# adam-kerrigan/pybader

Hardware: AMD Instinct MI355X
Metric: Mvoxels/s neargrid assign+refine on 512^3 grid (higher is better)
Workload: dtype f64; 1 GPU; 512^3 synthetic 8-Gaussian-atom cubic cell (BASELINE config 3), neargrid assign + neargrid edge refinement changed:2, density resident in HBM; method=neargrid, device_driven_slab_step=False, basins=8

## Files before the change

include/bader_hip.h:

```cpp
#ifndef BADER_HIP_H
#define BADER_HIP_H

#include <stdint.h>

#ifdef __cplusplus
extern "C" {
#endif

typedef struct xb_ctx xb_ctx;

enum { XB_OK = 0, XB_E_ARG = -1, XB_E_HIP = -2, XB_E_STATE = -3, XB_E_LIMIT = -4, XB_E_COMM = -5,
       XB_E_SHORT = -6  };

enum { XB_I8 = 1, XB_I16 = 2, XB_I32 = 4, XB_I64 = 8 };

enum { XB_METHOD_ONGRID = 0, XB_METHOD_NEARGRID = 1 };
enum { XB_REFINE_ALL = 0, XB_REFINE_CHANGED = 1 };

const char *xb_last_error(void);
int xb_device_count(void);
int xb_create(int device, xb_ctx **out);
void xb_destroy(xb_ctx *c);
int xb_sync(xb_ctx *c);
void *xb_stream(xb_ctx *c);
// ... 123 lines not shown
    XB_XC_LOST = 5,
    XB_XC_MINE = 6,
    XB_XC_ROUNDS = 7,
    XB_XC_COUNT = 8
};
int xb_slab_refine_counts(xb_ctx *c, int64_t *local, int64_t *global);
int xb_slab_block(xb_ctx *c, int which, void **dev_ptr, int64_t *bytes_total, int64_t *own_offset, int64_t *own_bytes);
int xb_slab_block_copy(xb_ctx *c, int which, int to_device, void *host, int64_t off, int64_t bytes);
int xb_host_waits(int64_t *n);

enum {
    XB_TIMER_ASSIGN = 0,
    XB_TIMER_OG_MASKS = 1,
    XB_TIMER_EDGE_FIND = 2,
    XB_TIMER_REFINE_TRACE = 3,
    XB_TIMER_MASKS_GROWTH = 4,
    XB_TIMER_BRICK_MASKS = 5,
    XB_TIMER_TRACE = 6,
    XB_TIMER_BRICK_RECORDS = 7,
    XB_TIMER_MOMENTS = 8,
    XB_TIMER_ADJACENCY = 9,
    XB_TIMER_MERGE = 10,
    XB_TIMER_COUNT = 11
};
int xb_kernel_time(xb_ctx *c, int which, double *ms_total, int64_t *launches);
int xb_kernel_time_reset(xb_ctx *c);
int xb_enable_timing(xb_ctx *c, int on);
enum {
    XB_OPT_REGIONS = 1,
    XB_OPT_CROSS_CHECK = 2,
    XB_OPT_DEBUG = 3,
    XB_OPT_EC_GROUPS = 4,
    XB_OPT_EC_QCAP = 5,
    XB_OPT_DROP_TABLE = 6,
    XB_OPT_KILL_LAUNCHES = 17,
    XB_OPT_SELF_EXCHANGE = 19,
    XB_OPT_ASYNC_COMM = 24,
    XB_OPT_WEIGHT_NO_LABELS = 30
};
enum {
    XB_REGIONS_BOXES = 1,
    XB_REGIONS_BRICKS = 2
};
enum { XB_DROP_TABLE_AND_MAXIMA = 2 };
enum {
    XB_CHECK_NO_MIRROR = 1,
    XB_CHECK_GENERIC_WALKER = 2,
    XB_CHECK_FULL_TGRAD = 4,
    XB_CHECK_LIST_DILATE = 8,
    XB_CHECK_WIDE_HALO = 16,
    XB_CHECK_NO_EC_SHARE = 32,
    XB_CHECK_IO_GATHER = 64
};
enum {
    XB_DBG_EC_PASSES = 4,
    XB_DBG_SLAB_STATS = 16,
    XB_DBG_STAGE_WAIT = 32,
    XB_DBG_SHORT_TIERS = 64
};
int xb_set_option(xb_ctx *c, int key, int value);
int xb_host_alloc(int64_t bytes, void **out);
int xb_host_free(void *p);
int xb_memory_stats(xb_ctx *c, int64_t *bytes_total, int64_t *bytes_table, int64_t *bytes_scratch);
int xb_box_stats(xb_ctx *c, int64_t *n_boxes, int64_t *box_voxels);
int xb_brick_labels(xb_ctx *c, int32_t *out, int64_t capacity, int64_t dims[3]);
int xb_slow_path_stats(xb_ctx *c, int64_t *assign_total, int64_t *refine_total);
int xb_deferred_stats(xb_ctx *c, int64_t *refine_total);
int xb_growth_stats(xb_ctx *c, int64_t *retries, int64_t *kill_launches);

int xb_comm_unique_id(uint8_t id_out[128]);
int xb_comm_init(xb_ctx *c, int rank, int nranks, const uint8_t id_in[128]);
int xb_comm_destroy(xb_ctx *c);
int xb_comm_exchange_planes(xb_ctx *c, int which, int n_send, const int32_t *send_peer, const int64_t *send_xa,
                            const int64_t *send_xb, int n_recv, const int32_t *recv_peer, const int64_t *recv_xa,
                            const int64_t *recv_xb);
int xb_comm_allreduce_i64(xb_ctx *c, int64_t *inout, int64_t n, int op);
int xb_comm_allgather_i64(xb_ctx *c, const int64_t *in, int64_t n, int64_t *out);
int xb_comm_share_brick_masks(xb_ctx *c, const int64_t *first, const int64_t *count);
int xb_comm_allgather_block(xb_ctx *c, int which, const int64_t *first, const int64_t *count);
int xb_comm_allreduce_block(xb_ctx *c);
int xb_comm_info(xb_ctx *c, int64_t out[4]);
int xb_comm_stats(xb_ctx *c, int64_t *bytes_sent);

#ifdef __cplusplus
}
#endif
#endif
```

pybader_amd/_lib.py:

```python
import ctypes as C
import threading
import os

import numpy as np

HERE = os.path.dirname(os.path.abspath(__file__))
LIB_PATH = os.environ.get('XB_LIBRARY') or os.path.join(HERE, 'libbader_hip.so')

METHODS = {'ongrid': 0, 'neargrid': 1}
REFINE_MODES = {'all': 0, 'changed': 1}
DTYPE_CODE = {np.dtype(np.int8): 1, np.dtype(np.int16): 2, np.dtype(np.int32): 4, np.dtype(np.int64): 8}
(XB_XC_EDGES, XB_XC_CHANGED, XB_XC_ESCAPED, XB_XC_TRAVELLING, XB_XC_SLOW, XB_XC_LOST, XB_XC_MINE, XB_XC_ROUNDS,
 XB_XC_COUNT) = range(9)
(XB_TIMER_ASSIGN, XB_TIMER_OG_MASKS, XB_TIMER_EDGE_FIND, XB_TIMER_REFINE_TRACE, XB_TIMER_MASKS_GROWTH, XB_TIMER_BRICK_MASKS,
 XB_TIMER_TRACE, XB_TIMER_BRICK_RECORDS, XB_TIMER_MOMENTS, XB_TIMER_ADJACENCY, XB_TIMER_MERGE, XB_TIMER_COUNT) = range(12)
XB_OPT_REGIONS = 1
XB_REGIONS_BOXES, XB_REGIONS_BRICKS = 1, 2
XB_OPT_CROSS_CHECK = 2
(XB_CHECK_NO_MIRROR, XB_CHECK_GENERIC_WALKER, XB_CHECK_FULL_TGRAD, XB_CHECK_LIST_DILATE, XB_CHECK_WIDE_HALO,
 XB_CHECK_NO_EC_SHARE, XB_CHECK_IO_GATHER) = (1, 2, 4, 8, 16, 32, 64)
XB_OPT_DEBUG = 3
XB_DBG_EC_PASSES, XB_DBG_SLAB_STATS, XB_DBG_STAGE_WAIT, XB_DBG_SHORT_TIERS = 4, 16, 32, 64
XB_OPT_EC_GROUPS = 4
XB_OPT_EC_QCAP = 5
XB_OPT_DROP_TABLE = 6
XB_DROP_TABLE_AND_MAXIMA = 2
XB_OPT_KILL_LAUNCHES = 17
XB_OPT_SELF_EXCHANGE = 19
XB_OPT_ASYNC_COMM = 24
XB_OPT_WEIGHT_NO_LABELS = 30
XB_VORONOI_FULL_SEARCH = 1
XB_VORONOI_CAND_MAX = 512

_vp, _i64, _dbl, _int = C.c_void_p, C.c_int64, C.c_double, C.c_int
_pi64, _pdbl = C.POINTER(C.c_int64), C.POINTER(C.c_double)
SYMBOLS = {
    'xb_last_error': (C.c_char_p, []),
    'xb_device_count': (_int, []),
    'xb_create': (_int, [_int, C.POINTER(_vp)]),
    'xb_destroy': (None, [_vp]),
    'xb_sync': (_int, [_vp]),
    'xb_stream': (_vp, [_vp]),
    'xb_set_grid': (_int, [_vp, _pi64, _pdbl, _pdbl, _i64, _i64]),
    'xb_upload_density': (_int, [_vp, _vp]),
    'xb_synth_density': (_int, [_vp, _pdbl, _pdbl, _i64, _dbl]),
    'xb_parse_density_text': (_int, [_vp, _vp, _i64, _dbl, _pi64, _pi64]),
    'xb_parse_cube_text': (_int, [_vp, _vp, _i64, _i64, _i64, _int, _dbl, _pi64, _pi64]),
    'xb_download_density': (_int, [_vp, _vp]),
    'xb_format_begin': (_int, [_vp, _vp, _pi64, _int, _dbl, _int, _int, _vp, _i64, _i64, _pi64]),
    'xb_format_host_values': (_int, [_vp, _vp, _vp]),
    'xb_format_set_host_text': (_int, [_vp, _vp, _vp]),
    'xb_format_next': (_int, [_vp, C.POINTER(_vp), _pi64]),
    'xb_format_times': (_int, [_vp, _pdbl, _pdbl]),
    'xb_format_end': (_int, [_vp]),
    'xb_upload_labels': (_int, [_vp, _vp, _int]),
    'xb_download_labels': (_int, [_vp, _vp, _int]),
    'xb_import_density': (_int, [_vp, _vp, _int, _pi64, _vp]),
    'xb_import_labels': (_int, [_vp, _vp, _int, _vp]),
    'xb_export_labels': (_int, [_vp, _vp, _int, _vp]),
    'xb_export_volume': (_int, [_vp, _i64, _vp, _int, _vp]),
    'xb_device_alloc': (_int, [_int, _i64, C.POINTER(_vp)]),
    'xb_device_free': (_int, [_vp]),
    'xb_device_read': (_int, [_vp, _vp, _vp, _i64, _vp]),
    'xb_upload_known': (_int, [_vp, _vp]),
    'xb_download_known': (_int, [_vp, _vp]),
    'xb_vacuum_assign': (_int, [_vp, _dbl, _dbl, _pdbl, _pdbl]),
    'xb_assign': (_int, [_vp, _int, _pi64]),
    'xb_get_maxima': (_int, [_vp, _vp, _i64]),
    'xb_assign_trace': (_int, [_vp, _int, _pi64]),
    'xb_assign_local_table': (_int, [_vp, _vp, _vp, _i64]),
    'xb_assign_finish': (_int, [_vp, _vp, _i64]),
    'xb_prepare_refine': (_int, [_vp]),
    'xb_edge_find': (_int, [_vp, _pi64]),
# ... 930 lines not shown
```

pybader_amd/csrc/bader_hip.hip:

```cpp
#include "bader_kernels.h"
#include "../../include/bader_hip.h"

#include <algorithm>
#include <cmath>
#include <cstdarg>
#include <cstdio>
#include <cstring>
#include <string>
#include <thread>
#include <vector>

static thread_local long long xb_waits = 0;
static inline hipError_t xb_counted_sync(hipStream_t s) { xb_waits++; return (hipStreamSynchronize)(s); }
#define hipStreamSynchronize(s) xb_counted_sync(s)

#include "k_common.h"
#include "k_masks.h"
#include "k_fused.h"
#include "k_trace.h"
#include "k_ongrid.h"
#include "k_edges.h"
#include "k_sums.h"
#include "k_text.h"
#include "k_format.h"
// ... 6 lines not shown

static thread_local std::string g_err;
static int fail(int code, const char *fmt, ...) {
    char buf[512];
    va_list ap;
    va_start(ap, fmt);
    vsnprintf(buf, sizeof buf, fmt, ap);
    va_end(ap);
    g_err = buf;
    return code;
}
#define XB_BIG_CHUNK ((size_t)16 << 20)
#define HIPCHK(x)                                                                                   \
    do {                                                                                            \
        hipError_t e_ = (x);                                                                        \
        if (e_ != hipSuccess) return fail(XB_E_HIP, "%s:%d %s: %s", __FILE__, __LINE__, #x, hipGetErrorString(e_)); \
    } while (0)

struct TimedKernel {
    std::vector<std::pair<hipEvent_t, hipEvent_t>> pending;
    double ms = 0.;
    long long launches = 0;
};

namespace xbcomm { struct State; }
struct xb_ctx {
    int device = 0;
    xbcomm::State *comm = nullptr;
    struct FmtState *fmt = nullptr;
    hipStream_t stream = nullptr;
    Grid g{};
    bool has_grid = false;
    long long N = 0;
    int halo = 0;
    double *rho = nullptr;
    GradRec *grad = nullptr;
    long long grad_cap = 0;
    long long list_cap = 0;
    int *ec_buf = nullptr;
    long long ec_buf_cap = 0;
    double *dist_dev = nullptr;
    int *boxbuf = nullptr;
    int *box_max_tab = nullptr;
    int n_boxes = 0;
    long long box_voxels = 0;
    struct Options {
        int boxes = 1, bricks = 1;
        int mirror = 1;
        int lean = 1;
        int mask_diag = 1;
        int tile_dilate = 1;
        int narrow_halo = 1;
        int ec_share = 1;
        int io_tiled = 1;
        int dbg = 0;
        int ec_groups = 256;
        int ec_qcap = EC_Q;
        int self_exchange = 0;
        int async_comm = 0;
        bool weight_no_labels = false;
    } opt;
    int *ec_share = nullptr;
    std::vector<int64_t> esc_starts, esc_offsets, esc_vox;
    unsigned long long *ec_pend = nullptr;
    int8_t *ec_pflag = nullptr;
    std::vector<int8_t> esc_complete;
    bool has_vacuum = true;
    bool vac_by_tol = false;
    double vac_tol = 0.;
    bool regions_pending = false;
    bool buni_valid = false;
    bool buni_halo_safe = false;
    bool regions_neargrid = false;
    bool regions_labels = false;
    int n_walk = 0;
    int *walk = nullptr;
    int table_margin = -1;
    bool table_prebuilt = false;
    int table_stage = 0;
    std::vector<int> window_seeds;
    bool window_ties = true;
    bool slab_sparse = false;
    int ec_local_n = 0;
    int walk_n_out = 0;
    void *walk_out_dev = nullptr;
    std::vector<int64_t> walk_host, res_host;
    int walk_n_res = 0;
    void *walk_in = nullptr, *walk_out2 = nullptr, *walk_res = nullptr;
    long long walk_cap = 0;
    long long stat_deferred = 0;
    long long stat_ovf_assign = 0, stat_ovf_refine = 0;
    int *bres_last = nullptr;
    int *blab = nullptr;
    int nbk[3] = {0, 0, 0};
    bool grad_valid = false;
    bool brick_max_valid = false;
    int grad_cover = 0;
    unsigned char *brick_rec = nullptr;
    void *xbuf = nullptr;
    int slab_rank = 0, slab_nranks = 0, slab_stage = 0;
    void *wbuf[2] = {nullptr, nullptr};
    void *wk_in = nullptr;
    int wbuf_ranks = 0, walk_last = -1, walk_round = 0, wcap = 0;
    int walk_send = 0;
    int grow_kill_launches = 6;
    long long stat_grow_retries = 0;
    bool defer_wait = false;
    bool pending_assign = false;
    int64_t pending_n_maxima = 0;
    int grad_rule = 0;
    int *labels = nullptr;
    int8_t *known = nullptr;
    int *first = nullptr;
    int *list = nullptr;
    int8_t *st = nullptr;
    void *stage = nullptr;
    size_t stage_bytes = 0;
    int *max_list = nullptr;
    int *max_aux = nullptr;
    int max_cap = 0;
    int *ovf_list = nullptr;
    int ovf_cap = 0;
    int *counters = nullptr;
    int *fs = nullptr;
    int *blab_buf = nullptr;
    long long blab_alloc = 0;
    bool labels_zero_pending = false;
    int zero_outside[3] = {-1, -1, -1};
    static constexpr int trace_waves = 8192;
    unsigned long long *counters64 = nullptr;
    double *dsum = nullptr;
    int *host_ints = nullptr;
    char *big_pin[2] = {nullptr, nullptr};
    hipEvent_t big_ev[2] = {nullptr, nullptr};
    hipEvent_t io_ev = nullptr;
    char *pin = nullptr;
    size_t pin_bytes = 0;
    std::vector<int> maxima_sorted;
    int label_wire = 4;
    std::vector<int> local_max, local_first;
    bool first_clean = false;
    int chg_n = -1;
    int list_n = 0;
    bool list_valid = false;
    unsigned timing = 0;
    TimedKernel tk[XB_TIMER_COUNT];
    long long n_alloc = 0;
    bool thin = false;
    double *w_A = nullptr, *w_V = nullptr, *w_S = nullptr;
    unsigned char *w_pending = nullptr;
    int *w_list[2] = {nullptr, nullptr};
// ... 82 lines not shown
                ip[(ax + 1) % 3] = im[(ax + 1) % 3] = u;
                ip[(ax + 2) % 3] = im[(ax + 2) % 3] = v;
                const double a = g.dist[ip[0] * 9 + ip[1] * 3 + ip[2]], b = g.dist[im[0] * 9 + im[1] * 3 + im[2]];
                ok = std::memcmp(&a, &b, sizeof a) == 0;
            }
        if (ok) mirror |= 1 << ax;
    }
    mu_scale = std::ldexp(1. + 1. / dmin, -48);
}

struct ScopedTimer {
    xb_ctx *c;
    int which;
    hipEvent_t a = nullptr, b = nullptr;
    ScopedTimer(xb_ctx *c_, int w) : c(c_), which(w) {
        if ((c->timing >> which) & 1u) {
            hipEventCreate(&a);
            hipEventCreate(&b);
            hipEventRecord(a, c->stream);
        }
    }
    ~ScopedTimer() {
        if ((c->timing >> which) & 1u) {
            hipEventRecord(b, c->stream);
            c->tk[which].pending.push_back({a, b});
        }
    }
};

extern "C" {

const char *xb_last_error(void) { return g_err.c_str(); }

#include "host_context.h"
#include "host_stages.h"
#include "host_format.h"
#include "host_assign.h"
#include "host_refine.h"
#include "host_sums.h"
#include "host_slab_table.h"
#include "host_interop.h"
#include "host_weight.h"
#include "host_moments.h"
#include "host_adjacency.h"
#include "host_merge.h"
#include "host_voronoi.h"

int xb_set_option(xb_ctx *c, int key, int value) {
    if (!c) return fail(XB_E_ARG, "null ctx");
    bool ok = true;
    switch (key) {
    case XB_OPT_REGIONS: c->opt.boxes = (value & XB_REGIONS_BOXES) != 0; c->opt.bricks = (value & XB_REGIONS_BRICKS) != 0; break;
    case XB_OPT_CROSS_CHECK:
        c->opt.mirror = !(value & XB_CHECK_NO_MIRROR);
        c->opt.lean = !(value & XB_CHECK_GENERIC_WALKER);
        c->opt.mask_diag = !(value & XB_CHECK_FULL_TGRAD);
        c->opt.tile_dilate = !(value & XB_CHECK_LIST_DILATE);
        c->opt.narrow_halo = !(value & XB_CHECK_WIDE_HALO);
        c->opt.ec_share = !(value & XB_CHECK_NO_EC_SHARE);
        c->opt.io_tiled = !(value & XB_CHECK_IO_GATHER);
        break;
    case XB_OPT_DEBUG: c->opt.dbg = value; break;
    case XB_OPT_EC_GROUPS: if ((ok = value >= 1 && value <= 4096)) c->opt.ec_groups = value; break;
    case XB_OPT_EC_QCAP: if ((ok = value >= 2 && value <= EC_Q)) c->opt.ec_qcap = value; break;
    case XB_OPT_DROP_TABLE: c->grad_valid = false; if (value == XB_DROP_TABLE_AND_MAXIMA) c->brick_max_valid = false; break;
    case XB_OPT_KILL_LAUNCHES: if ((ok = value >= 1)) c->grow_kill_launches = value; break;
    case XB_OPT_SELF_EXCHANGE: c->opt.self_exchange = value != 0; break;
    case XB_OPT_ASYNC_COMM: c->opt.async_comm = value != 0; break;
    case XB_OPT_WEIGHT_NO_LABELS: c->opt.weight_no_labels = value != 0; break;
    default: ok = false;
    }
    if (!ok) return fail(XB_E_ARG, "xb_set_option: unknown key %d", key);
    return XB_OK;
}
int xb_growth_stats(xb_ctx *c, int64_t *retries, int64_t *kill_launches) {
    if (!c) return fail(XB_E_ARG, "null ctx");
    if (retries) *retries = c->stat_grow_retries;
    if (kill_launches) *kill_launches = c->grow_kill_launches;
    return XB_OK;
}
int xb_deferred_stats(xb_ctx *c, int64_t *refine_total) {
    if (!c) return fail(XB_E_ARG, "null ctx");
    if (refine_total) *refine_total = c->stat_deferred;
    return XB_OK;
}
int xb_slow_path_stats(xb_ctx *c, int64_t *assign_total, int64_t *refine_total) {
    if (!c) return fail(XB_E_ARG, "null ctx");
    if (assign_total) *assign_total = c->stat_ovf_assign;
    if (refine_total) *refine_total = c->stat_ovf_refine;
    return XB_OK;
}
int xb_memory_stats(xb_ctx *c, int64_t *bytes_total, int64_t *bytes_table, int64_t *bytes_scratch) {
    if (!c || !c->has_grid) return fail(XB_E_STATE, "xb_memory_stats: no grid");
    const long long N = c->N;
    const long long table = c->grad_cap * (long long)sizeof(GradRec);
    const long long scratch = c->list_cap * 4 + (long long)c->stage_bytes + c->ec_buf_cap * 4 + (c->ec_pend ? 8 * N + 16 : 0) +
                              (c->w_cap ? 25 * c->w_cap + (c->w_S ? 8 * c->w_cap : 0) : 0)  +
                              (long long)c->m_cap * 8  +
                              (long long)c->aj_bytes  +
                              (long long)c->mg_cap * MG_BYTES  +
                              (long long)c->vo_cap * 8 ;
    const long long fixed = 8 * N  + 4 * N  + (N + 16)  + 4 * N  + N  +
                            2LL * c->max_cap * 4 + (long long)c->ovf_cap * 4 + c->blab_alloc * 5 + (long long)c->walk_cap * 3 * 80 +
                            (1 << 22) ;
    if (bytes_total) *bytes_total = fixed + table + scratch;
    if (bytes_table) *bytes_table = table;
    if (bytes_scratch) *bytes_scratch = scratch;
    return XB_OK;
}
int xb_box_stats(xb_ctx *c, int64_t *n_boxes, int64_t *box_voxels) {
    if (!c) return fail(XB_E_ARG, "null ctx");
    if (n_boxes) *n_boxes = c->n_boxes;
    if (box_voxels) *box_voxels = c->box_voxels;
    return XB_OK;
}
int xb_brick_labels(xb_ctx *c, int32_t *out, int64_t capacity, int64_t dims[3]) {
    if (!c || !c->has_grid) return fail(XB_E_STATE, "xb_brick_labels: no grid");
    if (!c->blab) return fail(XB_E_STATE, "xb_brick_labels: no trapping regions on this context (no neargrid assignment yet)");
    const int64_t nbr = (int64_t)c->nbk[0] * c->nbk[1] * c->nbk[2];
    if (dims) { dims[0] = c->nbk[0]; dims[1] = c->nbk[1]; dims[2] = c->nbk[2]; }
    if (!out) return XB_OK;
    if (capacity < nbr) return fail(XB_E_ARG, "xb_brick_labels: capacity too small");
    HIPCHK(hipSetDevice(c->device));
    HIPCHK(hipMemcpyAsync(out, c->blab, nbr * sizeof(int), hipMemcpyDeviceToHost, c->stream));
    HIPCHK(hipStreamSynchronize(c->stream));
    return XB_OK;
}
#ifdef XB_DEBUG_COUNT
int xb_debug_steps(xb_ctx *c, int on, signed char *host_out) {
    static signed char *buf = nullptr;
    if (host_out && buf) {
        if (hipMemcpy(host_out, buf, (size_t)c->N, hipMemcpyDeviceToHost) != hipSuccess) return XB_E_HIP;
    }
    if (on && !buf && hipMalloc(&buf, (size_t)c->N) != hipSuccess) return XB_E_HIP;
    if (on && hipMemset(buf, 0, (size_t)c->N) != hipSuccess) return XB_E_HIP;
    signed char *p = on ? buf : nullptr;
    return hipMemcpyToSymbol(HIP_SYMBOL(xb_dbg_steps), &p, sizeof p) == hipSuccess ? XB_OK : XB_E_HIP;
}
int xb_debug_counts(unsigned long long *out, int reset) {
    hipDeviceSynchronize();
    if (out && hipMemcpyFromSymbol(out, HIP_SYMBOL(xb_dbg), sizeof(unsigned long long) * 65536) != hipSuccess) return XB_E_HIP;
    if (reset) {
        static unsigned long long z[65536];
        if (hipMemcpyToSymbol(HIP_SYMBOL(xb_dbg), z, sizeof z) != hipSuccess) return XB_E_HIP;
    }
    return XB_OK;
}
#endif
int xb_enable_timing(xb_ctx *c, int on) {
    if (!c) return fail(XB_E_ARG, "null ctx");
    c->timing = on == 0 ? 0u : (on == 1 ? (1u << XB_TIMER_COUNT) - 1u : ((unsigned)on >> 1));
    return XB_OK;
}
int xb_kernel_time_reset(xb_ctx *c) {
    if (!c) return fail(XB_E_ARG, "null ctx");
    HIPCHK(hipSetDevice(c->device));
// ... 33 lines not shown
```

pybader_amd/csrc/bader_kernels.h:

```cpp
#pragma once
#include <hip/hip_runtime.h>
#include <stdint.h>

struct Grid {
    int nx, ny, nz;
    int nyz;
    int x0, x1;
    int vx0, vlen;
    int wx0, wlen;
    int wbase, ntot;
    int main_ties;
    double T[9];
    double dist[27];
};

struct GridS {
    int nx, ny, nz, nyz;
    int x0, x1, vx0, vlen;
    int wx0, wlen;
    int wbase, ntot;
    int main_ties;
    double T[9];
    double dsym[14];
};
// ... 47 lines not shown
__device__ __forceinline__ bool axis_flat(int main_ties, double hi, double c, double lo) {
    return main_ties ? (hi <= c && c >= lo) : (hi < c && c > lo);
}
__device__ __forceinline__ bool axis_tie(double hi, double c, double lo) {
    return (hi <= c && c >= lo) && !(hi < c && c > lo);
}
template <typename GT>
__device__ __forceinline__ bool ng_dir_vals(const GT &g, double c, double hx, double lx, double hy, double ly,
                                            double hz, double lz, double &d0, double &d1, double &d2) {
    const double g0 = axis_flat(g.main_ties, hx, c, lx) ? 0. : (hx - lx) / 2.;
    const double g1 = axis_flat(g.main_ties, hy, c, ly) ? 0. : (hy - ly) / 2.;
    const double g2 = axis_flat(g.main_ties, hz, c, lz) ? 0. : (hz - lz) / 2.;
    d0 = ((g.T[0] * g0) + (g.T[1] * g1)) + (g.T[2] * g2);
    d1 = ((g.T[3] * g0) + (g.T[4] * g1)) + (g.T[5] * g2);
    d2 = ((g.T[6] * g0) + (g.T[7] * g1)) + (g.T[8] * g2);
    const double mg = fmax(fmax(fabs(d0), fabs(d1)), fabs(d2));
    if (mg < 1E-14) return true;
    d0 /= mg; d1 /= mg; d2 /= mg;
    return false;
}
__device__ __forceinline__ bool ng_dir(const double *__restrict__ rho, const Grid &g, int px, int py, int pz,
                                       int lp, double c, double &d0, double &d1, double &d2) {
    const int xp = wrapi(px + 1, g.nx), xm = wrapi(px - 1, g.nx);
    const int yp = wrapi(py + 1, g.ny), ym = wrapi(py - 1, g.ny);
    const int zp = wrapi(pz + 1, g.nz), zm = wrapi(pz - 1, g.nz);
    const double hx = rho[lp + (xp - px) * g.nyz], lx = rho[lp + (xm - px) * g.nyz];
    const double hy = rho[lp + (yp - py) * g.nz], ly = rho[lp + (ym - py) * g.nz];
    const double hz = rho[lp + (zp - pz)], lz = rho[lp + (zm - pz)];
    return ng_dir_vals(g, c, hx, lx, hy, ly, hz, lz, d0, d1, d2);
}

__device__ __forceinline__ int rha_cs(double x) { return (int)(x + __builtin_copysign(0.5, x)); }
__device__ __forceinline__ void ng_move(const Grid &g, int px, int py, int pz, double d0, double d1, double d2,
                                        double &dr0, double &dr1, double &dr2, int &qx, int &qy, int &qz) {
    int ig, id;
    ig = rha_cs(d0); dr0 += d0 - (double)ig; id = rha_cs(dr0); qx = px + ig + id; dr0 -= (double)id;
    ig = rha_cs(d1); dr1 += d1 - (double)ig; id = rha_cs(dr1); qy = py + ig + id; dr1 -= (double)id;
    ig = rha_cs(d2); dr2 += d2 - (double)ig; id = rha_cs(dr2); qz = pz + ig + id; dr2 -= (double)id;
    qx = wrapi(qx, g.nx); qy = wrapi(qy, g.ny); qz = wrapi(qz, g.nz);
}

__device__ __forceinline__ bool ng_step(const double *__restrict__ rho, const Grid &g, int px, int py, int pz,
                                        int lp, double c, double &dr0, double &dr1, double &dr2, int &qx,
                                        int &qy, int &qz) {
    double d0, d1, d2;
    if (ng_dir(rho, g, px, py, pz, lp, c, d0, d1, d2)) { qx = px; qy = py; qz = pz; return true; }
    ng_move(g, px, py, pz, d0, d1, d2, dr0, dr1, dr2, qx, qy, qz);
    return false;
}

struct __attribute__((aligned(32))) GradRec { double r0, r1, r2, key; };
#define XB_STAY_CODE 63
#define XB_OG_SELF 13
#define XB_MAX_BOXES 1023
__device__ __forceinline__ GradRec fetch_rec(const GradRec *__restrict__ G, int l) {
    return *reinterpret_cast<const GradRec *>(reinterpret_cast<const char *>(G) + ((unsigned long long)(unsigned)l << 5));
}

template <typename GT>
__device__ __forceinline__ int rec_slot(const GT &g, int l) {
    const int s = l - g.wbase;
    return s + ((s >> 31) & g.ntot);
}
template <typename GT>
__device__ __forceinline__ GradRec fetch_rec_w(const GT &g, const GradRec *__restrict__ G, int l) { return fetch_rec(G, rec_slot(g, l)); }

__device__ __forceinline__ double pack_key(double rho, int code, int og) {
    return __longlong_as_double((__double_as_longlong(rho) & ~0x1FFFFFLL) | (long long)(code | (og << 6)));
}
__device__ __forceinline__ double key_floor(double rho) {
    const long long b = __double_as_longlong(rho);
    return __longlong_as_double(b >= 0 ? (b & ~0x1FFFFFLL) : (b | 0x1FFFFFLL));
}
__device__ __forceinline__ int key_bits(double key) { return (int)(__double_as_longlong(key) & 0x1FFFFFLL); }
__device__ __forceinline__ int key_code(double key) { return key_bits(key) & 63; }
__device__ __forceinline__ int key_og(double key) { return (key_bits(key) >> 6) & 31; }
__device__ __forceinline__ int key_box(double key) { return key_bits(key) >> 11; }

__device__ __forceinline__ int wrap_u(int q, int n) {
    unsigned u = min((unsigned)q, (unsigned)(q + n));
    return (int)min(u, u - (unsigned)n);
}
__device__ __forceinline__ int lin3f(const GridL &g, int x, int y, int z) {
    if (g.use24) return (int)__umul24(__umul24(x, g.ny) + y, g.nz) + z;
    return (x * g.ny + y) * g.nz + z;
}
__device__ __forceinline__ void ng_move_t(const GridL &g, int px, int py, int pz, const GradRec &rec, int code,
                                          double &dr0, double &dr1, double &dr2, int &qx, int &qy, int &qz) {
    int id;
    dr0 += rec.r0; id = rha_cs(dr0); qx = px + ((code & 3) - 1) + id; dr0 -= (double)id;
    dr1 += rec.r1; id = rha_cs(dr1); qy = py + (((code >> 2) & 3) - 1) + id; dr1 -= (double)id;
    dr2 += rec.r2; id = rha_cs(dr2); qz = pz + ((code >> 4) - 1) + id; dr2 -= (double)id;
    qx = wrap_u(qx, g.nx); qy = wrap_u(qy, g.ny); qz = wrap_u(qz, g.nz);
}

template <typename GT>
__device__ __forceinline__ void og_step(const double *__restrict__ rho, const GT &g, const double *__restrict__ dist,
                                        int px, int py, int pz, double ctr, int &qx, int &qy, int &qz) {
    double max_val = ctr;
    qx = px; qy = py; qz = pz;
#pragma unroll
    for (int ix = -1; ix < 2; ix++) {
        const int tx = wrapi(px + ix, g.nx);
#pragma unroll
        for (int iy = -1; iy < 2; iy++) {
            const int ty = wrapi(py + iy, g.ny);
#pragma unroll
            for (int iz = -1; iz < 2; iz++) {
                const int tz = wrapi(pz + iz, g.nz);
                double v = rho[(tx * g.ny + ty) * g.nz + tz];
                v = (v - ctr) * dist[((ix + 3) % 3) * 9 + ((iy + 3) % 3) * 3 + ((iz + 3) % 3)];
                v += ctr;
                if (v > max_val) { max_val = v; qx = tx; qy = ty; qz = tz; }
            }
        }
    }
}

template <int K>
struct PathWindow {
    int idx[K];
    double val[K];
    double m_old;
    __device__ __forceinline__ void init(int l, double c) {
#pragma unroll
        for (int k = 0; k < K; k++) { idx[k] = -1; val[k] = -1.7976931348623157e308; }
        idx[0] = l; val[0] = c;
        m_old = -1.7976931348623157e308;
    }
    __device__ __forceinline__ bool contains(int l) const {
// ... 57 lines not shown
```

pybader_amd/csrc/host_assign.h:

```cpp

static GridL light(const Grid &g);

static int ensure_brick_bytes(xb_ctx *c, int nbr) {
    if (c->blab_alloc < nbr) {
        hipFree(c->blab_buf); c->blab_buf = nullptr; c->blab_alloc = 0; c->brick_rec = nullptr; c->brick_max_valid = false;
        if (c->grad_cover) { c->grad_cover = 0; c->grad_valid = false; }
        HIPCHK(hipMalloc(&c->blab_buf, (size_t)nbr * sizeof(int) + (size_t)nbr + 16));
        c->blab_alloc = nbr;
        c->brick_rec = reinterpret_cast<unsigned char *>(c->blab_buf + nbr);
    }
    return XB_OK;
}

static int ensure_grad(xb_ctx *c, bool force, bool boxes, bool main_rule) {
    if (int rc = need_grad(c)) return rc;
    c->g.main_ties = main_rule ? 1 : 0;
    if (c->grad_valid && !force && (c->grad_rule == 2 || c->grad_rule == (main_rule ? 1 : 0))) return XB_OK;
    const Grid &g = c->g;
    if (c->grad_valid && !force && !boxes && c->grad_cover == 1 && c->brick_rec) {
        const int nb1r = (g.ny + BRK - 1) / BRK, nb2r = (g.nz + BRK - 1) / BRK, nbr = ((g.nx + BRK - 1) / BRK) * nb1r * nb2r;
        ScopedTimer t(c, XB_TIMER_MASKS_GROWTH);
        launch_brick_records(c, nullptr, nullptr, nbr, nb1r, nb2r);
        HIPCHK(hipGetLastError());
        c->grad_rule = main_rule ? 1 : 0;
        return XB_OK;
    }
    if (!force && !boxes && !table_windowed(c) && g.x0 == 0 && g.x1 == g.nx && g.nx >= 16 && g.ny >= 16 && g.nz >= 16) {
        const int nb0 = (g.nx + BRK - 1) / BRK, nb1 = (g.ny + BRK - 1) / BRK, nb2 = (g.nz + BRK - 1) / BRK, nbr = nb0 * nb1 * nb2;
        if (int rc = ensure_brick_bytes(c, nbr)) return rc;
        ScopedTimer t(c, XB_TIMER_MASKS_GROWTH);
        int *buni = reinterpret_cast<int *>(c->st);
        if (!c->buni_valid) k_label_uniform_list<<<4096, TPB, 0, c->stream>>>(light(g), c->labels, nb1, nb2, nullptr, nbr, nullptr, nullptr, buni, 0, nbr);
        c->buni_valid = true;
        k_buni3<<<(nbr + 255) / 256, 256, 0, c->stream>>>(nb0, nb1, nb2, buni, buni + nbr);
        k_flag_mixed_bricks<<<(nbr + 255) / 256, 256, 0, c->stream>>>(nbr, buni + nbr, c->brick_rec);
        launch_brick_records(c, nullptr, nullptr, nbr, nb1, nb2);
        HIPCHK(hipGetLastError());
        c->grad_valid = true;
        c->grad_cover = 1;
        c->grad_rule = main_rule ? 1 : 0;
        c->regions_labels = false;
        c->blab = nullptr;
        c->table_stage = 0;
        return XB_OK;
    }
    {
        const int nb0 = (g.nx + BRK - 1) / BRK, nb1 = (g.ny + BRK - 1) / BRK, nb2 = (g.nz + BRK - 1) / BRK, nbr = nb0 * nb1 * nb2;
        if (int rc = ensure_brick_bytes(c, nbr)) return rc;
        ScopedTimer t(c, XB_TIMER_MASKS_GROWTH);
        ScopedTimer t_masks(c, XB_TIMER_BRICK_MASKS);
        const int wb0 = table_windowed(c) ? g.wx0 / BRK : 0, wnb = table_windowed(c) ? g.wlen / BRK : nb0;
        k_flag_window_bricks<<<(nbr + 255) / 256, 256, 0, c->stream>>>(nb0, nb1 * nb2, wb0, wnb, (unsigned char)3, c->brick_rec);
        launch_brick_records(c, nullptr, nullptr, nbr, nb1, nb2);
        HIPCHK(hipGetLastError());
    }
    c->grad_valid = true;
    c->grad_cover = 1;
    c->grad_rule = main_rule ? 1 : 0;
    c->window_ties = true;
    c->n_boxes = 0;
    c->box_voxels = 0;
    c->blab = nullptr;
// ... 403 lines not shown
            const bool vac = c->has_vacuum && c->vac_by_tol;
            k_brick_walk_list_morton<<<(n_codes + 16 * TPB - 1) / (16 * TPB), TPB, 0, c->stream>>>(nb0, nb1, nb2, n_codes, c->blab, walk,
                                                                                                  fs + FS_N_WALK, fs + FS_GROW_RETRY,
                                                                                                  vac ? bpot : nullptr, c->vac_tol);
        }
        {
            ScopedTimer t_records(c, XB_TIMER_BRICK_RECORDS);
            launch_brick_records(c, walk, fs + FS_N_WALK, nbr, nb1, nb2);
        }
        stage_done("walk list + records");
        if (c->has_vacuum)
            k_fill_certain<<<nblocks(own), TPB, 0, c->stream>>>(gl, c->blab, nb1, nb2, box_max, c->labels, c->first, c->max_list,
                                                                fs + FS_N_MAX, c->max_cap, fs + FS_GROW_RETRY);
        else {
            k_note_regions<<<1, XB_BOXES_MAX, 0, c->stream>>>(gl, nb1, nb2, fs, box_first, box_max, c->first, c->max_list, fs + FS_N_MAX, c->max_cap);
            c->regions_pending = true;
        }
        {
            ScopedTimer t_trace(c, XB_TIMER_TRACE);
            int *bres_buf = c->has_vacuum ? nullptr : c->list + 6 * nbr;
            if (launch_persistent_trace(c, true, part, box_max, walk, c->has_vacuum ? 1 : 0, bres_buf)) bres = bres_buf;
        }
        HIPCHK(hipGetLastError());
        stage_done("trace");
    }
    c->bres_last = bres;
    if (int rc = fused_numbering_launch(c)) return rc;
    stage_done("numbering + relabel");
    HIPCHK(hipMemcpyAsync(c->host_ints, fs, (FS_TOTAL + XB_SORT_MAX) * sizeof(int), hipMemcpyDeviceToHost, c->stream));
    if (c->defer_wait) {
        g.main_ties = 0;
        c->grad_rule = 2;
        c->regions_pending = false;
        c->buni_valid = !c->has_vacuum;
        c->regions_labels = !c->has_vacuum;
        c->pending_assign = true;
        return XB_OK;
    }
    HIPCHK(hipStreamSynchronize(c->stream));
    return assign_neargrid_tail(c, n_maxima);
}

static int assign_neargrid_tail(xb_ctx *c, int64_t *n_maxima) {
    Grid &g = c->g;
    int *fs = c->fs;
    const int nb1 = c->nbk[1], nb2 = c->nbk[2];
    int *walk = c->walk, *box_max = c->box_max_tab;
    const int *h = c->host_ints;
    g.main_ties = 0;
    const GridL gl = light(g);
    if (h[FS_GROW_RETRY]) {
        c->grow_kill_launches = 1 << 20;
        c->stat_grow_retries++;
        c->grad_valid = false;
        return assign_neargrid_fused(c, n_maxima);
    }
    if (h[FS_TIES] == 0) c->grad_rule = 2;
    c->n_boxes = h[FS_N_BOXES];
    c->box_voxels = (long long)h[FS_N_CERTAIN] * BRK * BRK * BRK;
    c->n_walk = h[FS_N_WALK];
    const int novf = h[FS_N_OVF];
    int nmax = h[FS_N_MAX];
    if (nmax > c->max_cap) return fail(XB_E_LIMIT, "%d maxima exceed the table capacity %d", nmax, c->max_cap);
    c->stat_ovf_assign += novf;
    const int *sorted = h[FS_SORT_OK] && novf == 0 ? h + FS_TOTAL : nullptr;
    if (novf > 0) {
        g.main_ties = 1;
        const GridL glt = light(g);
        const int maxsteps = trace_maxsteps(g);
        int *list2 = (int *)c->stage;
        const int cap2 = (int)std::min<size_t>(c->stage_bytes / sizeof(int), 0x7fffffffu);
        auto two_tiers = [&](int n_listed) -> int {
            c->host_ints[HI_UPLOAD] = n_listed;
            HIPCHK(hipMemcpyAsync(c->counters + CT_MID_LISTED, c->host_ints + HI_UPLOAD, sizeof(int), hipMemcpyHostToDevice, c->stream));
            HIPCHK(hipMemsetAsync(c->counters + CT_MID_LEFT, 0, sizeof(int), c->stream));
            k_ng_trace_list<XB_MID_K><<<512, TPB, 0, c->stream>>>(glt, c->grad, box_max, c->blab, nb1, nb2, c->ovf_list, c->counters + CT_MID_LISTED, c->labels, c->first,
                                                          c->max_list, fs + FS_N_MAX, c->max_cap, list2, c->counters + CT_MID_LEFT, cap2, maxsteps, c->rho, c->dist_dev,
                                                          c->has_vacuum ? 1 : 0);
            HIPCHK(hipGetLastError());
            if (c->opt.dbg & XB_DBG_EC_PASSES) {
                int m2 = 0;
                if (int rc2 = read_counter(c, CT_MID_LEFT, &m2)) return rc2;
                fprintf(stderr, "[assign] %d walkers listed, %d left for the exact slow kernel after the %d-voxel window\n", n_listed, m2, XB_MID_K);
            }
            if (n_listed > cap2) return fail(XB_E_LIMIT, "%d walkers for the exact slow path exceed its list (%d)", n_listed, cap2);
            return run_slow(c, n_listed, 0, fs + FS_N_MAX, nullptr, nullptr, list2, c->counters + CT_MID_LEFT, true);
        };
        int rc = two_tiers(std::min(novf, c->ovf_cap));
        for (int left = novf - c->ovf_cap; !rc && left > 0;) {
            HIPCHK(hipMemsetAsync(c->counters + CT_N_OVF, 0, sizeof(int), c->stream));
            k_list_unfinished<<<4096, TPB, 0, c->stream>>>(gl, walk, fs + FS_N_WALK, nb1, nb2, c->labels, c->ovf_list, c->counters + CT_N_OVF, c->ovf_cap);
            HIPCHK(hipGetLastError());
            int m = 0;
            if ((rc = read_counter(c, CT_N_OVF, &m))) break;
            if (m == 0) break;
            rc = two_tiers(std::min(m, c->ovf_cap));
            left = m - c->ovf_cap;
        }
        g.main_ties = 0;
        if (rc) return rc;
        HIPCHK(hipMemsetAsync(fs + FS_N_OVF, 0, sizeof(int), c->stream));
        if (int rc2 = fused_numbering_launch(c)) return rc2;
        HIPCHK(hipMemcpyAsync(c->host_ints, fs, (FS_TOTAL + XB_SORT_MAX) * sizeof(int), hipMemcpyDeviceToHost, c->stream));
        HIPCHK(hipStreamSynchronize(c->stream));
        nmax = h[FS_N_MAX];
        if (nmax > c->max_cap) return fail(XB_E_LIMIT, "%d maxima exceed the table capacity %d", nmax, c->max_cap);
        if (h[FS_SORT_OK]) sorted = h + FS_TOTAL;
// ... 1 lines not shown
    if (!sorted) {
        if (int rc = number_maxima_big(c, nmax)) return rc;
    }
    numbering_done(c, sorted, nmax, n_maxima);
    c->buni_valid = !c->has_vacuum;
    c->regions_labels = !c->has_vacuum;
    return XB_OK;
}


static bool assign_neargrid_complete(xb_ctx *c, int64_t *n_maxima) {
    c->pending_assign = false;
    const int *h = c->host_ints;
    const int nmax = h[FS_N_MAX];
    if (h[FS_GROW_RETRY] || h[FS_TIES] != 0 || h[FS_N_OVF] != 0 || !h[FS_SORT_OK] || nmax > c->max_cap || nmax > XB_SORT_MAX) return false;
    c->n_boxes = h[FS_N_BOXES];
    c->box_voxels = (long long)h[FS_N_CERTAIN] * BRK * BRK * BRK;
    c->n_walk = h[FS_N_WALK];
    numbering_done(c, h + FS_TOTAL, nmax, n_maxima);
    return true;
}

static int assign_ongrid_fused(xb_ctx *c, int64_t *n_maxima) {
    Grid &g = c->g;
    const int nb0 = (g.nx + BRK - 1) / BRK, nb1 = (g.ny + BRK - 1) / BRK, nb2 = (g.nz + BRK - 1) / BRK, nbr = nb0 * nb1 * nb2;
    const bool part = g.nx % BRK || g.ny % BRK || g.nz % BRK;
    if (int rc = ensure_brick_bytes(c, nbr)) return rc;
    int *fs = c->fs;
    int *seed = c->list, *bmask = c->list + nbr, *buf0 = c->list + 2 * nbr, *buf1 = c->list + 3 * nbr, *walk = c->list + 4 * nbr;
    int *bmaxv = walk, *bpot = c->list + 5 * nbr;
    int *box_max = c->boxbuf + BB_REGMAX, *box_first = c->boxbuf + BB_REGFIRST;
    c->box_max_tab = box_max;
    if (int rc = begin_assignment(c, fs, FS_TOTAL, true)) return rc;
    c->zero_outside[0] = -1;
    const GridL gl = light(g);
    {
        ScopedTimer t(c, XB_TIMER_OG_MASKS);
        const int small = small_grid(g);
        dim3 grid((g.nz + GT_Z - 1) / GT_Z, (g.ny + GT_Y - 1) / GT_Y, (g.nx + GT_X - 1) / GT_X);
        GridS gs;
        if (sym_grid(g, gs)) {
            if (part) k_og_masks<GridS, true><<<grid, TPB, 0, c->stream>>>(gs, c->rho, c->labels, small, 0, bmask, bmaxv, bpot);
            else k_og_masks<GridS, false><<<grid, TPB, 0, c->stream>>>(gs, c->rho, c->labels, small, 0, bmask, bmaxv, bpot);
        } else {
            if (part) k_og_masks<Grid, true><<<grid, TPB, 0, c->stream>>>(g, c->rho, c->labels, small, 0, bmask, bmaxv, bpot);
            else k_og_masks<Grid, false><<<grid, TPB, 0, c->stream>>>(g, c->rho, c->labels, small, 0, bmask, bmaxv, bpot);
        }
    }
    {
        ScopedTimer t_growth(c, XB_TIMER_MASKS_GROWTH);
        launch_region_growth(c, nb0, nb1, nb2, bmask, bmaxv, bpot, seed, buf0, buf1, box_max, box_first, true);
        HIPCHK(hipGetLastError());
    }
    c->grad_valid = false;
    c->grad_cover = 0;
    c->brick_max_valid = true;
    c->blab = c->blab_buf;
    c->regions_neargrid = false;
    c->walk = walk;
    c->bres_last = nullptr;
    c->nbk[0] = nb0; c->nbk[1] = nb1; c->nbk[2] = nb2;
    {
        ScopedTimer t_assign(c, XB_TIMER_ASSIGN);
        int bits = 0;
        while ((1 << bits) < std::max(std::max(nb0, nb1), nb2)) bits++;
        const unsigned n_codes = 1u << (3 * bits);
        k_brick_walk_list_morton<<<(n_codes + 16 * TPB - 1) / (16 * TPB), TPB, 0, c->stream>>>(nb0, nb1, nb2, n_codes, c->blab, walk,
                                                                                              fs + FS_N_WALK, fs + FS_GROW_RETRY);
        k_note_regions<<<1, XB_BOXES_MAX, 0, c->stream>>>(gl, nb1, nb2, fs, box_first, box_max, c->first, c->max_list, fs + FS_N_MAX, c->max_cap);
        c->regions_pending = true;
        k_og_walk_dev<<<16384, XB_WAVE, 0, c->stream>>>(gl, box_max, c->blab, nb1, nb2, walk, fs, c->labels, c->first, c->max_list, c->max_cap,
                                                        1 << 22);
        HIPCHK(hipGetLastError());
    }
    if (int rc = fused_numbering_launch(c)) return rc;
    HIPCHK(hipMemcpyAsync(c->host_ints, fs, (FS_TOTAL + XB_SORT_MAX) * sizeof(int), hipMemcpyDeviceToHost, c->stream));
    HIPCHK(hipStreamSynchronize(c->stream));
    const int *h = c->host_ints;
    if (h[FS_GROW_RETRY]) {
        c->grow_kill_launches = 1 << 20;
        c->stat_grow_retries++;
        return assign_ongrid_fused(c, n_maxima);
    }
    if (h[FS_ERR] & 1) return fail(XB_E_STATE, "ongrid pointer chase did not terminate");
    c->n_boxes = h[FS_N_BOXES];
    c->box_voxels = (long long)h[FS_N_CERTAIN] * BRK * BRK * BRK;
    c->n_walk = h[FS_N_WALK];
    const int nmax = h[FS_N_MAX];
    if (nmax > c->max_cap) return fail(XB_E_LIMIT, "%d maxima exceed the table capacity %d", nmax, c->max_cap);
    const int *sorted = h[FS_SORT_OK] ? h + FS_TOTAL : nullptr;
    if (!sorted) {
        if (int rc = number_maxima_big(c, nmax)) return rc;
    }
    numbering_done(c, sorted, nmax, n_maxima);
    c->buni_valid = true;
    return XB_OK;
}

static int sort_and_finish(xb_ctx *c, int64_t n, int64_t *n_maxima);
int xb_assign(xb_ctx *c, int method, int64_t *n_maxima) {
    NEED_GRID_RAW("xb_assign");
    c->have_labels = true;
    if (method == XB_METHOD_NEARGRID && fused_ok(c)) {
        if (c->has_vacuum) { if (int rc = settle_labels(c)) return rc; }
        else c->labels_zero_pending = false;
        return assign_neargrid_fused(c, n_maxima);
    }
// ... 43 lines not shown
```

pybader_amd/csrc/host_context.h:

```cpp

int xb_device_count(void) {
    int n = 0;
    if (hipGetDeviceCount(&n) != hipSuccess) return 0;
    return n;
}

int xb_create(int device, xb_ctx **out) {
    if (!out) return fail(XB_E_ARG, "xb_create: null out");
    int n = 0;
    hipError_t e = hipGetDeviceCount(&n);
    if (e != hipSuccess || n <= 0)
        return fail(XB_E_HIP, "xb_create: no HIP device visible (%s); libbader_hip has no CPU fallback",
                    e == hipSuccess ? "device count 0" : hipGetErrorString(e));
    if (device < 0 || device >= n) return fail(XB_E_ARG, "xb_create: device %d out of range [0,%d)", device, n);
    HIPCHK(hipSetDevice(device));
    xb_ctx *c = new xb_ctx();
    c->device = device;
    HIPCHK(hipStreamCreate(&c->stream));
    HIPCHK(hipMalloc(&c->counters, (1024 + XB_SORT_MAX) * sizeof(int)));
    c->fs = c->counters + CT_FS;
    HIPCHK(hipMalloc(&c->counters64, 16 * sizeof(unsigned long long)));
    HIPCHK(hipMalloc(&c->dsum, 16 * sizeof(double)));
    HIPCHK(hipMalloc(&c->dist_dev, 36 * sizeof(double)));
    HIPCHK(hipMalloc(&c->boxbuf, (size_t)(1 << 20) * sizeof(int)));
    HIPCHK(hipHostMalloc(&c->host_ints, HI_TOTAL * sizeof(int)));
    *out = c;
    return XB_OK;
}

static void weight_free(xb_ctx *c);
static void moments_free(xb_ctx *c);
static void adjacency_free(xb_ctx *c);
static void merge_free(xb_ctx *c);
static void voronoi_free(xb_ctx *c);
static void free_grid(xb_ctx *c) {
    weight_free(c);
    moments_free(c);
    adjacency_free(c);
    merge_free(c);
    voronoi_free(c);
    c->have_rho = c->have_labels = false;
    hipFree(c->rho); hipFree(c->grad); hipFree(c->labels); hipFree(c->known); hipFree(c->first); hipFree(c->list);
    hipFree(c->st); hipFree(c->stage); hipFree(c->ec_pend); c->ec_pend = nullptr; hipFree(c->ec_share); c->ec_share = nullptr; hipFree(c->ec_pflag); c->ec_pflag = nullptr; hipFree(c->max_list); hipFree(c->max_aux); hipFree(c->ovf_list);
    hipFree(c->blab_buf); c->blab_buf = nullptr; c->blab_alloc = 0; c->labels_zero_pending = false;
    hipFree(c->ec_buf); c->ec_buf = nullptr; c->ec_buf_cap = 0; c->grad_cap = 0; c->list_cap = 0;
    c->brick_rec = nullptr; c->grad_cover = 0;
    c->rho = nullptr; c->grad = nullptr; c->grad_valid = false; c->brick_max_valid = false; c->labels = nullptr; c->known = nullptr; c->first = nullptr; c->list = nullptr;
    c->st = nullptr; c->stage = nullptr; c->max_list = nullptr; c->max_aux = nullptr; c->ovf_list = nullptr;
    c->n_alloc = 0; c->stage_bytes = 0;
}

int xb_comm_destroy(xb_ctx *c);
static void fmt_release(xb_ctx *c);
void xb_destroy(xb_ctx *c) {
    if (!c) return;
    hipSetDevice(c->device);
    hipStreamSynchronize(c->stream);
    xb_comm_destroy(c);
    fmt_release(c);
    for (auto &t : c->tk)
        for (auto &p : t.pending) { hipEventDestroy(p.first); hipEventDestroy(p.second); }
    free_grid(c);
    hipFree(c->counters); hipFree(c->counters64); hipFree(c->dsum); hipFree(c->dist_dev); hipFree(c->boxbuf);
    hipFree(c->walk_in); hipFree(c->walk_out2); hipFree(c->walk_res); hipFree(c->xbuf); hipFree(c->wbuf[0]); hipFree(c->wbuf[1]); hipFree(c->wk_in);
    hipHostFree(c->host_ints);
    hipHostFree(c->pin);
    for (int k = 0; k < 2; k++) { hipHostFree(c->big_pin[k]); if (c->big_ev[k]) hipEventDestroy(c->big_ev[k]); }
    if (c->io_ev) hipEventDestroy(c->io_ev);
    hipStreamDestroy(c->stream);
    delete c;
}

int xb_sync(xb_ctx *c) {
    HIPCHK(hipSetDevice(c->device));
    HIPCHK(hipStreamSynchronize(c->stream));
    return XB_OK;
}
void *xb_stream(xb_ctx *c) { return (void *)c->stream; }

#define XB_SYNTH_ATOMS_MAX 4096
#define XB_SURFACE_ATOMS_MAX 100000
#define XB_STAGE_FLOOR ((size_t)4 << 20)
static_assert((16 + 5 * (size_t)XB_SYNTH_ATOMS_MAX) * sizeof(double) <= XB_STAGE_FLOOR &&
              (16 + 4 * (size_t)XB_SURFACE_ATOMS_MAX) * sizeof(double) <= XB_STAGE_FLOOR, "stage floor below a documented atom maximum");
static int need_scratch(xb_ctx *c) {
    const Grid &g = c->g;
    const long long N = c->N ? c->N : (long long)g.nx * g.nyz;
    const int own = g.x1 - g.x0;
    long long planes = own + 2LL * (std::max(c->halo, 16) + 16);
    if (own == g.nx || planes >= g.nx) planes = g.nx;
    const long long list_want = planes == g.nx ? N : std::max<long long>(planes * g.nyz, 8 * (N / 512) + 4096);
    const size_t stage_want = planes == g.nx ? std::max<size_t>((size_t)N * 8, XB_STAGE_FLOOR) : std::max<size_t>((size_t)planes * g.nyz * 8, (size_t)64 << 20);
    if (c->list_cap < list_want) {
        HIPCHK(hipStreamSynchronize(c->stream));
        hipFree(c->list); c->list = nullptr; c->list_cap = 0;
        HIPCHK(hipMalloc(&c->list, (size_t)list_want * sizeof(int)));
        c->list_cap = list_want;
        c->list_valid = false; c->chg_n = -1; c->walk = nullptr; c->n_walk = 0;
    }
    if (c->stage_bytes < stage_want) {
        HIPCHK(hipStreamSynchronize(c->stream));
        hipFree(c->stage); c->stage = nullptr; c->stage_bytes = 0;
        HIPCHK(hipMalloc(&c->stage, stage_want));
        c->stage_bytes = stage_want;
    }
    return XB_OK;
}
static int need_grad(xb_ctx *c) {
    Grid &g = c->g;
    const long long want = (long long)g.wlen * g.nyz;
    g.wbase = g.wlen < g.nx ? g.wx0 * g.nyz : 0;
    g.ntot = (int)c->N;
    if (c->grad_cap < want || c->grad_cap > 2 * want) {
        HIPCHK(hipStreamSynchronize(c->stream));
        hipFree(c->grad); c->grad = nullptr; c->grad_cap = 0; c->grad_valid = false; c->brick_max_valid = false;
        HIPCHK(hipMalloc(&c->grad, (size_t)want * sizeof(GradRec)));
        c->grad_cap = want;
    }
    return XB_OK;
}

static void set_valid_range(xb_ctx *c) {
    Grid &g = c->g;
    const int own = g.x1 - g.x0;
    if (own + 2 * c->halo >= g.nx) { g.vx0 = 0; g.vlen = g.nx; }
    else {
        const int hv = c->halo - 2;
        g.vx0 = ((g.x0 - hv) % g.nx + g.nx) % g.nx;
        g.vlen = own + 2 * hv;
    }
}

int xb_set_grid(xb_ctx *c, const int64_t shape[3], const double dist_mat[27], const double T_grad[9],
                int64_t x0, int64_t x1) {
    if (!c || !shape) return fail(XB_E_ARG, "xb_set_grid: null argument");
    bool thin = false;
    for (int j = 0; j < 3; j++) {
        if (shape[j] < 1) return fail(XB_E_ARG, "xb_set_grid: every axis needs >= 1 voxel (got %lld)", (long long)shape[j]);
        thin = thin || shape[j] < 3;
    }
    const long long N = (long long)shape[0] * shape[1] * shape[2];
    if (N >= 2147483647LL) return fail(XB_E_LIMIT, "xb_set_grid: %lld voxels exceed the int32 index range", N);
    if (x0 < 0 || x1 > shape[0] || x0 >= x1) return fail(XB_E_ARG, "xb_set_grid: bad slab [%lld,%lld)", (long long)x0, (long long)x1);
    HIPCHK(hipSetDevice(c->device));
    if (N != c->n_alloc) {
        free_grid(c);
        HIPCHK(hipMalloc(&c->rho, N * sizeof(double)));
        HIPCHK(hipMalloc(&c->labels, N * sizeof(int)));
        HIPCHK(hipMalloc(&c->known, N + 16));
        HIPCHK(hipMalloc(&c->first, N * sizeof(int)));
        HIPCHK(hipMalloc(&c->st, N));
        c->max_cap = (int)std::min<long long>(N, 1 << 22);
        HIPCHK(hipMalloc(&c->max_list, c->max_cap * sizeof(int)));
        HIPCHK(hipMalloc(&c->max_aux, c->max_cap * sizeof(int)));
        c->ovf_cap = (int)std::min<long long>(N, std::max<long long>(1 << 22, N / 16));
        HIPCHK(hipMalloc(&c->ovf_list, c->ovf_cap * sizeof(int)));
        c->n_alloc = N;
        c->first_clean = false;
    }
    c->zero_outside[0] = -1;
    Grid &g = c->g;
    if (g.nx != (int)shape[0] || g.ny != (int)shape[1] || g.nz != (int)shape[2]) { c->grad_valid = false; c->brick_max_valid = false; c->have_rho = c->have_labels = false; adjacency_free(c); merge_free(c); }
    if (dist_mat && !T_grad) return fail(XB_E_ARG, "xb_set_grid: dist_mat without T_grad");
    g.nx = (int)shape[0]; g.ny = (int)shape[1]; g.nz = (int)shape[2];
    g.nyz = g.ny * g.nz;
    g.x0 = (int)x0; g.x1 = (int)x1;
    if (dist_mat) {
        if (memcmp(g.dist, dist_mat, sizeof g.dist) != 0) { c->grad_valid = false; c->brick_max_valid = false; }
        memcpy(g.dist, dist_mat, sizeof g.dist);
        HIPCHK(hipMemcpyAsync(c->dist_dev, dist_mat, sizeof g.dist, hipMemcpyHostToDevice, c->stream));
        HIPCHK(hipMemcpyAsync(c->dist_dev + 27, T_grad, sizeof g.T, hipMemcpyHostToDevice, c->stream));
        HIPCHK(hipStreamSynchronize(c->stream));
    }
    if (T_grad && memcmp(g.T, T_grad, sizeof g.T) != 0) { memcpy(g.T, T_grad, sizeof g.T); c->grad_valid = false; c->brick_max_valid = false; }
    c->N = N;
    c->thin = thin;
    c->halo = (x0 == 0 && x1 == shape[0]) ? g.nx : 0;
    set_valid_range(c);
    g.wx0 = 0; g.wlen = g.nx;
    g.wbase = 0; g.ntot = (int)N;
    c->table_margin = -1;
    if (int rc = need_scratch(c)) return rc;
    c->table_stage = 0;
    c->has_grid = true;
    c->maxima_sorted.clear();
    c->label_wire = 4;
    if (!c->first_clean) {
        k_fill<int><<<4096, TPB, 0, c->stream>>>(c->first, XB_INT_MAX, N);
        HIPCHK(hipGetLastError());
        c->first_clean = true;
    }
    return XB_OK;
}

static int settle_labels(xb_ctx *c);
int xb_set_halo(xb_ctx *c, int64_t halo) {
    if (!c || !c->has_grid) return fail(XB_E_STATE, "xb_set_halo: no grid");
    if (halo < 2) return fail(XB_E_ARG, "xb_set_halo: halo must be >= 2 planes");
    HIPCHK(hipSetDevice(c->device));
    if (int rc = settle_labels(c)) return rc;
    c->zero_outside[0] = -1;
    c->halo = (int)halo;
    set_valid_range(c);
    return need_scratch(c);
}

static int zero_slab_labels(xb_ctx *c) {
    const Grid &g = c->g;
    const int len = std::min(g.nx, (g.x1 - g.x0) + 2 * c->halo), first = ((g.x0 - c->halo) % g.nx + g.nx) % g.nx;
    const int run1 = std::min(len, g.nx - first);
    HIPCHK(hipMemsetAsync(c->labels + (size_t)first * g.nyz, 0, (size_t)run1 * g.nyz * sizeof(int), c->stream));
    if (len > run1) HIPCHK(hipMemsetAsync(c->labels, 0, (size_t)(len - run1) * g.nyz * sizeof(int), c->stream));
    return XB_OK;
}
static int settle_labels(xb_ctx *c) {
    if (c->labels_zero_pending) {
        c->labels_zero_pending = false;
        if (c->g.x1 - c->g.x0 == c->g.nx) HIPCHK(hipMemsetAsync(c->labels, 0, c->N * sizeof(int), c->stream));
        else return zero_slab_labels(c);
    }
    return XB_OK;
}
#define NEED_GRID_RAW_THIN(name) \
    if (!c || !c->has_grid) return fail(XB_E_STATE, name ": call xb_set_grid first"); \
    HIPCHK(hipSetDevice(c->device))
#define NEED_GRID_RAW(name) \
    NEED_GRID_RAW_THIN(name); \
// ... 32 lines not shown
        const size_t n = std::min<size_t>(XB_BIG_CHUNK, bytes - off);
        HIPCHK(hipEventSynchronize(c->big_ev[k]));
        copy_threads(c->big_pin[k], (const char *)src_host + off, n);
        HIPCHK(hipMemcpyAsync((char *)dst_dev + off, c->big_pin[k], n, hipMemcpyHostToDevice, c->stream));
        HIPCHK(hipEventRecord(c->big_ev[k], c->stream));
        off += n;
    }
    return XB_OK;
}
int xb_host_alloc(int64_t bytes, void **out) {
    if (!out || bytes <= 0) return fail(XB_E_ARG, "xb_host_alloc: bad argument");
    void *p = nullptr;
    HIPCHK(hipHostMalloc(&p, (size_t)bytes));
    *out = p;
    return XB_OK;
}
int xb_host_free(void *p) {
    if (p) HIPCHK(hipHostFree(p));
    return XB_OK;
}
static bool host_pinned(const void *p) {
    hipPointerAttribute_t a;
    if (hipPointerGetAttributes(&a, p) != hipSuccess) { (void)hipGetLastError(); return false; }
    return a.type == hipMemoryTypeHost;
}
static int staged_d2h(xb_ctx *c, void *dst_host, const void *src_dev, size_t bytes) {
    if (bytes < (4u << 20) || host_pinned(dst_host)) {
        HIPCHK(hipMemcpyAsync(dst_host, src_dev, bytes, hipMemcpyDeviceToHost, c->stream));
        HIPCHK(hipStreamSynchronize(c->stream));
        return XB_OK;
    }
    if (int rc = big_buffers(c)) return rc;
    size_t off = 0, prev_off = 0, prev_n = 0;
    int prev = -1;
    for (int k = 0; off < bytes; k ^= 1) {
        const size_t n = std::min<size_t>(XB_BIG_CHUNK, bytes - off);
        HIPCHK(hipMemcpyAsync(c->big_pin[k], (const char *)src_dev + off, n, hipMemcpyDeviceToHost, c->stream));
        HIPCHK(hipEventRecord(c->big_ev[k], c->stream));
        if (prev >= 0) {
            HIPCHK(hipEventSynchronize(c->big_ev[prev]));
            copy_threads((char *)dst_host + prev_off, c->big_pin[prev], prev_n);
        }
        prev = k; prev_off = off; prev_n = n;
        off += n;
    }
    HIPCHK(hipEventSynchronize(c->big_ev[prev]));
    copy_threads((char *)dst_host + prev_off, c->big_pin[prev], prev_n);
    return XB_OK;
}

int xb_upload_density(xb_ctx *c, const double *rho_host) {
    if (c) c->vac_by_tol = false;
    NEED_GRID_THIN("xb_upload_density");
    c->grad_valid = false; c->brick_max_valid = false; c->have_rho = true;
    if (int rc = staged_h2d(c, c->rho, rho_host, c->N * sizeof(double))) return rc;
    HIPCHK(hipStreamSynchronize(c->stream));
    return XB_OK;
}
int xb_download_density(xb_ctx *c, double *rho_host) {
    NEED_GRID_THIN("xb_download_density");
    HIPCHK(hipMemcpyAsync(rho_host, c->rho, c->N * sizeof(double), hipMemcpyDeviceToHost, c->stream));
    HIPCHK(hipStreamSynchronize(c->stream));
    return XB_OK;
}

static int read_counter(xb_ctx *c, int idx, int *out) {
    HIPCHK(hipMemcpyAsync(c->host_ints, c->counters + idx, sizeof(int), hipMemcpyDeviceToHost, c->stream));
    HIPCHK(hipStreamSynchronize(c->stream));
    *out = c->host_ints[0];
    return XB_OK;
}
static int device_scan(xb_ctx *c, int *data, int n, int *scratch) {
    const int nb = (n + 2047) / 2048;
    k_scan_2048<<<nb, TPB, 0, c->stream>>>(data, n, data, scratch);
    HIPCHK(hipGetLastError());
    if (nb > 1) {
        if (int rc = device_scan(c, scratch, nb, scratch + nb)) return rc;
        k_scan_add<<<nb, TPB, 0, c->stream>>>(data, n, scratch);
        HIPCHK(hipGetLastError());
    }
    return XB_OK;
}
extern "C++" {
template <class Map>
static int parse_text(xb_ctx *c, const char *who, const char *text, int64_t nbytes, const Map &map, int64_t *n_tokens,
                      int64_t *n_host) {
    if (!text || nbytes <= 0) return fail(XB_E_ARG, "%s: empty text", who);
    if (nbytes / (TPB * TXT_BYTES) >= (1LL << 31) - 2) return fail(XB_E_LIMIT, "%s: text too large", who);
    c->grad_valid = false; c->brick_max_valid = false; c->have_rho = true;
    static const double P10[23] = {1e0, 1e1, 1e2, 1e3, 1e4, 1e5, 1e6, 1e7, 1e8, 1e9, 1e10, 1e11,
                                   1e12, 1e13, 1e14, 1e15, 1e16, 1e17, 1e18, 1e19, 1e20, 1e21, 1e22};
    const int nblk = (int)((nbytes + TPB * TXT_BYTES - 1) / (TPB * TXT_BYTES));
    const int todo_cap = 1 << 20;
    unsigned char *dtext = nullptr;
    int *counts = nullptr;
    double *dp10 = nullptr;
    long long *dtodo = nullptr;
    int rc = XB_OK;
    auto cleanup = [&]() { hipFree(dtext); hipFree(counts); hipFree(dp10); hipFree(dtodo); };
    hipError_t e = hipMalloc(&dtext, (size_t)nbytes + 32);
    if (e == hipSuccess) e = hipMalloc(&counts, ((size_t)nblk + nblk / 1024 + 4096) * sizeof(int));
    if (e == hipSuccess) e = hipMalloc(&dp10, sizeof P10);
    if (e == hipSuccess) e = hipMalloc(&dtodo, (size_t)todo_cap * 2 * sizeof(long long));
    if (e == hipSuccess) e = hipMemcpyAsync(dtext, text, (size_t)nbytes, hipMemcpyHostToDevice, c->stream);
    if (e == hipSuccess) e = hipMemcpyAsync(dp10, P10, sizeof P10, hipMemcpyHostToDevice, c->stream);
    if (e == hipSuccess) e = hipMemsetAsync(c->counters + CT_TEXT_TODO, 0, sizeof(int), c->stream);
    if (e != hipSuccess) { cleanup(); return fail(XB_E_HIP, "%s: %s", who, hipGetErrorString(e)); }
    int last_count = 0, last_off = 0, n_todo = 0;
    k_text_count<<<nblk, TPB, 0, c->stream>>>(dtext, nbytes, counts);
    e = hipMemcpyAsync(&last_count, counts + nblk - 1, sizeof(int), hipMemcpyDeviceToHost, c->stream);
    if (e == hipSuccess) e = hipStreamSynchronize(c->stream);
    if (e == hipSuccess && (nbytes + 1) / 2 > XB_INT_MAX) {
        std::vector<int> blk(nblk);
        e = hipMemcpyAsync(blk.data(), counts, (size_t)nblk * sizeof(int), hipMemcpyDeviceToHost, c->stream);
        if (e == hipSuccess) e = hipStreamSynchronize(c->stream);
        long long sum = 0;
        for (int b : blk) sum += b;
        if (e == hipSuccess && sum > XB_INT_MAX) rc = fail(XB_E_LIMIT, "%s: %lld numbers in the text, at most %d", who, sum, XB_INT_MAX);
    }
    if (e == hipSuccess && rc == XB_OK) rc = device_scan(c, counts, nblk, counts + nblk);
    if (e == hipSuccess && rc == XB_OK) e = hipMemcpyAsync(&last_off, counts + nblk - 1, sizeof(int), hipMemcpyDeviceToHost, c->stream);
    if (e == hipSuccess && rc == XB_OK) e = hipStreamSynchronize(c->stream);
    const long long tokens = (long long)last_off + last_count;
    if (e == hipSuccess && rc == XB_OK && tokens < map.count())
        rc = fail(XB_E_SHORT, "%s: %lld numbers in the text, the grid needs %lld", who, tokens, map.count());
    if (e == hipSuccess && rc == XB_OK) {
        k_text_parse<<<nblk, TPB, 0, c->stream>>>(dtext, nbytes, counts, dp10, map, c->rho, dtodo, c->counters + CT_TEXT_TODO, todo_cap);
        e = hipGetLastError();
        if (e == hipSuccess) rc = read_counter(c, CT_TEXT_TODO, &n_todo);
    }
    if (e == hipSuccess && rc == XB_OK && n_todo > todo_cap)
        rc = fail(XB_E_LIMIT, "%s: %d tokens need the host parser (cap %d)", who, n_todo, todo_cap);
    if (e == hipSuccess && rc == XB_OK && n_todo) {
        std::vector<long long> todo(2 * (size_t)n_todo), at(n_todo);
        std::vector<double> val(n_todo);
        e = hipMemcpyAsync(todo.data(), dtodo, todo.size() * sizeof(long long), hipMemcpyDeviceToHost, c->stream);
        if (e == hipSuccess) e = hipStreamSynchronize(c->stream);
        for (int k = 0; k < n_todo && e == hipSuccess && rc == XB_OK; k++) {
            const long long off = todo[2 * k], idx = todo[2 * k + 1];
            long long end = off;
            while (end < nbytes && !(text[end] == ' ' || (text[end] >= 9 && text[end] <= 13))) end++;
            const std::string tok(text + off, text + end);
            char *stop = nullptr;
            val[k] = std::strtod(tok.c_str(), &stop);
            if (stop == tok.c_str() || *stop != 0) rc = fail(XB_E_ARG, "%s: could not convert '%s' to a number", who, tok.c_str());
            map.voxel(idx, at[k]);
        }
        if (e == hipSuccess && rc == XB_OK) {
            long long *dat = dtodo;
            double *dval = reinterpret_cast<double *>(dtodo + n_todo);
            e = hipMemcpyAsync(dat, at.data(), n_todo * sizeof(long long), hipMemcpyHostToDevice, c->stream);
            if (e == hipSuccess) e = hipMemcpyAsync(dval, val.data(), n_todo * sizeof(double), hipMemcpyHostToDevice, c->stream);
            if (e == hipSuccess) k_text_patch<<<(n_todo + 255) / 256, 256, 0, c->stream>>>(dat, dval, n_todo, map, c->rho);
            if (e == hipSuccess) e = hipGetLastError();
            if (e == hipSuccess) e = hipStreamSynchronize(c->stream);
        }
    }
    if (e == hipSuccess) e = hipStreamSynchronize(c->stream);
    cleanup();
    if (e != hipSuccess) return fail(XB_E_HIP, "%s: %s", who, hipGetErrorString(e));
    if (rc != XB_OK) return rc;
    if (n_tokens) *n_tokens = tokens;
    if (n_host) *n_host = n_todo;
    return XB_OK;
}
}
int xb_parse_density_text(xb_ctx *c, const char *text, int64_t nbytes, double divisor, int64_t *n_tokens,
                          int64_t *n_host) {
    if (c) c->vac_by_tol = false;
    NEED_GRID("xb_parse_density_text");
    if (!(divisor == divisor) || divisor == 0.) return fail(XB_E_ARG, "xb_parse_density_text: bad divisor");
    const TxtFortran map{c->g.nx, c->g.ny, c->g.nz, divisor};
    return parse_text(c, "xb_parse_density_text", text, nbytes, map, n_tokens, n_host);
}
int xb_parse_cube_text(xb_ctx *c, const char *text, int64_t nbytes, int64_t nval, int64_t pick, int accumulate,
                       double scale, int64_t *n_tokens, int64_t *n_host) {
    if (c) c->vac_by_tol = false;
    NEED_GRID("xb_parse_cube_text");
    if (nval < 1 || pick < 0 || pick >= nval) return fail(XB_E_ARG, "xb_parse_cube_text: bad nval %lld / pick %lld", (long long)nval, (long long)pick);
    if (nval > XB_INT_MAX / c->N) return fail(XB_E_LIMIT, "xb_parse_cube_text: %lld voxels x %lld values exceed %d numbers", (long long)c->N, (long long)nval, XB_INT_MAX);
    const TxtCube map{(long long)c->N * nval, nval, pick, accumulate ? 1 : 0, scale};
    return parse_text(c, "xb_parse_cube_text", text, nbytes, map, n_tokens, n_host);
}

int xb_synth_density(xb_ctx *c, const double lattice[9], const double *atoms5, int64_t n_atoms, double background) {
    if (c) c->vac_by_tol = false;
    NEED_GRID("xb_synth_density");
    if (n_atoms < 0 || n_atoms > XB_SYNTH_ATOMS_MAX) return fail(XB_E_ARG, "xb_synth_density: bad atom count");
    if ((16 + 5 * (size_t)n_atoms) * sizeof(double) > c->stage_bytes)
        return fail(XB_E_LIMIT, "xb_synth_density: %lld atoms do not fit the scratch buffer", (long long)n_atoms);
    c->grad_valid = false; c->brick_max_valid = false; c->have_rho = true;
    double *tmp = (double *)c->stage;
    HIPCHK(hipMemcpyAsync(tmp, lattice, 9 * sizeof(double), hipMemcpyHostToDevice, c->stream));
    HIPCHK(hipMemcpyAsync(tmp + 16, atoms5, n_atoms * 5 * sizeof(double), hipMemcpyHostToDevice, c->stream));
    k_synth_density<<<nblocks(c->N), TPB, 0, c->stream>>>(c->g, tmp, tmp + 16, (int)n_atoms, background, c->rho);
    HIPCHK(hipGetLastError());
    HIPCHK(hipStreamSynchronize(c->stream));
    return XB_OK;
}

static size_t dtype_size(int dtype) { return (dtype == XB_I8 || dtype == XB_I16 || dtype == XB_I32 || dtype == XB_I64) ? (size_t)dtype : 0; }

int xb_upload_labels(xb_ctx *c, const void *labels_host, int dtype) {
    NEED_GRID_RAW_THIN("xb_upload_labels");
    c->labels_zero_pending = false;
    c->zero_outside[0] = -1;
    c->list_valid = false; c->chg_n = -1;
    c->has_vacuum = true;
    c->vac_by_tol = false;
    c->buni_valid = false; c->regions_labels = false;
    const size_t sz = dtype_size(dtype);
    if (!sz) return fail(XB_E_ARG, "xb_upload_labels: bad dtype code %d", dtype);
    c->label_wire = sz >= 4 ? 4 : (int)sz;
    c->have_labels = true;
    if (dtype == XB_I32) {
        if (int rc = staged_h2d(c, c->labels, labels_host, c->N * 4)) return rc;
    } else {
        const long long per = std::max<long long>(1, (long long)(c->stage_bytes / sz));
        for (long long o = 0; o < c->N; o += per) {
            const long long n = std::min(per, c->N - o);
            if (int rc = staged_h2d(c, c->stage, (const char *)labels_host + (size_t)o * sz, (size_t)n * sz)) return rc;
            if (dtype == XB_I8) k_widen<int8_t><<<nblocks(n), TPB, 0, c->stream>>>((const int8_t *)c->stage, c->labels + o, n);
            else if (dtype == XB_I16) k_widen<int16_t><<<nblocks(n), TPB, 0, c->stream>>>((const int16_t *)c->stage, c->labels + o, n);
            else k_widen<long long><<<nblocks(n), TPB, 0, c->stream>>>((const long long *)c->stage, c->labels + o, n);
            HIPCHK(hipGetLastError());
        }
    }
    HIPCHK(hipMemsetAsync(c->counters + CT_ANY_EQUAL, 0, sizeof(int), c->stream));
    k_any_equal<<<2048, TPB, 0, c->stream>>>(c->labels, c->N, -1, c->counters + CT_ANY_EQUAL);
    HIPCHK(hipGetLastError());
    int any = 0;
    if (int rc = read_counter(c, CT_ANY_EQUAL, &any)) return rc;
    c->has_vacuum = any != 0;
    return XB_OK;
}
int xb_download_labels(xb_ctx *c, void *labels_host, int dtype) {
    NEED_GRID_THIN("xb_download_labels");
    const size_t sz = dtype_size(dtype);
    if (!sz) return fail(XB_E_ARG, "xb_download_labels: bad dtype code %d", dtype);
    if (dtype == XB_I32) {
        if (int rc = staged_d2h(c, labels_host, c->labels, c->N * 4)) return rc;
    } else if (void *dev_view = nullptr; host_pinned(labels_host) && hipHostGetDevicePointer(&dev_view, labels_host, 0) == hipSuccess && dev_view) {
        if (dtype == XB_I8 || dtype == XB_I16) {
            const long long per = 16 / (long long)sz, n16 = c->N / per, done = n16 * per;
// ... 78 lines not shown
```

pybader_amd/csrc/host_interop.h:

```cpp

static size_t io_float_size(int dtype) { return dtype == XB_F32 ? 4 : (dtype == XB_F64 ? 8 : 0); }

static int io_check(xb_ctx *c, const char *who, const void *p, size_t isz, const int64_t shape[3], const int64_t stride[3],
                    uintptr_t *lo_out, uintptr_t *hi_out) {
    if (!p) return fail(XB_E_ARG, "%s: null device pointer", who);
    __int128 lo = 0, hi = 0;
    for (int j = 0; j < 3; j++) {
        const __int128 reach = (__int128)(shape[j] - 1) * stride[j];
        (reach < 0 ? lo : hi) += reach;
    }
    lo *= (__int128)isz;
    hi = (hi + 1) * (__int128)isz;
    hipPointerAttribute_t a;
    if (hipPointerGetAttributes(&a, p) != hipSuccess) {
        (void)hipGetLastError();
        return fail(XB_E_ARG, "%s: %p is not memory the HIP runtime knows (a host pointer?)", who, p);
    }
    if (a.type != hipMemoryTypeDevice) return fail(XB_E_ARG, "%s: %p is not device memory (memory type %d)", who, p, (int)a.type);
    if (a.device != c->device) return fail(XB_E_ARG, "%s: %p lives on device %d, the context on device %d", who, p, a.device, c->device);
    hipDeviceptr_t base = nullptr;
    size_t size = 0;
    if (hipMemGetAddressRange(&base, &size, (hipDeviceptr_t)p) != hipSuccess) {
        (void)hipGetLastError();
        return fail(XB_E_ARG, "%s: no allocation holds %p", who, p);
// ... 44 lines not shown
int xb_device_free(void *p) {
    if (p) HIPCHK(hipFree(p));
    return XB_OK;
}

extern "C++" {
template <typename T>
static int io_import_density(xb_ctx *c, const T *src, const int64_t st[3], double *dst) {
    const Grid &g = c->g;
    const long long N = c->N, sx = st[0], sy = st[1], sz = st[2];
    const bool contiguous = sz == 1 && sy == g.nz && sx == g.nyz;
    long long first = 0;
    if (contiguous && sizeof(T) == 8) {
        HIPCHK(hipMemcpyAsync(dst, src, (size_t)N * 8, hipMemcpyDeviceToDevice, c->stream));
        return XB_OK;
    }
    if constexpr (sizeof(T) == 4)
        if (contiguous && (uintptr_t)src % 16 == 0) {
            const long long n4 = N / 4;
            k_io_widen4<<<nblocks(n4), TPB, 0, c->stream>>>(src, dst, n4);
            HIPCHK(hipGetLastError());
            first = 4 * n4;
            if (first == N) return XB_OK;
        }
    if (first == 0 && sz != 1 && (sy == 1 || sx == 1) && c->opt.io_tiled) {
        const bool fy = sy == 1;
        const int nf = fy ? g.ny : g.nx, no = fy ? g.nx : g.ny;
        const int tiles_f = (nf + IO_TILE - 1) / IO_TILE, tiles_z = (g.nz + IO_TILE - 1) / IO_TILE;
        const long long blocks = (long long)tiles_f * tiles_z * no;
        k_io_tiled<T><<<(unsigned)blocks, TPB, 0, c->stream>>>(src, dst, no, nf, g.nz, fy ? sx : sy, sz, fy ? (long long)g.nyz : g.nz,
                                                              fy ? (long long)g.nz : g.nyz, tiles_f, tiles_z);
        HIPCHK(hipGetLastError());
        return XB_OK;
    }
    k_io_gather<T><<<nblocks(N - first), TPB, 0, c->stream>>>(src, dst, g.ny, g.nz, sx, sy, sz, first, N);
    HIPCHK(hipGetLastError());
    return XB_OK;
}
}

int xb_import_density(xb_ctx *c, const void *dev_ptr, int dtype, const int64_t stride[3], void *stream) {
    if (!c || !c->has_grid) return fail(XB_E_ARG, "xb_import_density: call xb_set_grid first");
    const size_t isz = io_float_size(dtype);
    if (!isz) return fail(XB_E_ARG, "xb_import_density: dtype code %d is neither XB_F32 nor XB_F64", dtype);
    if (!stride) return fail(XB_E_ARG, "xb_import_density: null stride");
    if ((uintptr_t)dev_ptr % isz) return fail(XB_E_ARG, "xb_import_density: %p is not aligned to its %zu-byte elements", dev_ptr, isz);
    HIPCHK(hipSetDevice(c->device));
    const int64_t shape[3] = {c->g.nx, c->g.ny, c->g.nz};
    uintptr_t lo, hi;
    if (int rc = io_check(c, "xb_import_density", dev_ptr, isz, shape, stride, &lo, &hi)) return rc;
    if (io_overlaps(lo, hi, c->rho, (size_t)c->N * 8)) return fail(XB_E_ARG, "xb_import_density: the source overlaps the resident density");
    c->vac_by_tol = false;
    NEED_GRID_THIN("xb_import_density");
    c->grad_valid = false; c->brick_max_valid = false; c->have_rho = true;
    const hipStream_t s = (hipStream_t)stream;
    if (int rc = io_after_caller(c, s)) return rc;
    if (int rc = dtype == XB_F32 ? io_import_density(c, (const float *)dev_ptr, stride, c->rho) : io_import_density(c, (const double *)dev_ptr, stride, c->rho)) return rc;
    return io_before_caller(c, s);
}

int xb_import_labels(xb_ctx *c, const void *dev_ptr, int dtype, void *stream) {
    if (!c || !c->has_grid) return fail(XB_E_ARG, "xb_import_labels: call xb_set_grid first");
    const size_t sz = dtype_size(dtype);
    if (!sz) return fail(XB_E_ARG, "xb_import_labels: bad dtype code %d", dtype);
    if ((uintptr_t)dev_ptr % sz) return fail(XB_E_ARG, "xb_import_labels: %p is not aligned to its %zu-byte elements", dev_ptr, sz);
    HIPCHK(hipSetDevice(c->device));
    uintptr_t lo, hi;
    if (int rc = io_check_flat(c, "xb_import_labels", dev_ptr, sz, &lo, &hi)) return rc;
    if (io_overlaps(lo, hi, c->labels, (size_t)c->N * 4)) return fail(XB_E_ARG, "xb_import_labels: the source overlaps the resident labels");
    c->labels_zero_pending = false;
    c->zero_outside[0] = -1;
    c->list_valid = false; c->chg_n = -1;
    c->has_vacuum = true;
    c->vac_by_tol = false;
    c->buni_valid = false; c->regions_labels = false;
    c->label_wire = sz >= 4 ? 4 : (int)sz;
    c->have_labels = true;
    const hipStream_t s = (hipStream_t)stream;
    if (int rc = io_after_caller(c, s)) return rc;
    if (dtype == XB_I32) HIPCHK(hipMemcpyAsync(c->labels, dev_ptr, (size_t)c->N * 4, hipMemcpyDeviceToDevice, c->stream));
    else if (dtype == XB_I8) k_widen<int8_t><<<nblocks(c->N), TPB, 0, c->stream>>>((const int8_t *)dev_ptr, c->labels, c->N);
    else if (dtype == XB_I16) k_widen<int16_t><<<nblocks(c->N), TPB, 0, c->stream>>>((const int16_t *)dev_ptr, c->labels, c->N);
    else k_widen<long long><<<nblocks(c->N), TPB, 0, c->stream>>>((const long long *)dev_ptr, c->labels, c->N);
    HIPCHK(hipGetLastError());
    if (int rc = io_before_caller(c, s)) return rc;
    HIPCHK(hipMemsetAsync(c->counters + CT_ANY_EQUAL, 0, sizeof(int), c->stream));
    k_any_equal<<<2048, TPB, 0, c->stream>>>(c->labels, c->N, -1, c->counters + CT_ANY_EQUAL);
    HIPCHK(hipGetLastError());
    int any = 0;
    if (int rc = read_counter(c, CT_ANY_EQUAL, &any)) return rc;
    c->has_vacuum = any != 0;
    return XB_OK;
}

int xb_export_labels(xb_ctx *c, void *dev_ptr, int dtype, void *stream) {
    if (!c || !c->has_grid) return fail(XB_E_ARG, "xb_export_labels: call xb_set_grid first");
    const size_t sz = dtype_size(dtype);
    if (!sz) return fail(XB_E_ARG, "xb_export_labels: bad dtype code %d", dtype);
    if ((uintptr_t)dev_ptr % sz) return fail(XB_E_ARG, "xb_export_labels: %p is not aligned to its %zu-byte elements", dev_ptr, sz);
    HIPCHK(hipSetDevice(c->device));
    uintptr_t lo, hi;
    if (int rc = io_check_flat(c, "xb_export_labels", dev_ptr, sz, &lo, &hi)) return rc;
    if (io_overlaps(lo, hi, c->labels, (size_t)c->N * 4)) return fail(XB_E_ARG, "xb_export_labels: the destination overlaps the resident labels");
    NEED_GRID_THIN("xb_export_labels");
    const hipStream_t s = (hipStream_t)stream;
    if (int rc = io_after_caller(c, s)) return rc;
    const long long N = c->N;
// ... 46 lines not shown
```

pybader_amd/csrc/host_refine.h:

```cpp

static void plane_range(const Grid &g, int ext, int &xa, int &np) {
    const int own = g.x1 - g.x0;
    if (own + 2 * ext >= g.nx) { xa = 0; np = g.nx; }
    else { xa = ((g.x0 - ext) % g.nx + g.nx) % g.nx; np = own + 2 * ext; }
}

static int preset_known_planes(xb_ctx *c, int p0, int np) {
    const Grid &g = c->g;
    const int run1 = std::min(np, g.nx - p0);
    HIPCHK(hipMemsetAsync(c->known + (size_t)p0 * g.nyz, 2, (size_t)run1 * g.nyz, c->stream));
    if (np > run1) HIPCHK(hipMemsetAsync(c->known, 2, (size_t)(np - run1) * g.nyz, c->stream));
    return XB_OK;
}
static int *launch_brick_uniformity(xb_ctx *c, const GridL &gl, int b_off, int count, unsigned scan_grid) {
    const Grid &g = c->g;
    const int nb0 = (g.nx + 7) / 8, nb1 = (g.ny + 7) / 8, nb2 = (g.nz + 7) / 8, nbr = nb0 * nb1 * nb2;
    int *buni = reinterpret_cast<int *>(c->st);
    if (!c->buni_valid)
        k_label_uniform_list<<<scan_grid, TPB, 0, c->stream>>>(gl, c->labels, nb1, nb2, nullptr, count, nullptr, nullptr, buni, b_off, nbr);
    k_buni3<<<(nbr + 255) / 256, 256, 0, c->stream>>>(nb0, nb1, nb2, buni, buni + nbr);
    return buni + nbr;
}

static int edge_find_launch(xb_ctx *c, bool *dilate_owned) {
// ... 192 lines not shown
        if (e == hipSuccess) e = hipMemcpyAsync(lab, dlab, n * sizeof(int), hipMemcpyDeviceToHost, c->stream);
        if (e == hipSuccess) e = hipMemcpyAsync(kn, dkn, n, hipMemcpyDeviceToHost, c->stream);
    }
    if (e == hipSuccess) e = hipStreamSynchronize(c->stream);
    if (e != hipSuccess) return fail(XB_E_HIP, "xb_gather/scatter_voxels: %s", hipGetErrorString(e));
    return XB_OK;
}
int xb_gather_voxels(xb_ctx *c, const int64_t *idx, int64_t n, int32_t *labels_out, int8_t *known_out) {
    return voxel_io(c, idx, n, labels_out, known_out, false);
}
int xb_scatter_voxels(xb_ctx *c, const int64_t *idx, int64_t n, const int32_t *labels_in, const int8_t *known_in) {
    return voxel_io(c, idx, n, const_cast<int32_t *>(labels_in), const_cast<int8_t *>(known_in), true);
}

static int refine_trace_impl(xb_ctx *c, int flag, int64_t *changed, int64_t *escaped);
int xb_refine_trace(xb_ctx *c, int64_t *changed, int64_t *escaped) { return refine_trace_impl(c, -2, changed, escaped); }
int xb_refine_trace_escaped(xb_ctx *c, int64_t *changed, int64_t *escaped) { return refine_trace_impl(c, -6, changed, escaped); }
static int refine_trace_impl(xb_ctx *c, int flag, int64_t *changed, int64_t *escaped) {
    NEED_GRID("xb_refine_trace");
    const Grid &g = c->g;
    c->g.main_ties = 0;
    int n = 0;
    if (c->list_valid && flag == -2) n = c->list_n;
    else if (int rc = compact(c, flag, &n)) return rc;
    c->list_valid = false; c->chg_n = -1;
    c->buni_valid = false;
    c->walk_n_out = 0; c->walk_n_res = 0; c->walk_out_dev = nullptr;
    c->walk_host.clear(); c->res_host.clear();
    static_assert(CT_ESCAPED == CT_N_MAX + 3 && CT_WALK_OUT == CT_N_MAX + 16, "one memset clears maxima .. escaped; one copy brings back everything up to the exported walkers");
    HIPCHK(hipMemsetAsync(c->counters + CT_N_MAX, 0, CT_INTS(CT_N_MAX, CT_ESCAPED) * sizeof(int), c->stream));
    int n_changed = 0, n_escaped = 0;
    if (n) {
        Walker *wio_out = nullptr;
        int wio_cap = 0;
        if (int rc = ensure_grad(c, false, false, false)) return rc;
        {
            ScopedTimer t(c, XB_TIMER_REFINE_TRACE);
            const unsigned char *brec = c->grad_cover == 1 ? c->brick_rec : nullptr;
            const int regions_ok = brec && c->regions_labels && !c->has_vacuum ? 1 : 0;
            const int *slab_regions = slab_regions_of(c);
            const bool slab = g.vlen < g.nx;
            int *defer = (int *)c->stage;
            WalkerIO wio{};
            if (flag == -2 && slab) {
                const size_t off = (((size_t)n * sizeof(int)) + 255) & ~(size_t)255;
                if (off + sizeof(Walker) <= c->stage_bytes) {
                    HIPCHK(hipMemsetAsync(c->counters + CT_WALK_OUT, 0, sizeof(int), c->stream));
                    wio.out = (Walker *)((char *)c->stage + off); wio.out_count = c->counters + CT_WALK_OUT;
                    wio.out_cap = (int)std::min<size_t>((c->stage_bytes - off) / sizeof(Walker), 1u << 30);
                    c->walk_out_dev = wio.out;
                }
            }
            HIPCHK(hipMemsetAsync(c->counters + CT_DEFER, 0, sizeof(int), c->stream));
            launch_refine_trace<2, false>(c, nblocks(n), TPB, c->list, n, nullptr, c->counters + CT_CHANGED, c->counters + CT_ESCAPED, c->ovf_list,
                                          c->counters + CT_N_OVF, c->ovf_cap, brec, defer, c->counters + CT_DEFER, regions_ok, slab_regions, WalkerIO{});
            if (brec || slab || table_windowed(c))
                launch_refine_trace<2, true>(c, 512, TPB, defer, 0, c->counters + CT_DEFER, c->counters + CT_CHANGED, c->counters + CT_ESCAPED, c->ovf_list,
                                             c->counters + CT_N_OVF, c->ovf_cap, brec, nullptr, nullptr, 0, slab_regions, wio);
            wio_out = wio.out; wio_cap = wio.out_cap;
        }
        HIPCHK(hipGetLastError());
        HIPCHK(hipMemcpyAsync(c->host_ints, c->counters + CT_N_MAX, CT_INTS(CT_N_MAX, CT_WALK_OUT) * sizeof(int), hipMemcpyDeviceToHost, c->stream));
        HIPCHK(hipStreamSynchronize(c->stream));
        const int novf = c->host_ints[CT_N_OVF];
        n_changed = c->host_ints[CT_CHANGED]; n_escaped = c->host_ints[CT_ESCAPED];
        if (wio_out) {
            c->walk_n_out = std::min(c->host_ints[CT_WALK_OUT], wio_cap);
            c->walk_host.resize((size_t)c->walk_n_out * (sizeof(Walker) / 8));
            if (int rc = download_pinned(c, c->walk_host.data(), wio_out, (size_t)c->walk_n_out * sizeof(Walker))) return rc;
        }
        if (novf > c->ovf_cap) return fail(XB_E_LIMIT, "%d retraces need the slow path (cap %d)", novf, c->ovf_cap);
        c->stat_ovf_refine += novf;
        if (novf > 0) {
            if (int rc = run_slow(c, novf, 1)) return rc;
            HIPCHK(hipMemcpyAsync(c->host_ints, c->counters + CT_CHANGED, CT_INTS(CT_CHANGED, CT_ESCAPED) * sizeof(int), hipMemcpyDeviceToHost, c->stream));
            HIPCHK(hipStreamSynchronize(c->stream));
            n_changed = c->host_ints[0]; n_escaped = c->host_ints[1];
        }
    }
    if (changed) *changed = n_changed;
    if (escaped) *escaped = n_escaped;
    return XB_OK;
}

static int ensure_walker_bufs(xb_ctx *c, int64_t n) {
    if (c->walk_cap >= n) return XB_OK;
    (void)hipFree(c->walk_in); (void)hipFree(c->walk_out2); (void)hipFree(c->walk_res);
    c->walk_in = c->walk_out2 = c->walk_res = nullptr; c->walk_cap = 0;
    const size_t cap = (size_t)n + n / 2 + 4096;
    HIPCHK(hipMalloc(&c->walk_in, cap * sizeof(Walker)));
    HIPCHK(hipMalloc(&c->walk_out2, cap * sizeof(Walker)));
    HIPCHK(hipMalloc(&c->walk_res, cap * 2 * sizeof(int)));
    c->walk_cap = (long long)cap;
    return XB_OK;
}
int xb_walkers_count(xb_ctx *c, int64_t *n_walkers, int64_t *n_results) {
    NEED_GRID("xb_walkers_count");
    if (n_walkers) *n_walkers = c->walk_n_out;
    if (n_results) *n_results = c->walk_n_res;
    return XB_OK;
}
int xb_walkers_fetch(xb_ctx *c, int64_t *walkers, int64_t *results) {
    NEED_GRID("xb_walkers_fetch");
    if (walkers && c->walk_n_out) memcpy(walkers, c->walk_host.data(), (size_t)c->walk_n_out * sizeof(Walker));
    if (results && c->walk_n_res) memcpy(results, c->res_host.data(), (size_t)c->walk_n_res * sizeof(int64_t));
    return XB_OK;
}
// ... 281 lines not shown
    HIPCHK(hipMemsetAsync(fs + FS_N_EDGES, 0, 7 * sizeof(int), c->stream));
    c->chg_n = -1;
    {
        ScopedTimer t(c, XB_TIMER_EDGE_FIND);
        const int small = small_grid(g);
        int *buni = nullptr;
        int ntiles_listed = 0;
        if (g.nx >= 16 && g.ny >= 16 && g.nz >= 16)
            buni = launch_brick_uniformity(c, gl, 0, ((g.nx + 7) / 8) * ((g.ny + 7) / 8) * ((g.nz + 7) / 8), 4096);
        const unsigned char *brec = (c->grad_valid && c->grad_cover == 1) || late_records ? c->brick_rec : nullptr;
        if (buni) {
            const int ntiles = ((g.nz + ET_Z - 1) / ET_Z) * ((g.ny + ET_Y - 1) / ET_Y) * ((g.nx + ET_X - 1) / ET_X);
            ntiles_listed = ntiles;
            int *tiles = (int *)c->stage;
            HIPCHK(hipMemsetAsync(c->known, 2, (size_t)c->N, c->stream));
            k_edge_tile_list<<<(ntiles + TPB - 1) / TPB, TPB, 0, c->stream>>>(gl, buni, tiles, fs + FS_N_TILES, 0, (g.nx + ET_X - 1) / ET_X,
                                                                              c->pending_assign ? fs : nullptr);
            k_edge_flag_listed<<<std::min(ntiles, 2048), TPB, 0, c->stream>>>(gl, c->rho, c->labels, c->known, c->list, fs + FS_N_EDGES, small,
                                                           c->grad_valid ? c->grad : nullptr, brec, c->has_vacuum ? 0 : 1, tiles, fs + FS_N_TILES);
        } else {
            dim3 grid((g.nz + ET_Z - 1) / ET_Z, (g.ny + ET_Y - 1) / ET_Y, (g.nx + ET_X - 1) / ET_X);
            k_edge_flag_tiled<<<grid, TPB, 0, c->stream>>>(gl, c->rho, c->labels, c->known, 0, g.nx, c->list, fs + FS_N_EDGES, small, buni,
                                                           c->grad_valid ? c->grad : nullptr, brec, c->has_vacuum ? 0 : 1);
        }
        if (buni && c->opt.tile_dilate && g.nz % ET_Z == 0) k_edge_dilate_tiles<<<std::min(ntiles_listed, 4096), TPB, 0, c->stream>>>(gl, c->known, (const int *)c->stage, fs + FS_N_TILES);
        else k_edge_dilate_list<<<nblocks(c->N / 16), TPB, 0, c->stream>>>(gl, c->known, c->list, 0, fs + FS_N_EDGES);
    }
    c->list_valid = false; c->chg_n = -1;
    c->buni_valid = false;
    if (late_records) {
        if (int rc = need_grad(c)) return rc;
        ScopedTimer t(c, XB_TIMER_MASKS_GROWTH);
        const int nb0 = (g.nx + 7) / 8, nb1 = (g.ny + 7) / 8, nb2 = (g.nz + 7) / 8, nbr = nb0 * nb1 * nb2;
        unsigned char *band = reinterpret_cast<unsigned char *>(c->blab_buf);
        HIPCHK(hipMemsetAsync(band, 0, (size_t)nbr, c->stream));
        k_flag_band_bricks<<<4096, TPB, 0, c->stream>>>(gl, c->known, (const int *)c->stage, fs + FS_N_TILES, band);
        k_rec_set_bit0<<<(nbr + 255) / 256, 256, 0, c->stream>>>(nbr, c->brick_rec, band);
        launch_brick_records(c, nullptr, nullptr, nbr, nb1, nb2);
        HIPCHK(hipGetLastError());
        c->grad_valid = true;
        c->grad_cover = 1;
        c->grad_rule = 0;
        c->regions_labels = false;
        c->blab = nullptr;
        c->table_stage = 0;
    }
    const unsigned char *brec = c->grad_cover == 1 ? c->brick_rec : nullptr;
    const int regions_ok = c->grad_cover == 1 && c->regions_labels && !c->has_vacuum ? 1 : 0;
    {
        ScopedTimer t(c, XB_TIMER_REFINE_TRACE);
        int *defer = (int *)c->stage;
        WalkerIO wl{};
        constexpr int XB_RT_BLOCK = 128;
        launch_refine_trace<2, false>(c, (unsigned)((c->N / 16 + XB_RT_BLOCK - 1) / XB_RT_BLOCK), XB_RT_BLOCK, c->list, 0, fs + FS_N_EDGES,
                                      fs + FS_CHANGED, fs + FS_ESCAPED, c->ovf_list, fs + FS_R_OVF, c->ovf_cap, brec, defer, fs + FS_R_DEFER,
                                      regions_ok, nullptr, wl);
        if (c->grad_cover == 1 && !regions_ok)
            launch_refine_trace<2, true>(c, 512, TPB, (int *)c->stage, 0, fs + FS_R_DEFER, fs + FS_CHANGED, fs + FS_ESCAPED, c->ovf_list,
                                         fs + FS_R_OVF, c->ovf_cap, c->brick_rec, nullptr, nullptr, 0, nullptr, wl);
    }
    HIPCHK(hipGetLastError());
    int *hr = c->host_ints + HI_REFINE;
    HIPCHK(hipMemcpyAsync(hr, fs + FS_N_EDGES, 7 * sizeof(int), hipMemcpyDeviceToHost, c->stream));
    HIPCHK(hipStreamSynchronize(c->stream));
    if (c->pending_assign && !assign_neargrid_complete(c, &c->pending_n_maxima)) return XB_STEP_REDO;
    *edges = hr[0];
    *changed = hr[1];
    const int novf = hr[3];
    if (novf == 0 && hr[1] > 0 && c->stage_bytes >= 8 * (size_t)c->N && hr[1] <= (int)std::min<long long>(c->N, 0x7fffffffLL)) {
        k_list_changed<<<1024, TPB, 0, c->stream>>>(c->list, fs + FS_N_EDGES, c->known, (int *)c->stage + c->N, fs + FS_N_CHGLIST,
                                                    (int)std::min<long long>(c->N, 0x7fffffffLL), fs + FS_CHANGED);
        HIPCHK(hipGetLastError());
        c->chg_n = hr[1];
    } else if (novf == 0 && hr[1] == 0)
        c->chg_n = 0;
    c->stat_deferred += hr[4];
    if (hr[2]) return fail(XB_E_STATE, "xb_refine: %d traces left the grid", hr[2]);
    if (novf > c->ovf_cap) return fail(XB_E_LIMIT, "%d retraces need the slow path (cap %d)", novf, c->ovf_cap);
    c->stat_ovf_refine += novf;
    if (novf > 0) {
        const int *slow_list = nullptr, *slow_n_dev = nullptr;
        const int n_slow = novf;
        const bool can_defer = c->grad_cover == 1 && !regions_ok;
        if (!can_defer && c->stage_bytes >= sizeof(int) * (size_t)novf) {
            int *list2 = (int *)c->stage;
            HIPCHK(hipMemsetAsync(c->counters + CT_MID_LEFT, 0, sizeof(int), c->stream));
            launch_refine_trace<XB_MID_K, false>(c, nblocks(novf), TPB, c->ovf_list, novf, nullptr, fs + FS_CHANGED, fs + FS_ESCAPED, list2,
                                                 c->counters + CT_MID_LEFT, novf, brec, nullptr, nullptr, regions_ok, nullptr, WalkerIO{});
            HIPCHK(hipGetLastError());
            slow_list = list2;
            slow_n_dev = c->counters + CT_MID_LEFT;
            if (c->opt.dbg & XB_DBG_EC_PASSES) {
                int m2 = 0;
                if (int rc = read_counter(c, CT_MID_LEFT, &m2)) return rc;
                fprintf(stderr, "[refine] %d retraces listed, %d left for the exact slow kernel after the %d-voxel window\n", novf, m2, XB_MID_K);
            }
        }
        if (int rc = run_slow(c, n_slow, 1, nullptr, fs + FS_CHANGED, fs + FS_ESCAPED, slow_list, slow_n_dev, true)) return rc;
        HIPCHK(hipMemcpyAsync(hr, fs + FS_CHANGED, sizeof(int), hipMemcpyDeviceToHost, c->stream));
        HIPCHK(hipStreamSynchronize(c->stream));
        *changed = hr[0];
    }
    return XB_OK;
}

static int refine_impl(xb_ctx *c, int mode, int64_t iters, int64_t *log, int64_t log_capacity, int64_t *n_iters);
int xb_refine(xb_ctx *c, int mode, int64_t iters, int64_t *log, int64_t log_capacity, int64_t *n_iters) {
// ... 29 lines not shown
    for (int64_t it = 2; iters < 0 || it <= iters; it++) {
        if (fused && mode != XB_REFINE_ALL && changed == 0) {
            put(0, 0);
            break;
        }
        if (fused && mode == XB_REFINE_ALL) {
            if (int rc = refine_iteration_fused(c, &edges, &changed)) return rc;
            put(edges, changed);
            if (changed == 0) break;
            continue;
        }
        if (mode == XB_REFINE_ALL) {
            if (int rc = xb_edge_find(c, &edges)) return rc;
        } else {
            if (int rc = xb_edge_check(c, &checked, &edges)) return rc;
        }
        if (int rc = xb_refine_trace(c, &changed, &esc)) return rc;
        if (esc) return fail(XB_E_STATE, "xb_refine: %lld traces left the valid slab", (long long)esc);
        put(edges, changed);
        if (changed == 0) break;
    }
    return XB_OK;
}

int xb_assign_refine(xb_ctx *c, int method, int mode, int64_t iters, int64_t *n_maxima, int64_t *log, int64_t log_capacity, int64_t *n_iters) {
    NEED_GRID_RAW("xb_assign_refine");
    c->have_labels = true;
    if (n_iters) *n_iters = 0;
    const bool fused = c->g.x0 == 0 && c->g.x1 == c->g.nx && !table_windowed(c);
    if (method == XB_METHOD_NEARGRID && fused && fused_ok(c) && !c->has_vacuum && iters != 0 && (mode == XB_REFINE_ALL || mode == XB_REFINE_CHANGED)) {
        c->labels_zero_pending = false;
        c->defer_wait = true;
        int rc = assign_neargrid_fused(c, nullptr);
        c->defer_wait = false;
        if (rc) { c->pending_assign = false; return rc; }
        rc = refine_impl(c, mode, iters, log, log_capacity, n_iters);
        c->chg_n = -1;
        const bool redo = rc == XB_STEP_REDO || c->pending_assign;
        const bool arrived = rc == XB_STEP_REDO;
        c->pending_assign = false;
        if (!redo) {
            if (n_maxima) *n_maxima = c->pending_n_maxima;
            return rc;
        }
        if (n_iters) *n_iters = 0;
        if (arrived) {
            c->grad_rule = 1;
            c->buni_valid = false; c->regions_labels = false;
            c->regions_pending = true;
            c->list_valid = false;
            if (int rc2 = assign_neargrid_tail(c, n_maxima)) return rc2;
            return xb_refine(c, mode, iters, log, log_capacity, n_iters);
        }
        c->grad_valid = false;
        c->first_clean = false;
        c->buni_valid = false; c->regions_labels = false;
        if (n_iters) *n_iters = 0;
    }
    if (int rc = xb_assign(c, method, n_maxima)) return rc;
    return xb_refine(c, mode, iters, log, log_capacity, n_iters);
}
```

pybader_amd/csrc/host_slab_table.h:

```cpp


int xb_set_table_window(xb_ctx *c, int64_t margin) {
    NEED_GRID("xb_set_table_window");
    Grid &g = c->g;
    c->grad_valid = false;
    c->table_stage = 0;
    const int own = g.x1 - g.x0;
    if (margin < 0 || own == g.nx) { g.wx0 = 0; g.wlen = g.nx; c->table_margin = -1; g.wbase = 0; return XB_OK; }
    if (g.nx % 8 || g.ny % 8 || g.nz % 8 || g.x0 % 8 || g.x1 % 8)
        return fail(XB_E_ARG, "xb_set_table_window: grid and slab must be made of whole 8^3 bricks");
    const int m8 = (int)((std::max<int64_t>(margin, c->halo) + 7) / 8) * 8;
    if (own + 2 * m8 >= g.nx) { g.wx0 = 0; g.wlen = g.nx; c->table_margin = -1; g.wbase = 0; return XB_OK; }
    g.wx0 = ((g.x0 - m8) % g.nx + g.nx) % g.nx;
    g.wlen = own + 2 * m8;
    c->table_margin = m8;
    return need_grad(c);
}
static bool slab_sparse_ok(const xb_ctx *c) {
    const Grid &g = c->g;
    return c->opt.boxes && c->opt.bricks && table_windowed(c) && g.nx % BRK == 0 && g.ny % BRK == 0 && g.nz % BRK == 0 &&
           g.x0 % BRK == 0 && g.x1 % BRK == 0 && g.ny >= 16 && g.nz >= 16 && 7LL * (c->N / (BRK * BRK * BRK)) <= c->N;
}
int xb_table_build(xb_ctx *c, int64_t *n_local_seeds) {
    NEED_GRID_RAW("xb_table_build");
    if (int rc = need_grad(c)) return rc;
    c->slab_sparse = false;
    if (slab_sparse_ok(c)) {
        Grid &g = c->g;
        const int nb1 = g.ny / BRK, nb2 = g.nz / BRK, nbr = (g.nx / BRK) * nb1 * nb2;
        if (int rc = ensure_brick_bytes(c, nbr)) return rc;
        int *fs = c->fs, *bmask = c->list + nbr, *bmaxv = c->list + 4 * nbr;
        HIPCHK(hipMemsetAsync(fs, 0, FS_TOTAL * sizeof(int), c->stream));
        g.main_ties = 1;
        {
            ScopedTimer t_growth(c, XB_TIMER_MASKS_GROWTH);
            ScopedTimer t_masks(c, XB_TIMER_BRICK_MASKS);
            launch_brick_masks(c, false, false, bmask, bmaxv, nullptr);
        }
        HIPCHK(hipGetLastError());
        int ties = 0;
        HIPCHK(hipMemcpyAsync(c->host_ints, fs + FS_TIES, sizeof(int), hipMemcpyDeviceToHost, c->stream));
        HIPCHK(hipStreamSynchronize(c->stream));
        ties = c->host_ints[0];
        c->window_ties = ties != 0;
        c->window_seeds.clear();
        c->grad_valid = true;
        c->grad_cover = 1;
        c->grad_rule = 1;
        c->blab = nullptr;
        c->n_boxes = 0; c->box_voxels = 0;
        c->table_stage = 1;
        c->slab_sparse = true;
        if (n_local_seeds) *n_local_seeds = 0;
        return XB_OK;
    }
    if (int rc = ensure_grad(c, true, true, true)) return rc;
    if (n_local_seeds) *n_local_seeds = table_windowed(c) ? (int64_t)c->window_seeds.size() : 0;
    return XB_OK;
// ... 119 lines not shown
```

pybader_amd/csrc/host_stages.h:

```cpp

enum { BB_TOTAL = 1 << 20, BB_REGMAX = 1 << 16, BB_REGFIRST = 1 << 17 };

static bool table_windowed(const xb_ctx *c) { return c->g.wlen < c->g.nx; }
static int small_grid(const Grid &g) { return g.nx < 16 || g.ny < 16 || g.nz < 80; }
static int trace_maxsteps(const Grid &g) { return 8 * (g.nx + g.ny + g.nz) + 64; }
static const int *slab_regions_of(const xb_ctx *c) {
    const Grid &g = c->g;
    return (table_windowed(c) && c->blab && c->regions_labels && !c->has_vacuum && (c->grad_rule == 2 || c->slab_sparse) &&
            g.nx % 8 == 0 && g.ny % 8 == 0 && g.nz % 8 == 0) ? c->blab : nullptr;
}

static_assert(CT_REDO == CT_N_MAX + 15, "a host-driven assignment zeroes CT_N_MAX .. CT_REDO at once");
static int begin_assignment(xb_ctx *c, int *counts, int n, bool invalidate) {
    HIPCHK(hipMemsetAsync(counts, 0, n * sizeof(int), c->stream));
    if (!c->first_clean) {
        k_fill<int><<<4096, TPB, 0, c->stream>>>(c->first, XB_INT_MAX, c->N);
        HIPCHK(hipGetLastError());
    }
    c->first_clean = false;
    c->regions_pending = false;
    if (invalidate) {
        c->buni_valid = false; c->regions_labels = false;
        c->list_valid = false; c->chg_n = -1;
    }
    return XB_OK;
}

static void launch_brick_masks(xb_ctx *c, bool part, bool allow_diag, int *bmask, int *bmaxv, int *bpot) {
    const Grid &g = c->g;
    const dim3 grid((g.nz + GT_Z - 1) / GT_Z, (g.ny + GT_Y - 1) / GT_Y, (g.x1 - g.x0 + GT_X - 1) / GT_X);
    GridS gs;
    const bool sym = sym_grid(g, gs);
    int mirror = 0;
    double mu_scale = 0.;
    if (sym && c->opt.mirror) mirror_prefilter(g, mirror, mu_scale);
    const bool diag = allow_diag && c->opt.mask_diag && g.T[1] == 0. && g.T[2] == 0. && g.T[3] == 0. && g.T[5] == 0. && g.T[6] == 0. && g.T[7] == 0.;
    auto launch = [&](auto kernel, const auto &gt) {
        kernel<<<grid, TPB, 0, c->stream>>>(gt, c->rho, small_grid(g), bmask, bmaxv, c->fs + FS_TIES, g.x0, mu_scale, mirror, bpot);
    };
    if (!sym) launch(part ? k_brick_masks<Grid, 1, false, true> : k_brick_masks<Grid, 1, false>, g);
    else if (part) launch(diag ? k_brick_masks<GridS, 1, true, true> : k_brick_masks<GridS, 1, false, true>, gs);
    else launch(diag ? k_brick_masks<GridS, 1, true> : k_brick_masks<GridS, 1, false>, gs);
}

static void launch_brick_records(xb_ctx *c, const int *list, const int *n_dev, int nbr, int nb1, int nb2) {
    const Grid &g = c->g;
    auto launch = [&](auto kernel, const auto &gt) {
        kernel<<<4096, TPB, 0, c->stream>>>(gt, c->rho, c->grad, list, n_dev, nbr, nb1, nb2, c->brick_rec, small_grid(g));
    };
    GridS gs;
    if (sym_grid(g, gs)) launch(k_brick_records<GridS>, gs);
    else launch(k_brick_records<Grid>, g);
}

static void launch_region_growth(xb_ctx *c, int nb0, int nb1, int nb2, int *bmask, int *bmaxv, int *bpot, int *seed, int *buf0,
                                 int *buf1, int *box_max, int *box_first, bool chase) {
    const int nbr = nb0 * nb1 * nb2;
    int *fs = c->fs;
    k_seed_bricks<<<(nbr + 255) / 256, 256, 0, c->stream>>>(nbr, bmask, bmaxv, fs, seed, buf0, box_max, box_first);
    if (chase) {
        k_grow_parent<<<(nbr + TPB - 1) / TPB, TPB, 0, c->stream>>>(nb0, nb1, nb2, bmask, bpot, seed, buf1);
        k_grow_chase<<<(nbr + TPB - 1) / TPB, TPB, 0, c->stream>>>(nbr, buf1, seed, buf0, 4 * (nb0 + nb1 + nb2) + 64, fs);
    } else
        k_seed_finish<<<1, 1, 0, c->stream>>>(fs);
    const int long_schedule = 2 * ((std::max(std::max(nb0, nb1), nb2) + BG - 1) / BG) + 12;
    const int launches = chase ? std::min(long_schedule, c->grow_kill_launches) : long_schedule;
    const dim3 ggrid((nb2 + BG - 1) / BG, (nb1 + BG - 1) / BG, (nb0 + BG - 1) / BG);
    for (int l = 0; l < launches; l++)
        k_brick_grow_dev<<<ggrid, BG * BG * BG, 0, c->stream>>>(nb0, nb1, nb2, bmask, seed, buf0, buf1, fs, BG, 0);
    k_grow_finish<<<64, TPB, 0, c->stream>>>(nbr, seed, buf0, buf1, fs, c->blab_buf, box_first, bmask, c->brick_rec, 0, chase && launches < long_schedule ? 1 : 0);
}

static void launch_window_bricks(xb_ctx *c, int *list, int *count, const int *skip) {
    const Grid &g = c->g;
    const int nb0 = c->nbk[0], per_plane = c->nbk[1] * c->nbk[2], nbr = nb0 * per_plane;
    const int w0 = g.wx0 / BRK, wn = g.wlen / BRK, run1 = std::min(wn, nb0 - w0);
    const unsigned grid = (nbr + 16 * TPB - 1) / (16 * TPB);
    k_brick_walk_list<<<grid, TPB, 0, c->stream>>>(nbr, w0 * per_plane, (w0 + run1) * per_plane, c->blab, list, count, skip);
    if (wn > run1) k_brick_walk_list<<<grid, TPB, 0, c->stream>>>(nbr, 0, (wn - run1) * per_plane, c->blab, list, count, skip);
}

static bool launch_persistent_trace(xb_ctx *c, bool lean_ok, bool part, const int *box_max, const int *walk, int has_vacuum, int *bres) {
    const Grid &g = c->g;
    const int groups = std::max(1, c->trace_waves / XB_TRACE_WAVES);
    const int lean = lean_ok && light(g).use24 && c->opt.lean ? ((long long)g.wlen * g.nyz <= (1LL << 27) ? 4 : 3) : 0;
    const bool window = table_windowed(c);
    int *ovf = window ? (int *)c->stage : c->ovf_list;
    const int ovf_cap = window ? (int)std::min<size_t>(c->stage_bytes / sizeof(int), 0x7fffffffu) : c->ovf_cap;
    auto kernel = !lean ? k_ng_trace_g<2, 0>
                : window ? (lean == 4 ? k_ng_trace_g<2, 4, true> : k_ng_trace_g<2, 3, true>)
                : part ? (lean == 4 ? k_ng_trace_g<2, 4, false, true> : k_ng_trace_g<2, 3, false, true>)
                : (lean == 4 ? k_ng_trace_g<2, 4> : k_ng_trace_g<2, 3>);
    kernel<<<groups, XB_WAVE * XB_TRACE_WAVES, 0, c->stream>>>(light(g), c->grad, box_max, c->blab, c->nbk[1], c->nbk[2], walk, c->fs, c->labels,
                                                               c->first, c->max_list, c->max_cap, ovf, ovf_cap, trace_maxsteps(g), has_vacuum,
                                                               8, 1, lean ? bres : nullptr);
    if (window)
        k_ng_trace_list<2><<<512, TPB, 0, c->stream>>>(light(g), c->grad, box_max, c->blab, c->nbk[1], c->nbk[2], ovf, c->fs + FS_N_OVF, c->labels,
                                                       c->first, c->max_list, c->fs + FS_N_MAX, c->max_cap, c->ovf_list, c->counters + CT_N_OVF,
                                                       c->ovf_cap, trace_maxsteps(g), c->rho, c->dist_dev, has_vacuum);
    return lean != 0;
}

enum { BUNI_NONE, BUNI_SCAN, BUNI_MIXED };
static void launch_relabel(xb_ctx *c, int *fs, int n_maxima, bool regions, const int *box_max, int buni, const int *bres) {
    const Grid &g = c->g;
    const GridL gl = light(g);
    const int nb1 = c->nbk[1], nb2 = c->nbk[2], nbr = c->nbk[0] * nb1 * nb2;
    const int *gate = fs ? fs + FS_SORT_OK : nullptr, *n_walk_dev = fs ? fs + FS_N_WALK : nullptr;
    int *ubuf = reinterpret_cast<int *>(c->st);
    if (regions) {
        const int v = g.nz % 4 == 0 ? 4 : 1;
        (v == 4 ? k_relabel_regions_brick<4> : k_relabel_regions_brick<1>)<<<dim3((g.nz / v + 63) / 64, nb1, (g.x1 - g.x0 + 3) / 4), TPB, 0, c->stream>>>(
            gl, c->labels, c->first, c->blab, nb1, nb2, box_max, fs, gate, fs ? -1 : c->n_boxes);
        if (buni == BUNI_MIXED) k_fill<int><<<(nbr + 4 * TPB - 1) / (4 * TPB), TPB, 0, c->stream>>>(ubuf, XB_MIXED, nbr);
        if (buni != BUNI_NONE && bres)
            k_buni_after_relabel<<<(nbr + 255) / 256, 256, 0, c->stream>>>(nbr, c->blab, box_max, c->first, ubuf, gate, c->walk, n_walk_dev, bres);
        else if (buni != BUNI_NONE) {
            k_buni_after_relabel<<<(nbr + 255) / 256, 256, 0, c->stream>>>(nbr, c->blab, box_max, c->first, ubuf, gate, nullptr, nullptr, nullptr);
            if (fs) k_label_uniform_list<<<2048, TPB, 0, c->stream>>>(gl, c->labels, nb1, nb2, c->walk, 0, n_walk_dev, gate, ubuf);
            else if (c->n_walk)
                k_label_uniform_list<<<(c->n_walk + 3) / 4, TPB, 0, c->stream>>>(gl, c->labels, nb1, nb2, c->walk, c->n_walk, nullptr, nullptr, ubuf);
        }
    } else
        k_relabel<<<nblocks((long long)(g.x1 - g.x0) * g.nyz), TPB, 0, c->stream>>>(g, c->labels, c->first, gate);
    if (fs) k_reset_first<<<8, 256, 0, c->stream>>>(c->first, c->max_aux, 0, fs + FS_N_MAX, gate);
    else if (n_maxima) k_reset_first<<<(unsigned)((n_maxima + 255) / 256), 256, 0, c->stream>>>(c->first, c->max_aux, n_maxima, nullptr, nullptr);
}

static void numbering_done(xb_ctx *c, const int *sorted, int nmax, int64_t *n_maxima) {
    if (sorted) c->maxima_sorted.assign(sorted, sorted + nmax);
    c->label_wire = label_wire_for(nmax);
    c->regions_pending = false;
    c->first_clean = true;
    if (n_maxima) *n_maxima = nmax;
}

extern "C++" template <int K, bool RHO, bool RESUME = false, bool EXPORT = false>
static void launch_refine_trace(xb_ctx *c, unsigned grid, int block, const int *list, int n_host, const int *n_dev, int *changed, int *escaped,
                                int *ovf_list, int *ovf_count, int ovf_cap, const unsigned char *brec, int *defer_list, int *defer_count,
                                int regions_ok, const int *region_blab, const WalkerIO &wio) {
    k_refine_trace<K, RHO, RESUME, EXPORT><<<grid, block, 0, c->stream>>>(light(c->g), c->grad, c->labels, c->known, list, n_host, n_dev, changed,
                                                                           escaped, ovf_list, ovf_count, ovf_cap, trace_maxsteps(c->g), c->rho,
                                                                           c->dist_dev, brec, defer_list, defer_count, regions_ok, region_blab, wio);
}
```

pybader_amd/csrc/k_edges.h:

```cpp
#pragma once

__device__ __forceinline__ void classify27(const Grid &g, const double *__restrict__ rho,
                                           const int *__restrict__ labels, int x, int y, int z, int v,
                                           bool &is_edge, bool &is_max) {
    const int vol_num = labels[v];
    is_edge = false;
    is_max = true;
    int nb[27];
    int k = 0;
#pragma unroll
    for (int ix = -1; ix < 2; ix++) {
        const int tx = wrapi(x + ix, g.nx);
#pragma unroll
        for (int iy = -1; iy < 2; iy++) {
            const int ty = wrapi(y + iy, g.ny);
#pragma unroll
            for (int iz = -1; iz < 2; iz++) {
                const int tz = wrapi(z + iz, g.nz);
                const int l = lin3(g, tx, ty, tz);
                const int nv = labels[l];
                nb[k++] = (nv == -1) ? -1 : l;
                if (nv != -1 && nv != vol_num) is_edge = true;
            }
        }
// ... 479 lines not shown
    for (int c = 0; c < CK_CHUNKS; c++)
#pragma unroll
        for (int k = 0; k < 16; k++)
            if (b[c][k] == value) list[w++] = (int)(base[c] + k);
}

__global__ __launch_bounds__(TPB) void k_edge_dilate(Grid g, int8_t *known, int xa, int nplanes, int flag) {
    const long long vv = (long long)blockIdx.x * TPB + threadIdx.x;
    if (vv >= (long long)nplanes * g.nyz) return;
    const int xr = (int)(vv / g.nyz);
    const int r = (int)(vv - (long long)xr * g.nyz);
    int x = xa + xr;
    if (x >= g.nx) x -= g.nx;
    const int y = r / g.nz, z = r - y * g.nz;
    const int v = lin3(g, x, y, z);
    if (known[v] < 0) return;
    bool near = false;
#pragma unroll
    for (int ix = -1; ix < 2; ix++) {
        const int tx = wrapi(x + ix, g.nx);
#pragma unroll
        for (int iy = -1; iy < 2; iy++) {
            const int ty = wrapi(y + iy, g.ny);
#pragma unroll
            for (int iz = -1; iz < 2; iz++) {
                const int tz = wrapi(z + iz, g.nz);
                near |= (known[lin3(g, tx, ty, tz)] == flag);
            }
        }
    }
    if (near) known[v] = -1;
}

struct Walker {
    int v, vol_num;
    int lp, lq;
    double dr0, dr1, dr2;
    int widx[2];
    double wval[2];
    double m_old;
    int steps, og_move;
};
struct WalkerIO {
    const Walker *in;
    Walker *out;
    int *out_count;
    int out_cap;
    int *res;
    int *res_count;
    int own0, own1;
};
#define XB_WALKER_STUCK (-2147483647 - 1)

template <int K, bool RHO, bool RESUME = false, bool EXPORT = false>
__global__ __launch_bounds__(TPB) void k_refine_trace(GridL g, const GradRec *__restrict__ G, int *labels,
                                                      int8_t *known, const int *__restrict__ list, int n_host,
                                                      const int *n_dev, int *changed, int *escaped, int *ovf_list,
                                                      int *ovf_count, int ovf_cap, int maxsteps,
                                                      const double *__restrict__ rho, const double *__restrict__ gc,
                                                      const unsigned char *__restrict__ brick_rec, int *defer_list,
                                                      int *defer_count, int regions_ok, const int *__restrict__ region_blab,
                                                      WalkerIO wio) {
    static_assert(!RESUME || (RHO && K == 2), "walkers are carried on by the from-rho kernel");
    const int n = n_dev ? *n_dev : n_host;
    int n_ch = 0, n_es = 0;
  const XcdRange xr = xcd_range((n + (int)blockDim.x - 1) / (int)blockDim.x);
  for (int chunk = xr.begin; chunk < xr.end; chunk += xr.step) {
    const int t = chunk * (int)blockDim.x + threadIdx.x;
    bool valid = t < n;
    int v = (valid && !RESUME) ? list[t] : 0;
    bool moving = false;
    int result = -3;
    int px = 0, py = 0, pz = 0, lp = 0, steps = 0, vol_num = 0;
    double dr0 = 0., dr1 = 0., dr2 = 0.;
    GradRec rec = {0., 0., 0., 0.};
    PathWindow<K> w;
    w.init(0, 0.);
    bool arrive = false, og_in = false;
    int lq_in = 0;
    if (RESUME) {
        if (valid) {
            const Walker wk = wio.in[t];
            const int qx = wk.lq / g.nyz;
            valid = qx >= wio.own0 && qx < wio.own1;
            if (valid) {
                v = wk.v; vol_num = wk.vol_num; lp = wk.lp; lq_in = wk.lq;
                px = lp / g.nyz;
                const int r = lp - px * g.nyz;
                py = r / g.nz;
                pz = r - py * g.nz;
                dr0 = wk.dr0; dr1 = wk.dr1; dr2 = wk.dr2;
                w.idx[0] = wk.widx[0]; w.idx[K - 1] = wk.widx[1];
                w.val[0] = wk.wval[0]; w.val[K - 1] = wk.wval[1];
                w.m_old = wk.m_old;
                steps = wk.steps; og_in = wk.og_move != 0;
                arrive = true; moving = true;
            }
        }
    } else
    if (valid) {
        px = v / g.nyz;
        const int r = v - px * g.nyz;
        py = r / g.nz;
        pz = r - py * g.nz;
        lp = v;
        rec = fetch_rec_w(g, G, v);
        vol_num = labels[v];
        moving = true;
        if (region_blab && region_blab[((px >> 3) * ((g.ny + 7) >> 3) + (py >> 3)) * ((g.nz + 7) >> 3) + (pz >> 3)] > 0) {
            result = v; moving = false;
        } else
        if (!(plane_in_window(g, px) && rec_exists(brick_rec, g, px, py, pz))) {
            if (RHO) rec = make_rec_rho(g, rho, gc, px, py, pz);
            else { result = regions_ok ? v : -5; moving = false; }
        }
        w.init(v, rec.key);
    }
#ifdef XB_DEBUG_COUNT
    int dbg_it = 0;
#endif
    while (__any(moving)) {
        if (moving) {
#ifdef XB_DEBUG_COUNT
            dbg_it++;
#endif
            int qx = 0, qy = 0, qz = 0, lq = 0;
            bool og_move = false;
            if (RESUME && arrive) {
                arrive = false;
                lq = lq_in; og_move = og_in;
                qx = lq / g.nyz;
                const int r = lq - qx * g.nyz;
                qy = r / g.nz;
                qz = r - qy * g.nz;
            } else {
            const int bits = key_bits(rec.key);
            const int code = bits & 63;
            og_move = (code == XB_STAY_CODE);
            if (!og_move) {
                ng_move_t(g, px, py, pz, rec, code, dr0, dr1, dr2, qx, qy, qz);
                lq = lin3f(g, qx, qy, qz);
                og_move = w.contains(lq);
            }
            if (og_move) {
                const int og = (bits >> 6) & 31;
                if (og == XB_OG_SELF) { result = lp; moving = false; }
                else {
                    int ox, oy, oz;
                    og_offsets(og, ox, oy, oz);
                    dr0 = dr1 = dr2 = 0.;
                    qx = wrap_u(px + ox, g.nx); qy = wrap_u(py + oy, g.ny); qz = wrap_u(pz + oz, g.nz);
                    lq = lin3f(g, qx, qy, qz);
                }
            }
            }
            if (moving) {
                const bool in_win = plane_in_window(g, qx);
                const bool ok_plane = plane_valid(g, qx);
                GradRec nr = fetch_rec(G, in_win ? rec_slot(g, lq) : 0);
                const int8_t kq = known[ok_plane ? lq : lp];
                const bool missing = !(in_win && rec_exists(brick_rec, g, qx, qy, qz));
                const bool in_region = region_blab && ok_plane && region_blab[((qx >> 3) * ((g.ny + 7) >> 3) + (qy >> 3)) * ((g.nz + 7) >> 3) + (qz >> 3)] > 0;
                if (in_region || (!RHO && regions_ok && in_win && missing && ok_plane)) {
                    result = lq;
                    moving = false;
                } else {
                    if (missing && ok_plane) {
                        if (RHO) nr = make_rec_rho(g, rho, gc, qx, qy, qz);
                        else nr.key = key_floor(rho[lq]);
                    }
                    if (!ok_plane) {
                        result = (RHO || EXPORT || !defer_list) ? -4 : -5;
                        moving = false;
                        if ((RHO || EXPORT) && K == 2 && wio.out) {
                            const int k = atomicAdd(wio.out_count, 1);
                            if (k < wio.out_cap) {
                                Walker wk;
                                wk.v = v; wk.vol_num = vol_num; wk.lp = lp; wk.lq = lq;
                                wk.dr0 = dr0; wk.dr1 = dr1; wk.dr2 = dr2;
                                wk.widx[0] = w.idx[0]; wk.widx[1] = w.idx[K - 1];
                                wk.wval[0] = w.val[0]; wk.wval[1] = w.val[K - 1];
                                wk.m_old = w.m_old; wk.steps = steps; wk.og_move = og_move ? 1 : 0;
                                wio.out[k] = wk;
                            }
                        }
                    }
                    else if ((!og_move && nr.key <= w.m_old) || ++steps > maxsteps) { result = -2; moving = false; }
                    else if (kq == 2) { result = lq; moving = false; }
                    else if (!RHO && missing) { result = -5; moving = false; }
                    else {
                        w.push(lq, nr.key);
                        px = qx; py = qy; pz = qz; lp = lq; rec = nr;
                    }
                }
            }
        }
    }
#ifdef XB_DEBUG_COUNT
    if (xb_dbg_steps && valid && !RESUME) xb_dbg_steps[v] = (signed char)min(dbg_it + 1, 127);
#endif
    int ch = 0, es = 0;
    if (RESUME) {
        if (valid) {
            if (result == -4) es = 1;
            else {
                const int k = atomicAdd(wio.res_count, 1);
                wio.res[2 * k] = v;
                wio.res[2 * k + 1] = result >= 0 ? labels[result] : XB_WALKER_STUCK;
            }
        }
    } else
    if (valid) {
        if (result >= 0) {
            const int nv = labels[result];
// ... 551 lines not shown
```

pybader_amd/csrc/k_masks.h:

```cpp
#pragma once

#define GT_X 8
#define GT_Y 8
#define GT_Z 32

#define BRK 8
#define BG 8

__device__ __forceinline__ int wrap_any(int v, int n) { v %= n; return v < 0 ? v + n : v; }

__global__ void k_flag_window_bricks(int nb0, int per_plane, int b0, int nb, unsigned char flag, unsigned char *brick_rec) {
    const int b = blockIdx.x * blockDim.x + threadIdx.x;
    if (b >= nb0 * per_plane) return;
    int d = b / per_plane - b0;
    if (d < 0) d += nb0;
    brick_rec[b] = d < nb ? flag : (unsigned char)0;
}


#define BM_EPS 2e-12
#ifdef XB_DEBUG_COUNT
__device__ unsigned long long xb_dbg[65536];
__device__ signed char *xb_dbg_steps;
#endif
// ... 257 lines not shown
    const double kInf = __builtin_huge_val();
    BmCoef co;
    co.yl = ty == 0 ? BM_EPS : (ty == 1 ? -(1. - BM_EPS) : -kInf);
    co.yh = at_yh ? -BM_EPS : (ty == wy - 2 ? (1. - BM_EPS) : kInf);
    co.zl = zz == 0 ? BM_EPS : (zz == 1 ? -(1. - BM_EPS) : -kInf);
    co.zh = at_zh ? -BM_EPS : (zz == wz - 2 ? (1. - BM_EPS) : kInf);
    const int y = y0 + ty, z = z0 + tz;
    const bool col_in = y < g.ny && z < g.nz;
    const double dface = fmin(fmin(fmin(dist_at(g, 0, 1, 1), dist_at(g, 2, 1, 1)), fmin(dist_at(g, 1, 0, 1), dist_at(g, 1, 2, 1))),
                              fmin(dist_at(g, 1, 1, 0), dist_at(g, 1, 1, 2)));
    double a[3][3][3];
#pragma unroll
    for (int iy = 0; iy < 3; iy++)
#pragma unroll
        for (int iz = 0; iz < 3; iz++) {
            a[1][iy][iz] = tile[0][ty + iy][tz + iz];
            a[2][iy][iz] = tile[1][ty + iy][tz + iz];
        }
    int mine = 0;
    bool any_tie = false;
    double cmax = -1.7976931348623157e308;
#define BM_STEP(K)                                                                                                   \
    {                                                                                                                \
        _Pragma("unroll") for (int iy = 0; iy < 3; iy++) _Pragma("unroll") for (int iz = 0; iz < 3; iz++) {          \
            a[0][iy][iz] = a[1][iy][iz];                                                                             \
            a[1][iy][iz] = a[2][iy][iz];                                                                             \
            a[2][iy][iz] = tile[K + 2][ty + iy][tz + iz];                                                            \
        }                                                                                                            \
        const int x = x0 + K;                                                                                        \
        if (!PART || x < g.nx) cmax = max_raw(cmax, a[1][1][1]);    \
        bm_voxel<MT, K, DIAG, PART>(g, a, dface, col_in && x < g.nx, (x * g.ny + y) * g.nz + z, ty, zz, mine, any_tie, \
                                    &s_cnt[tz >> 3], &s_mv[tz >> 3], mu, mirror, co, deep, wx, at_yh, at_zh);          \
    }
    BM_STEP(0) BM_STEP(1) BM_STEP(2) BM_STEP(3) BM_STEP(4) BM_STEP(5) BM_STEP(6) BM_STEP(7)
#undef BM_STEP
    static_assert(GT_X == 8, "eight x-positions per column");
    if (__any(any_tie) && threadIdx.x % XB_WAVE == 0) atomicAdd(tie_count, 1);
    atomicOr(&s_mask[tz >> 3], mine);
    if (bpot && col_in) {
        const int fi = __float_as_int((float)cmax);
        atomicMax(&s_pot[tz >> 3], fi >= 0 ? fi : fi ^ 0x7fffffff);
    }
    __syncthreads();
    if (threadIdx.x < GT_Z / 8 && z0 + threadIdx.x * 8 < g.nz) {
        const int nb1 = (g.ny + 7) >> 3, nb2 = (g.nz + 7) >> 3;
        if (bpot) bpot[((x0 >> 3) * nb1 + (y0 >> 3)) * nb2 + (z0 >> 3) + threadIdx.x] = s_pot[threadIdx.x];
        const int b = ((x0 >> 3) * nb1 + (y0 >> 3)) * nb2 + (z0 >> 3) + threadIdx.x, n = s_cnt[threadIdx.x];
        const bool dead = PART && (g.nx - x0 == 1 || g.ny - y0 == 1 || g.nz - (z0 + 8 * (int)threadIdx.x) == 1);
        bmask[b] = (s_mask[threadIdx.x] & 0x7ffdfff) | ((n >= 1 || dead) ? 1 << 27 : 0) | ((n >= 2 || dead) ? 1 << 28 : 0);
        bmaxv[b] = (n == 1 && !dead) ? s_mv[threadIdx.x] : -1;
    }
}

#define BR_ROW 24
template <typename GT>
__global__ __launch_bounds__(TPB, 4) void k_brick_records(GT g, const double *__restrict__ rho, GradRec *__restrict__ G,
                                                       const int *__restrict__ walk, const int *n_list, int nbr, int nb1, int nb2,
                                                       unsigned char *brick_rec, int small) {
    __shared__ double tile[10][10][BR_ROW];
    const int n = walk ? *n_list : nbr;
    int goff[4], loff[4];
#pragma unroll
    for (int j = 0; j < 4; j++) {
        const int e = threadIdx.x + j * TPB;
        const int ex = e / 100, ey = (e / 10) % 10, ez = e % 10;
        goff[j] = (ex * g.ny + ey) * g.nz + ez;
        loff[j] = (ex * 10 + ey) * BR_ROW + ez;
    }
    const XcdRange xr = xcd_range(n);
    for (int item = xr.begin; item < xr.end; item += xr.step) {
        const int b = walk ? walk[item] : item;
        if (!walk && !(brick_rec[b] & 1)) continue;
        const int b0 = b / (nb1 * nb2), b1 = (b / nb2) % nb1, b2 = b % nb2;
        const int x0 = b0 * 8, y0 = b1 * 8, z0 = b2 * 8;
        const bool inner = !(small & 1) && x0 >= 1 && x0 + 8 < g.nx && y0 >= 1 && y0 + 8 < g.ny && z0 >= 1 && z0 + 8 < g.nz;
        __syncthreads();
        {
            double val[4];
            if (inner) {
                const double *corner = rho + ((size_t)(x0 - 1) * g.ny + (y0 - 1)) * g.nz + (z0 - 1);
#pragma unroll
                for (int j = 0; j < 4; j++) val[j] = (threadIdx.x + j * TPB < 1000) ? corner[goff[j]] : 0.;
            } else {
#pragma unroll
                for (int j = 0; j < 4; j++) {
                    const int e = threadIdx.x + j * TPB;
                    const int ex = e / 100, ey = (e / 10) % 10, ez = e % 10;
                    int X = x0 + ex - 1, Y = y0 + ey - 1, Z = z0 + ez - 1;
                    if (small & 1) {
                        X = ((X % g.nx) + g.nx) % g.nx; Y = ((Y % g.ny) + g.ny) % g.ny; Z = ((Z % g.nz) + g.nz) % g.nz;
                    } else {
                        X = wrap_u(X, g.nx); Y = wrap_u(Y, g.ny); Z = wrap_u(Z, g.nz);
                    }
                    val[j] = e < 1000 ? rho[(X * g.ny + Y) * g.nz + Z] : 0.;
                }
            }
#pragma unroll
            for (int j = 0; j < 4; j++)
                if (threadIdx.x + j * TPB < 1000) (&tile[0][0][0])[loff[j]] = val[j];
        }
        __syncthreads();
        const int vbase = (x0 * g.ny + y0) * g.nz + z0;
#pragma unroll 1
        for (int j = 0; j < 2; j++) {
            const int l = threadIdx.x + j * TPB;
            const int tx = l >> 6, ty = (l >> 3) & 7, tz = l & 7;
            const double c = tile[tx + 1][ty + 1][tz + 1];
            double max_val = c;
            int og = XB_OG_SELF;
#pragma unroll
            for (int ix = 0; ix < 3; ix++) {
#pragma unroll
                for (int iy = 0; iy < 3; iy++)
#pragma unroll
                    for (int iz = 0; iz < 3; iz++) {
                        double w = tile[tx + ix][ty + iy][tz + iz];
                        w = (w - c) * dist_at(g, ix, iy, iz);
                        w += c;
                        og = (w > max_val) ? ix * 9 + iy * 3 + iz : og;
                        max_val = fmax(max_val, w);
                    }
            }
            GradRec o;
            double d0, d1, d2;
            int code;
            if (ng_dir_vals(g, c, tile[tx + 2][ty + 1][tz + 1], tile[tx][ty + 1][tz + 1], tile[tx + 1][ty + 2][tz + 1],
                            tile[tx + 1][ty][tz + 1], tile[tx + 1][ty + 1][tz + 2], tile[tx + 1][ty + 1][tz], d0, d1, d2)) {
                o.r0 = o.r1 = o.r2 = 0.;
                code = XB_STAY_CODE;
            } else {
                const int i0 = rha_cs(d0), i1 = rha_cs(d1), i2 = rha_cs(d2);
                o.r0 = d0 - (double)i0;
                o.r1 = d1 - (double)i1;
                o.r2 = d2 - (double)i2;
                code = (i0 + 1) | ((i1 + 1) << 2) | ((i2 + 1) << 4);
            }
            o.key = pack_key(c, code, og);
            if (inner || (x0 + tx < g.nx && y0 + ty < g.ny && z0 + tz < g.nz)) G[rec_slot(g, vbase + (tx * g.ny + ty) * g.nz + tz)] = o;
        }
        if (threadIdx.x == 0) brick_rec[b] |= 1;
    }
}

#define XB_MIXED_LABEL (-2147483647 - 1)
__global__ void k_flag_mixed_bricks(int nbr, const int *__restrict__ buni3, unsigned char *brick_rec) {
    const int b = blockIdx.x * blockDim.x + threadIdx.x;
    if (b < nbr) brick_rec[b] = (unsigned char)(2 | (buni3[b] == XB_MIXED_LABEL ? 1 : 0));
}
__global__ void k_rec_set_bit0(int nbr, unsigned char *brick_rec, const unsigned char *__restrict__ flag) {
    const int b = blockIdx.x * blockDim.x + threadIdx.x;
    if (b < nbr) brick_rec[b] = (unsigned char)((brick_rec[b] & 2) | (flag[b] ? 1 : 0));
}
__global__ __launch_bounds__(TPB) void k_flag_band_bricks(GridL g, const int8_t *__restrict__ known, const int *__restrict__ tiles, const int *n_tiles,
                                                          unsigned char *flag) {
    const int ntz = (g.nz + 63) / 64, nty = (g.ny + 7) / 8, n = *n_tiles;
    const int nb0 = (g.nx + 7) >> 3, nb1 = (g.ny + 7) >> 3, nb2 = (g.nz + 7) >> 3;
    for (int item = blockIdx.x; item < n; item += gridDim.x) {
        const int t = (int)((unsigned)tiles[item] & 0x7fffffffu);
        const int x = (t / (ntz * nty)) * 4 + threadIdx.x / 64, y = ((t / ntz) % nty) * 8 + (threadIdx.x / 8) % 8, z = (t % ntz) * 64 + 8 * (threadIdx.x % 8);
        if (x >= g.nx || y >= g.ny || z >= g.nz) continue;
        const int8_t *row = known + ((size_t)x * g.ny + y) * g.nz;
        bool any = false, lo = false, hi = false;
        if (g.nz % 8 == 0) {
            const unsigned long long w = *reinterpret_cast<const unsigned long long *>(row + z);
            any = w != 0x0202020202020202ull; lo = (w & 0xffull) != 2; hi = (w >> 56) != 2;
        } else
            for (int k = 0; k < 8 && z + k < g.nz; k++) {
                const bool bnd = row[z + k] != 2;
                any |= bnd;
                if (k == 0) lo = bnd;
                if (k == 7 || z + k == g.nz - 1) hi = bnd;
            }
        if (!any) continue;
        const int bx = x >> 3, by = y >> 3, bz = z >> 3;
        const bool mx = (x & 7) == 0, px = (x & 7) == 7 || x == g.nx - 1, my = (y & 7) == 0, py = (y & 7) == 7 || y == g.ny - 1;
        for (int ax = -1; ax < 2; ax++) {
            if ((ax < 0 && !mx) || (ax > 0 && !px)) continue;
            for (int ay = -1; ay < 2; ay++) {
                if ((ay < 0 && !my) || (ay > 0 && !py)) continue;
                for (int az = -1; az < 2; az++) {
                    if ((az < 0 && !lo) || (az > 0 && !hi)) continue;
                    flag[(wrapi(bx + ax, nb0) * nb1 + wrapi(by + ay, nb1)) * nb2 + wrapi(bz + az, nb2)] = 1;
                }
            }
        }
    }
}
__device__ __forceinline__ bool rec_exists(const unsigned char *__restrict__ brick_rec, const GridL &g, int x, int y, int z) {
    return !brick_rec || (brick_rec[((x >> 3) * ((g.ny + 7) >> 3) + (y >> 3)) * ((g.nz + 7) >> 3) + (z >> 3)] & 1) != 0;
}
// ... 1 lines not shown
```

pybader_amd/csrc/k_trace.h:

```cpp
#pragma once

__global__ __launch_bounds__(TPB) void k_fill_certain(GridL g, const int *__restrict__ blab, int nb1, int nb2,
                                                      const int *__restrict__ box_max, int *labels, int *first,
                                                      int *max_list, int *max_count, int max_cap, const int *skip = nullptr) {
    if (skip && *skip) return;
    const int vbeg = g.x0 * g.nyz, vend = g.x1 * g.nyz;
    const int v = vbeg + blockIdx.x * TPB + threadIdx.x;
    const bool in = v < vend;
    int result = -1;
    bool has = false;
    if (in) {
        const int x = v / g.nyz;
        const int r = v - x * g.nyz;
        const int y = r / g.nz, z = r - y * g.nz;
        const int b = blab[((x >> 3) * nb1 + (y >> 3)) * nb2 + (z >> 3)];
        if (b > 0 && labels[v] != -1) {
            result = box_max[b - 1];
            if (result != v && labels[result] == -1) result = -1;
            labels[v] = result;
            has = result >= 0;
        }
    }
    note_maximum_wave(has, result, in ? v : 0, first, max_list, max_count, max_cap);
}
// ... 31 lines not shown
#pragma unroll
        for (int k = 0; k < V; k++) v.l[k] = l;
#pragma unroll
        for (int r = 0; r < 8; r++)
            if (r < rows) p[(size_t)r * stride] = v;
    } else {
        Vec m[8];
#pragma unroll
        for (int r = 0; r < 8; r++) {
            if (r < rows) m[r] = p[(size_t)r * stride];
            else
#pragma unroll
                for (int k = 0; k < V; k++) m[r].l[k] = -1;
        }
#pragma unroll
        for (int r = 0; r < 8; r++)
#pragma unroll
            for (int k = 0; k < V; k++)
                if (m[r].l[k] >= 0) m[r].l[k] = rank[m[r].l[k]];
#pragma unroll
        for (int r = 0; r < 8; r++)
            if (r < rows) p[(size_t)r * stride] = m[r];
    }
}
__global__ __launch_bounds__(TPB) void k_brick_walk_list(int nbr, int b_lo, int b_hi, const int *__restrict__ blab,
                                                         int *walk, int *n_walk, const int *skip = nullptr) {
    if (skip && *skip) return;
    const int base = (blockIdx.x * TPB + threadIdx.x) * 16;
    unsigned int hits = 0;
#pragma unroll
    for (int k = 0; k < 16; k++) {
        const int b = base + k;
        if (b < nbr && b >= b_lo && b < b_hi && blab[b] <= 0) hits |= 1u << k;
    }
    int total;
    const int off = block_scan_excl(__popc(hits), total);
    __shared__ int base_s;
    if (threadIdx.x == 0) base_s = total ? atomicAdd(n_walk, total) : 0;
    __syncthreads();
    int w = base_s + off;
#pragma unroll
    for (int k = 0; k < 16; k++)
        if ((hits >> k) & 1u) walk[w++] = base + k;
}

__device__ __forceinline__ int compact3(unsigned x) {
    x &= 0x09249249u;
    x = (x ^ (x >> 2)) & 0x030c30c3u;
    x = (x ^ (x >> 4)) & 0x0300f00fu;
    x = (x ^ (x >> 8)) & 0xff0000ffu;
    x = (x ^ (x >> 16)) & 0x000003ffu;
    return (int)x;
}
#define XB_NOREC (-2147483647 - 1)
__device__ __forceinline__ bool brick_is_vacuum(const int *__restrict__ bpot, int b, double vac_tol) {
    if (!bpot) return false;
    const int p = bpot[b];
    const double f = (double)__int_as_float(p >= 0 ? p : p ^ 0x7fffffff);
    return f + fabs(f) * 1e-6 < vac_tol;
}
__global__ __launch_bounds__(TPB) void k_brick_walk_list_morton(int nb0, int nb1, int nb2, unsigned n_codes,
                                                                int *blab, int *walk, int *n_walk, const int *skip,
                                                                const int *__restrict__ bpot = nullptr, double vac_tol = 0.) {
    if (skip && *skip) return;
    const unsigned base = (blockIdx.x * TPB + threadIdx.x) * 16u;
    unsigned int hits = 0;
    int bidx[16];
#pragma unroll
    for (int k = 0; k < 16; k++) {
        const unsigned code = base + k;
        const int b2 = compact3(code), b1 = compact3(code >> 1), b0 = compact3(code >> 2);
        const bool in = code < n_codes && b0 < nb0 && b1 < nb1 && b2 < nb2;
        bidx[k] = in ? (b0 * nb1 + b1) * nb2 + b2 : 0;
        if (in && blab[bidx[k]] <= 0) {
            if (brick_is_vacuum(bpot, bidx[k], vac_tol)) blab[bidx[k]] = XB_NOREC;
            else hits |= 1u << k;
        }
    }
    int total;
    const int off = block_scan_excl(__popc(hits), total);
    __shared__ int base_s;
    if (threadIdx.x == 0) base_s = total ? atomicAdd(n_walk, total) : 0;
    __syncthreads();
    int w = base_s + off;
#pragma unroll
    for (int k = 0; k < 16; k++)
        if ((hits >> k) & 1u) walk[w++] = bidx[k];
}

__device__ __forceinline__ void og_offsets(int og, int &ox, int &oy, int &oz) {
    ox = og / 9 - 1; oy = (og / 3) % 3 - 1; oz = og % 3 - 1;
}

template <int K, bool WIN>
__device__ __forceinline__ void ng_walk_wave(const GridL &g, const GradRec *__restrict__ G, const int *__restrict__ box_max,
                                             const int *__restrict__ blab, int nb1, int nb2, bool in_walk, int sx, int sy, int sz,
                                             int *labels, int *first, int *max_list, int *max_count, int max_cap,
                                             int *ovf_list, int *ovf_count, int ovf_cap, int maxsteps,
                                             const double *__restrict__ rho, const double *__restrict__ gc,
                                             bool has_vacuum = true) {
    const bool valid = sx < g.x1 && sy < g.ny && sz < g.nz;
    const int v = valid ? (sx * g.ny + sy) * g.nz + sz : 0;
    bool moving = false;
    int result = -1;
    int px = 0, py = 0, pz = 0, lp = 0, steps = 0;
    double dr0 = 0., dr1 = 0., dr2 = 0.;
    GradRec rec = {0., 0., 0., 0.};
    PathWindow<K> w;
    w.init(0, 0.);
    if (valid) {
        const int lab0 = has_vacuum ? labels[v] : 0;
        int b = (blab && !in_walk) ? blab[((sx >> 3) * nb1 + (sy >> 3)) * nb2 + (sz >> 3)] : 0;
        rec = fetch_rec_w(g, G, v);
        if (lab0 != -1) {
            px = sx; py = sy; pz = sz;
            lp = v;
            if (b <= 0) b = key_box(rec.key);
            if (b > 0) result = box_max[b - 1];
            else { w.init(v, rec.key); moving = true; }
        }
    }
    while (__any(moving)) {
        if (moving) {
            const int bits = key_bits(rec.key);
            const int code = bits & 63;
            int qx, qy, qz, lq = 0;
            bool og_move = (code == XB_STAY_CODE);
            if (!og_move) {
                ng_move_t(g, px, py, pz, rec, code, dr0, dr1, dr2, qx, qy, qz);
                lq = lin3f(g, qx, qy, qz);
                og_move = w.contains(lq);
            }
            if (og_move) {
                const int og = (bits >> 6) & 31;
                if (og == XB_OG_SELF) { result = lp; moving = false; }
                else {
                    int ox, oy, oz;
                    og_offsets(og, ox, oy, oz);
                    dr0 = dr1 = dr2 = 0.;
                    qx = wrap_u(px + ox, g.nx); qy = wrap_u(py + oy, g.ny); qz = wrap_u(pz + oz, g.nz);
                    lq = lin3f(g, qx, qy, qz);
                }
            }
            if (moving) {
                const bool in_win = plane_in_window(g, qx);
                GradRec nr = fetch_rec(G, in_win ? rec_slot(g, lq) : 0);
                const int bl = blab ? blab[((qx >> 3) * nb1 + (qy >> 3)) * nb2 + (qz >> 3)] : 0;
                if (WIN && !in_win && bl <= 0) nr = make_rec_rho(g, rho, gc, qx, qy, qz);
                const int b = bl > 0 ? bl : key_box(nr.key);
                if (bl == XB_NOREC) {
                    result = -2;
                    moving = false;
                } else if (b) {
                    result = box_max[b - 1];
                    moving = false;
                } else if ((!WIN && !in_win) || (!og_move && nr.key <= w.m_old) || ++steps > maxsteps) {
                    result = -2;
                    moving = false;
                } else {
                    w.push(lq, nr.key);
                    px = qx; py = qy; pz = qz; lp = lq; rec = nr;
                }
            }
        }
    }
    if (has_vacuum && valid && result >= 0 && result != v && labels[result] == -1) result = -1;
    if (valid) labels[v] = result;
    note_maximum_wave(valid && result >= 0, result, v, first, max_list, max_count, max_cap);
    if (valid && result == -2) {
        const int k = atomicAdd(ovf_count, 1);
        if (k < ovf_cap) ovf_list[k] = v;
    }
}
__device__ __forceinline__ int wrap3(int q, int n) {
    return (int)min(min((unsigned)q, (unsigned)(q + n)), (unsigned)(q - n));
}
__device__ __forceinline__ int mad24(int a, int b, int c) {
    int r;
    asm("v_mad_u32_u24 %0, %1, %2, %3" : "=v"(r) : "v"(a), "s"(b), "v"(c));
    return r;
}
__device__ __forceinline__ int lin24(const GridL &g, int x, int y, int z) { return mad24(mad24(x, g.ny, y), g.nz, z); }
template <bool OFF32>
__device__ __forceinline__ GradRec fetch_rec_o(const GradRec *__restrict__ G, int l) {
    if (OFF32) return *reinterpret_cast<const GradRec *>(reinterpret_cast<const char *>(G) + ((unsigned)l << 5));
    return fetch_rec(G, l);
}
constexpr int XB_TRACE_WAVES = 4;
__shared__ GradRec xb_s_rec[512];
template <bool OFF32, bool CACHE, bool WINDOW = false>
__device__ __forceinline__ int ng_walk_lean(const GridL &g, const GradRec *__restrict__ G, const int *__restrict__ box_max,
                                             const int *__restrict__ blab, int nb1, int nb2, int sx, int sy, int sz,
                                             int *labels, int *first, int *max_list, int *max_count, int max_cap,
                                             int *ovf_list, int *ovf_count, int ovf_cap, int maxsteps, bool has_vacuum) {
    const int v = lin24(g, sx, sy, sz);
    const int lab0 = has_vacuum ? labels[v] : 0;
    const int ox8 = sx & ~7, oy8 = sy & ~7, oz8 = sz & ~7;
    GradRec rec = CACHE ? xb_s_rec[((sx & 7) << 6) | ((sy & 7) << 3) | (sz & 7)] : fetch_rec_o<OFF32>(G, WINDOW ? rec_slot(g, v) : v);
    int result = -1;
    int px = sx, py = sy, pz = sz, steps = 0;
    double dr0 = 0., dr1 = 0., dr2 = 0.;
    int i0 = v, i1 = -1;
    double k0 = rec.key, k1 = -1.7976931348623157e308, m_old = -1.7976931348623157e308;
#ifdef XB_DEBUG_COUNT
    int dbg_lane_steps = 0;
#endif
    if (lab0 != -1) for (;;) {
        const int bits = key_bits(rec.key);
        const double t0 = dr0 + rec.r0, t1 = dr1 + rec.r1, t2 = dr2 + rec.r2;
        const int id0 = rha_cs(t0), id1 = rha_cs(t1), id2 = rha_cs(t2);
        const int m0 = (bits & 3) + id0 - 1, m1 = ((bits >> 2) & 3) + id1 - 1, m2 = ((bits >> 4) & 3) + id2 - 1;
        px += m0; py += m1; pz += m2;
        dr0 = t0 - (double)id0; dr1 = t1 - (double)id1; dr2 = t2 - (double)id2;
        if (__builtin_amdgcn_ballot_w64((unsigned)px >= (unsigned)g.nx || (unsigned)py >= (unsigned)g.ny || (unsigned)pz >= (unsigned)g.nz) != 0) {
            px = wrap3(px, g.nx); py = wrap3(py, g.ny); pz = wrap3(pz, g.nz);
        }
        int lq = lin24(g, px, py, pz);
        const bool og_move = (bits & 63) == XB_STAY_CODE || lq == i0 || lq == i1;
        bool at_max = false;
        if (__builtin_amdgcn_ballot_w64(og_move) != 0) {
            if (og_move) {
                const int og = (bits >> 6) & 31;
                int ox, oy, oz;
                og_offsets(og, ox, oy, oz);
                at_max = og == XB_OG_SELF;
                dr0 = dr1 = dr2 = 0.;
                px = wrap3(wrap3(px - m0, g.nx) + ox, g.nx);
                py = wrap3(wrap3(py - m1, g.ny) + oy, g.ny);
                pz = wrap3(wrap3(pz - m2, g.nz) + oz, g.nz);
                lq = lin24(g, px, py, pz);
            }
        }
        int bl = 0;
        const bool own = CACHE && (unsigned)((px ^ ox8) | (py ^ oy8) | (pz ^ oz8)) < 8u;
        const bool in_win = !WINDOW || own || plane_in_window(g, px);
        if (own) rec = xb_s_rec[((px & 7) << 6) | ((py & 7) << 3) | (pz & 7)];
        else {
            rec = fetch_rec_o<OFF32>(G, WINDOW ? (in_win ? rec_slot(g, lq) : 0) : lq);
            const unsigned bidx = (unsigned)mad24(mad24(px >> 3, nb1, py >> 3), nb2, pz >> 3);
            bl = *reinterpret_cast<const int *>(reinterpret_cast<const char *>(blab) + (bidx << 2));
        }
        steps++;
#ifdef XB_DEBUG_COUNT
        dbg_lane_steps++;
#endif
        const bool arrived = bl > 0 && !at_max;
        const bool undecided = (!og_move && rec.key <= m_old) || steps > maxsteps || (WINDOW && !in_win) || bl == XB_NOREC;
        if (arrived) result = box_max[bl - 1];
        else if (at_max) result = i0;
        else if (undecided) result = -2;
        if (arrived || at_max || undecided) break;
        m_old = max_raw(m_old, k1);
        i1 = i0; k1 = k0;
        i0 = lq; k0 = rec.key;
    }
#ifdef XB_DEBUG_COUNT
    if (xb_dbg_steps) xb_dbg_steps[v] = (signed char)min(dbg_lane_steps, 127);
#endif
    if (has_vacuum && result >= 0 && result != v && labels[result] == -1) result = -1;
    labels[v] = result;
    note_maximum_wave(result >= 0, result, v, first, max_list, max_count, max_cap);
    if (result == -2) {
        const int k = atomicAdd(ovf_count, 1);
        if (k < ovf_cap) ovf_list[k] = v;
    }
    return result;
}
__device__ __forceinline__ void brick_sub_voxel(int b, int sub, int lane, int nb1, int nb2, int &sx, int &sy, int &sz) {
    const int b0 = b / (nb1 * nb2), b1 = (b / nb2) % nb1, b2 = b % nb2;
    sx = b0 * 8 + ((sub >> 2) << 2) + (lane >> 4);
    sy = b1 * 8 + ((sub & 3) << 1) + ((lane >> 3) & 1);
    sz = b2 * 8 + (lane & 7);
}
template <int K, bool WIN>
__global__ __launch_bounds__(TPB) void k_ng_trace(GridL g, const GradRec *__restrict__ G,
                                                  const int *__restrict__ box_max, const int *__restrict__ blab,
                                                  int nb1, int nb2, const int *__restrict__ walk, int n_walk,
                                                  int *labels, int *first,
                                                  int *max_list, int *max_count, int max_cap, int *ovf_list,
                                                  int *ovf_count, int ovf_cap, int maxsteps, int opt,
                                                  const double *__restrict__ rho, const double *__restrict__ gc, int has_vacuum) {
    int blk = blockIdx.x;
    if (opt & 2) {
        const int per = gridDim.x >> 3;
        if (blk < (per << 3)) blk = (blk & 7) * per + (blk >> 3);
    }
    const int wpb = blockDim.x / XB_WAVE;
    const int wave = blk * wpb + threadIdx.x / XB_WAVE;
    const int lane = threadIdx.x % XB_WAVE;
    int sx, sy, sz;
    if (walk) {
        if ((wave >> 3) >= n_walk) return;
        brick_sub_voxel(walk[wave >> 3], wave & 7, lane, nb1, nb2, sx, sy, sz);
        if (sx < g.x0 || sx >= g.x1) return;
    } else if (opt & 1) {
        const int bz_n = (g.nz + 3) >> 2, by_n = (g.ny + 3) >> 2;
        const int bx = wave / (by_n * bz_n);
        const int brem = wave - bx * (by_n * bz_n);
        const int by = brem / bz_n, bz = brem - by * bz_n;
        sx = g.x0 + bx * 4 + (lane >> 4); sy = by * 4 + ((lane >> 2) & 3); sz = bz * 4 + (lane & 3);
    } else {
        const int rz_n = (g.nz + 63) >> 6;
        const int row = wave / rz_n;
        sz = (wave - row * rz_n) * 64 + lane;
        sx = g.x0 + row / g.ny;
        sy = row - (row / g.ny) * g.ny;
    }
    ng_walk_wave<K, WIN>(g, G, box_max, blab, nb1, nb2, walk != nullptr, sx, sy, sz, labels, first, max_list, max_count,
                         max_cap, ovf_list, ovf_count, ovf_cap, maxsteps, rho, gc, has_vacuum != 0);
}
template <int K>
__global__ __launch_bounds__(TPB) void k_ng_trace_list(GridL g, const GradRec *__restrict__ G, const int *__restrict__ box_max,
                                                       const int *__restrict__ blab, int nb1, int nb2,
                                                       const int *__restrict__ vox, const int *n_dev, int *labels, int *first,
                                                       int *max_list, int *max_count, int max_cap, int *ovf_list,
                                                       int *ovf_count, int ovf_cap, int maxsteps,
                                                       const double *__restrict__ rho, const double *__restrict__ gc, int has_vacuum) {
    const int n = *n_dev;
    for (int base = blockIdx.x * TPB; base < n; base += gridDim.x * TPB) {
        const int t = base + threadIdx.x;
        int sx = g.x1, sy = 0, sz = 0;
        if (t < n) {
            const int v = vox[t];
            sx = v / g.nyz;
            const int r = v - sx * g.nyz;
            sy = r / g.nz;
            sz = r - sy * g.nz;
        }
        ng_walk_wave<K, true>(g, G, box_max, blab, nb1, nb2, true, sx, sy, sz, labels, first, max_list, max_count, max_cap,
                              ovf_list, ovf_count, ovf_cap, maxsteps, rho, gc, has_vacuum != 0);
    }
}
__device__ __forceinline__ int xcc_id() {
    int x;
    asm volatile("s_getreg_b32 %0, hwreg(HW_REG_XCC_ID)" : "=s"(x));
    return x & 7;
}

template <int K, int LEAN, bool WINDOW = false, bool PART = false>
__global__ __launch_bounds__(XB_WAVE * XB_TRACE_WAVES, 8) void k_ng_trace_g(GridL g, const GradRec *__restrict__ G, const int *__restrict__ box_max,
                                                       const int *__restrict__ blab, int nb1, int nb2,
                                                       const int *__restrict__ walk, int *fs, int *labels, int *first,
                                                       int *max_list, int max_cap, int *ovf_list, int ovf_cap, int maxsteps,
                                                       int has_vacuum, int CH, int xcd_split, int *__restrict__ bres = nullptr) {
    __shared__ int s_base, s_next;
    __shared__ int s_w[8], s_mixed;
    constexpr bool CACHE = LEAN >= 3;
    int prev_brick = -1;
#ifdef XB_DEBUG_COUNT
    const long long pr_t0 = clock64();
    long long pr_walk = 0, pr_wait = 0, pr_load = 0;
    int pr_bricks = 0;
    const unsigned long long pr_e0 = wall_clock64();
#endif
    const int n_items = fs[FS_N_WALK] * 8;
    const int per = (((n_items + 7) >> 3) + 7) & ~7;
    const int home = xcd_split ? xcc_id() : (blockIdx.x & 7);
    const int lane = threadIdx.x & (XB_WAVE - 1);
    auto verdict = [&]() {
        if (CACHE && bres && prev_brick >= 0) {
            int r0 = s_mixed ? -1 : s_w[0];
#pragma unroll
            for (int k = 1; k < 8; k++) r0 = (s_w[k] == r0) ? r0 : -1;
            bres[prev_brick] = r0 >= 0 ? r0 : (-2147483647 - 1);
        }
        prev_brick = -1;
    };
    for (int r = 0; r < 8; r++) {
        const int q = (home + r) & 7;
        const int beg = q * per, end = min(beg + per, n_items);
        for (;;) {
#ifdef XB_DEBUG_COUNT
            const long long pr_a = clock64();
#endif
            __syncthreads();
#ifdef XB_DEBUG_COUNT
            pr_wait += clock64() - pr_a;
#endif
            if (threadIdx.x == 0) {
                verdict();
                s_mixed = 0;
                s_base = beg + atomicAdd(&fs[FS_CURSOR0 + q * FS_CURSOR_STRIDE], CH);
                s_next = 0;
            }
            __syncthreads();
            const int base = s_base;
            if (base >= end) break;
            const int stop = min(base + CH, end);
#ifdef XB_DEBUG_COUNT
            const long long pr_b = clock64();
            pr_bricks++;
#endif
            if (CACHE) {
                constexpr int PER = 512 / (XB_WAVE * XB_TRACE_WAVES);
                const int b = walk[base >> 3];
                prev_brick = b;
                const int b0 = b / (nb1 * nb2), b1 = (b / nb2) % nb1, b2 = b % nb2;
                GradRec tmp[PER];
#pragma unroll
                for (int k = 0; k < PER; k++) {
                    const int t = threadIdx.x + k * XB_WAVE * XB_TRACE_WAVES;
                    int cx = b0 * 8 + (t >> 6), cy = b1 * 8 + ((t >> 3) & 7), cz = b2 * 8 + (t & 7);
                    if (PART) { cx = min(cx, g.nx - 1); cy = min(cy, g.ny - 1); cz = min(cz, g.nz - 1); }
                    const int lt = lin24(g, cx, cy, cz);
                    tmp[k] = fetch_rec(G, WINDOW ? rec_slot(g, lt) : lt);
                }
#pragma unroll
                for (int k = 0; k < PER; k++) xb_s_rec[threadIdx.x + k * XB_WAVE * XB_TRACE_WAVES] = tmp[k];
                __syncthreads();
            }
#ifdef XB_DEBUG_COUNT
            pr_load += clock64() - pr_b;
#endif
            for (;;) {
                int i = 0;
                if (lane == 0) i = atomicAdd(&s_next, 1);
                const int item = base + __builtin_amdgcn_readfirstlane(i);
                if (item >= stop) break;
                int sx, sy, sz;
                brick_sub_voxel(walk[item >> 3], item & 7, lane, nb1, nb2, sx, sy, sz);
                if (PART) { sx = min(sx, g.nx - 1); sy = min(sy, g.ny - 1); sz = min(sz, g.nz - 1); }
                if (LEAN) {
#ifdef XB_DEBUG_COUNT
                    const long long pr_c = clock64();
#endif
                    const int res = ng_walk_lean<LEAN == 4, CACHE, WINDOW>(g, G, box_max, blab, nb1, nb2, sx, sy, sz, labels, first, max_list, &fs[FS_N_MAX],
                                                                max_cap, ovf_list, &fs[FS_N_OVF], ovf_cap, maxsteps, has_vacuum != 0);
#ifdef XB_DEBUG_COUNT
                    pr_walk += clock64() - pr_c;
#endif
                    if (CACHE && bres) {
                        volatile int *w = s_w;
                        if (lane == 0) w[item - base] = res;
                        if (w[item - base] != res) *(volatile int *)&s_mixed = 1;
                    }
                }
                else
                    ng_walk_wave<K, false>(g, G, box_max, blab, nb1, nb2, true, sx, sy, sz, labels, first, max_list, &fs[FS_N_MAX],
                                           max_cap, ovf_list, &fs[FS_N_OVF], ovf_cap, maxsteps, nullptr, nullptr, has_vacuum != 0);
            }
        }
    }
#ifdef XB_DEBUG_COUNT
    if (lane == 0 && blockIdx.x < 2048) {
        unsigned long long *o = xb_dbg + 64 + 6 * (blockIdx.x * XB_TRACE_WAVES + (threadIdx.x >> 6));
        o[0] = (unsigned long long)pr_walk; o[1] = (unsigned long long)(clock64() - pr_t0); o[2] = (unsigned long long)pr_wait;
        o[3] = (unsigned long long)pr_load; o[4] = pr_e0; o[5] = (unsigned long long)wall_clock64();
        if (threadIdx.x == 0) xb_dbg[64 + 6 * 8192 + blockIdx.x] = (unsigned long long)pr_bricks;
    }
#endif
    if (CACHE && bres) {
        __syncthreads();
        if (threadIdx.x == 0) verdict();
    }
}

__global__ __launch_bounds__(TPB) void k_list_unfinished(GridL g, const int *__restrict__ walk, const int *n_walk, int nb1, int nb2,
                                                         const int *__restrict__ labels, int *out, int *out_count, int out_cap) {
    __shared__ int s_buf[BlockAppender<2>::CAP], s_n[2];
    BlockAppender<2> app;
    app.init(s_buf, s_n, out, out_count, out_cap);
    const int n = *n_walk;
    for (int e = blockIdx.x; e < n; e += gridDim.x) {
        const int b = walk[e];
        const int b0 = b / (nb1 * nb2), b1 = (b / nb2) % nb1, b2 = b % nb2;
        int v[2];
        int cnt = 0;
#pragma unroll
        for (int k = 0; k < 2; k++) {
            const int t = threadIdx.x + k * TPB;
            const int x = b0 * 8 + (t >> 6), y = b1 * 8 + ((t >> 3) & 7), z = b2 * 8 + (t & 7);
            if (x < g.nx && y < g.ny && z < g.nz) {
                const int l = (x * g.ny + y) * g.nz + z;
                if (labels[l] == -2) v[cnt++] = l;
            }
        }
        app.add(cnt, [&](int k) { return v[k]; });
    }
    app.finish();
// ... 88 lines not shown
```

pybader_amd/csrc/slab_step.h:

```cpp

#define XB_TAB_ROWS 1024
#define XB_TAB_INTS (2 + 2 * XB_TAB_ROWS)
#define XB_SLAB_RANKS_MAX 64
#define XB_XCNT XB_XC_COUNT
__host__ __device__ __forceinline__ size_t walk_part(int cap) { return 16 + (size_t)cap * (sizeof(Walker) + 8); }
static inline int walk_cap_for(const Grid &g) { return (int)std::min<long long>(std::max<long long>(32768, (long long)g.nyz / 8), 1 << 20); }

__global__ void k_slab_flag(const int *fs, int *flags, int rank) { flags[rank] = fs[FS_TIES] != 0; }
__global__ void k_slab_any_flag(const int *flags, int nranks, int *fs) {
    int any = 0;
    for (int r = 0; r < nranks; r++) any |= flags[r];
    fs[FS_TIES] = any;
}
__global__ void k_slab_pack_table(int *tab, const int *__restrict__ max_list, const int *__restrict__ first, int *fs,
                                  const int *slow_count) {
    const int n = fs[FS_N_MAX];
    const bool bad = n > XB_TAB_ROWS || *slow_count > 0 || fs[FS_GROW_RETRY];
    if (threadIdx.x == 0) { tab[0] = bad ? -1 : n; tab[1] = 0; fs[FS_N_REDO] = fs[FS_N_OVF]; fs[FS_N_OVF] = *slow_count; }
    if (bad) return;
    for (int i = threadIdx.x; i < n; i += blockDim.x) {
        const int m = max_list[i];
        tab[2 + 2 * i] = m;
        tab[3 + 2 * i] = first[m];
    }
// ... 234 lines not shown
    {
        ScopedTimer t_growth(c, XB_TIMER_MASKS_GROWTH);
        k_slab_any_flag<<<1, 1, 0, c->stream>>>(slab_flags(c), c->slab_nranks, fs);
        launch_region_growth(c, nb0, nb1, nb2, bmask, bmaxv, bpot, seed, buf0, buf1, box_max, box_first, true);
        HIPCHK(hipGetLastError());
    }
    c->blab = c->blab_buf;
    c->walk = walk;
    c->nbk[0] = nb0; c->nbk[1] = nb1; c->nbk[2] = nb2;
    {
        ScopedTimer t_assign(c, XB_TIMER_ASSIGN);
        const int per_plane = nb1 * nb2;
        launch_window_bricks(c, reclist, fs + FS_N_RECL, fs + FS_GROW_RETRY);
        k_brick_walk_list<<<(nbr + 16 * TPB - 1) / (16 * TPB), TPB, 0, c->stream>>>(nbr, (g.x0 / BRK) * per_plane, (g.x1 / BRK) * per_plane, c->blab, walk, fs + FS_N_WALK, fs + FS_GROW_RETRY);
        {
            ScopedTimer t_records(c, XB_TIMER_BRICK_RECORDS);
            launch_brick_records(c, reclist, fs + FS_N_RECL, nbr, nb1, nb2);
        }
        k_note_certain_bricks<<<(nbr + 255) / 256, 256, 0, c->stream>>>(gl, nb0, nb1, nb2, (g.x0 / BRK) * per_plane, (g.x1 / BRK) * per_plane, c->blab,
                                                                      box_max, c->first, c->max_list, fs + FS_N_MAX, c->max_cap, fs + FS_GROW_RETRY);
        c->regions_pending = true;
        {
            ScopedTimer t_trace(c, XB_TIMER_TRACE);
            launch_persistent_trace(c, true, false, box_max, walk, 0, nullptr);
        }
        k_slab_pack_table<<<1, 256, 0, c->stream>>>(slab_tables(c) + (size_t)c->slab_rank * XB_TAB_INTS, c->max_list, c->first, fs, c->counters + CT_N_OVF);
    }
    HIPCHK(hipGetLastError());
    g.main_ties = 0;
    c->slab_stage = 2;
    return XB_OK;
}

int xb_slab_assign_finish(xb_ctx *c, int64_t *n_maxima, int64_t *status) {
    NEED_GRID_RAW("xb_slab_assign_finish");
    if (c->slab_stage != 2) return fail(XB_E_STATE, "xb_slab_assign_finish: call xb_slab_assign_trace first");
    c->slab_stage = 0;
    int *fs = c->fs;
    const int *tabs = slab_tables(c);
    k_slab_merge_min<<<c->slab_nranks, 256, 0, c->stream>>>(tabs, c->first);
    k_slab_merge_list<<<1, 1024, 0, c->stream>>>(tabs, c->slab_nranks, c->max_list, c->max_cap, fs);
    k_number_maxima<<<1, 1024, 0, c->stream>>>(fs, c->first, c->max_list, c->max_cap, c->max_aux);
    launch_relabel(c, fs, 0, true, c->boxbuf + BB_REGMAX, BUNI_MIXED, nullptr);
    HIPCHK(hipGetLastError());
    HIPCHK(hipMemcpyAsync(c->host_ints, fs, FS_COUNT * sizeof(int), hipMemcpyDeviceToHost, c->stream));
    HIPCHK(hipMemcpyAsync(c->host_ints + FS_COUNT, c->max_aux, XB_SORT_MAX * sizeof(int), hipMemcpyDeviceToHost, c->stream));
    HIPCHK(hipStreamSynchronize(c->stream));
    const int *h = c->host_ints;
    if (n_maxima) *n_maxima = 0;
    c->regions_pending = false;
    if (h[FS_GROW_RETRY]) {
        c->grow_kill_launches = 1 << 20;
        c->stat_grow_retries++;
        c->grad_valid = false;
        if (status) *status = 1;
        return XB_OK;
    }
    if (!h[FS_SORT_OK]) {
        c->grad_valid = false;
        if (status) *status = 2;
        return XB_OK;
    }
    c->grad_rule = h[FS_TIES] ? 1 : 2;
    c->window_ties = h[FS_TIES] != 0;
    c->n_boxes = h[FS_N_BOXES];
    c->box_voxels = (long long)h[FS_N_CERTAIN] * BRK * BRK * BRK;
    c->n_walk = h[FS_N_WALK];
    if (c->opt.dbg & XB_DBG_SLAB_STATS)
        fprintf(stderr, "[slab %d] bricks traced %d, with records %d, trajectories redone beyond the table window %d, regions %d\n", c->slab_rank,
                h[FS_N_WALK], h[FS_N_RECL], h[FS_N_REDO], h[FS_N_BOXES]);
    numbering_done(c, h + FS_COUNT, h[FS_N_MAX], n_maxima);
    c->buni_valid = true;
    c->buni_halo_safe = true;
    c->regions_labels = true;
    c->table_stage = 2;
    if (status) *status = 0;
    return XB_OK;
}

int xb_slab_refine_pass(xb_ctx *c) {
    NEED_GRID("xb_slab_refine_pass");
    if (int rc = slab_need_xbuf(c)) return rc;
    const Grid &g = c->g;
    if (g.vlen >= g.nx) return fail(XB_E_STATE, "xb_slab_refine_pass: not a slab");
    if (c->slab_nranks < 2) return fail(XB_E_STATE, "xb_slab_refine_pass: call xb_slab_assign_masks first");
    if (int rc = slab_need_wbuf(c)) return rc;
    if (int rc = ensure_grad(c, false, false, false)) return rc;
    bool dilate_owned = false;
    if (int rc = edge_find_launch(c, &dilate_owned)) return rc;
    const GridL gl = light(g);
    if (dilate_owned) {
        ScopedTimer t(c, XB_TIMER_EDGE_FIND);
        k_edge_dilate_list<<<2048, TPB, 0, c->stream>>>(gl, c->known, c->list, 0, c->counters + CT_N_EDGES);
    }
    c->g.main_ties = 0;
    c->list_valid = false; c->chg_n = -1;
    c->buni_valid = false;
    c->walk_n_out = 0; c->walk_n_res = 0; c->walk_out_dev = nullptr;
    c->walk_host.clear(); c->res_host.clear();
    static_assert(CT_OG_MOVED == CT_N_MAX + 4 && CT_N_EDGES == CT_OG_MOVED + 1 && CT_HALO_EDGES == CT_N_EDGES + 1 && CT_TILES_HALO == CT_HALO_EDGES + 17, "two memsets either side of CT_N_EDGES");
    HIPCHK(hipMemsetAsync(c->counters + CT_N_MAX, 0, CT_INTS(CT_N_MAX, CT_OG_MOVED) * sizeof(int), c->stream));
    HIPCHK(hipMemsetAsync(c->counters + CT_HALO_EDGES, 0, CT_INTS(CT_HALO_EDGES, CT_TILES_HALO) * sizeof(int), c->stream));
    {
        ScopedTimer t(c, XB_TIMER_REFINE_TRACE);
        const unsigned char *brec = c->grad_cover == 1 ? c->brick_rec : nullptr;
        const int regions_ok = brec && c->regions_labels && !c->has_vacuum ? 1 : 0;
        const int *slab_regions = slab_regions_of(c);
        int *defer = (int *)c->stage;
        char *part = (char *)c->wbuf[0] + (size_t)c->slab_rank * walk_part(c->wcap);
        HIPCHK(hipMemsetAsync(part, 0, 16, c->stream));
        WalkerIO wio{};
        wio.out = (Walker *)(part + 16); wio.out_count = (int *)part;
// ... 111 lines not shown
```

Before: 42220 Mvoxels/s.

## Encode per-brick neighbour no-record bits in gradient keys to skip brick-label lookups

Replaces the old box index in the low key bits with seven neighbour bits, one per combination of crossed axes. A per-brick neighbour table written when gradient records are built supplies these bits. The lean walker then detects a step into a brick without records straight from the current key, instead of loading the brick label array on every off-brick step. It reads the label only once, at the exit. This adds a per-brick 64-bit table and extra bit arithmetic per step, and enables a specialised refine-trace path that only applies to the whole-grid, non-slab case.

```diff
diff --git a/include/bader_hip.h b/include/bader_hip.h
--- a/include/bader_hip.h
+++ b/include/bader_hip.h
@@ -199,6 +199,7 @@
     XB_CHECK_NO_EC_SHARE = 32,
     XB_CHECK_IO_GATHER = 64
 };
+#define XB_CHECK_BRICK_LOOKUP 128
 enum {
     XB_DBG_EC_PASSES = 4,
     XB_DBG_SLAB_STATS = 16,
diff --git a/pybader_amd/_lib.py b/pybader_amd/_lib.py
--- a/pybader_amd/_lib.py
+++ b/pybader_amd/_lib.py
@@ -19,6 +19,7 @@
 XB_OPT_CROSS_CHECK = 2
 (XB_CHECK_NO_MIRROR, XB_CHECK_GENERIC_WALKER, XB_CHECK_FULL_TGRAD, XB_CHECK_LIST_DILATE, XB_CHECK_WIDE_HALO,
  XB_CHECK_NO_EC_SHARE, XB_CHECK_IO_GATHER) = (1, 2, 4, 8, 16, 32, 64)
+CROSS_CHECK_BRICK_LOOKUP = 128
 XB_OPT_DEBUG = 3
 XB_DBG_EC_PASSES, XB_DBG_SLAB_STATS, XB_DBG_STAGE_WAIT, XB_DBG_SHORT_TIERS = 4, 16, 32, 64
 XB_OPT_EC_GROUPS = 4
diff --git a/pybader_amd/csrc/bader_hip.hip b/pybader_amd/csrc/bader_hip.hip
--- a/pybader_amd/csrc/bader_hip.hip
+++ b/pybader_amd/csrc/bader_hip.hip
@@ -82,6 +82,7 @@
         int tile_dilate = 1;
         int narrow_halo = 1;
         int ec_share = 1;
+        int nb_bits = 1;
         int io_tiled = 1;
         int dbg = 0;
         int ec_groups = 256;
@@ -124,9 +125,11 @@
     int *blab = nullptr;
     int nbk[3] = {0, 0, 0};
     bool grad_valid = false;
+    bool grad_nb = false;
     bool brick_max_valid = false;
     int grad_cover = 0;
     unsigned char *brick_rec = nullptr;
+    unsigned long long *nb_tab = nullptr;
     void *xbuf = nullptr;
     int slab_rank = 0, slab_nranks = 0, slab_stage = 0;
     void *wbuf[2] = {nullptr, nullptr};
@@ -315,6 +318,7 @@
     switch (key) {
     case XB_OPT_REGIONS: c->opt.boxes = (value & XB_REGIONS_BOXES) != 0; c->opt.bricks = (value & XB_REGIONS_BRICKS) != 0; break;
     case XB_OPT_CROSS_CHECK:
+        if (!(ok = value >= 0 && value < 2 * XB_CHECK_BRICK_LOOKUP)) break;
         c->opt.mirror = !(value & XB_CHECK_NO_MIRROR);
         c->opt.lean = !(value & XB_CHECK_GENERIC_WALKER);
         c->opt.mask_diag = !(value & XB_CHECK_FULL_TGRAD);
@@ -322,11 +326,12 @@
         c->opt.narrow_halo = !(value & XB_CHECK_WIDE_HALO);
         c->opt.ec_share = !(value & XB_CHECK_NO_EC_SHARE);
         c->opt.io_tiled = !(value & XB_CHECK_IO_GATHER);
+        c->opt.nb_bits = !(value & XB_CHECK_BRICK_LOOKUP);
         break;
     case XB_OPT_DEBUG: c->opt.dbg = value; break;
     case XB_OPT_EC_GROUPS: if ((ok = value >= 1 && value <= 4096)) c->opt.ec_groups = value; break;
     case XB_OPT_EC_QCAP: if ((ok = value >= 2 && value <= EC_Q)) c->opt.ec_qcap = value; break;
-    case XB_OPT_DROP_TABLE: c->grad_valid = false; if (value == XB_DROP_TABLE_AND_MAXIMA) c->brick_max_valid = false; break;
+    case XB_OPT_DROP_TABLE: c->grad_valid = false; c->grad_nb = false; if (value == XB_DROP_TABLE_AND_MAXIMA) c->brick_max_valid = false; break;
     case XB_OPT_KILL_LAUNCHES: if ((ok = value >= 1)) c->grow_kill_launches = value; break;
     case XB_OPT_SELF_EXCHANGE: c->opt.self_exchange = value != 0; break;
     case XB_OPT_ASYNC_COMM: c->opt.async_comm = value != 0; break;
@@ -364,7 +369,7 @@
                               (long long)c->mg_cap * MG_BYTES  +
                               (long long)c->vo_cap * 8 ;
     const long long fixed = 8 * N  + 4 * N  + (N + 16)  + 4 * N  + N  +
-                            2LL * c->max_cap * 4 + (long long)c->ovf_cap * 4 + c->blab_alloc * 5 + (long long)c->walk_cap * 3 * 80 +
+                            2LL * c->max_cap * 4 + (long long)c->ovf_cap * 4 + c->blab_alloc * 13 + (long long)c->walk_cap * 3 * 80 +
                             (1 << 22) ;
     if (bytes_total) *bytes_total = fixed + table + scratch;
     if (bytes_table) *bytes_table = table;
diff --git a/pybader_amd/csrc/bader_kernels.h b/pybader_amd/csrc/bader_kernels.h
--- a/pybader_amd/csrc/bader_kernels.h
+++ b/pybader_amd/csrc/bader_kernels.h
@@ -123,7 +123,7 @@
 struct __attribute__((aligned(32))) GradRec { double r0, r1, r2, key; };
 #define XB_STAY_CODE 63
 #define XB_OG_SELF 13
-#define XB_MAX_BOXES 1023
+#define XB_NOREC (-2147483647 - 1)
 __device__ __forceinline__ GradRec fetch_rec(const GradRec *__restrict__ G, int l) {
     return *reinterpret_cast<const GradRec *>(reinterpret_cast<const char *>(G) + ((unsigned long long)(unsigned)l << 5));
 }
@@ -136,17 +136,51 @@
 template <typename GT>
 __device__ __forceinline__ GradRec fetch_rec_w(const GT &g, const GradRec *__restrict__ G, int l) { return fetch_rec(G, rec_slot(g, l)); }
 
-__device__ __forceinline__ double pack_key(double rho, int code, int og) {
-    return __longlong_as_double((__double_as_longlong(rho) & ~0x1FFFFFLL) | (long long)(code | (og << 6)));
+#define XB_KEY_BITS 21
+#define XB_NB_SHIFT 11
+constexpr __host__ __device__ int nb_side(int pos) { return pos < 4 ? -1 : 1; }
+constexpr __host__ __device__ int nb_index(int cx, int cy, int cz) { return cx + 2 * cy + 4 * cz - 1; }
+constexpr __host__ __device__ int key_low(int code, int og, int nb) { return code | (og << 6) | ((nb & 127) << XB_NB_SHIFT); }
+constexpr __host__ __device__ int low_code(int bits) { return bits & 63; }
+constexpr __host__ __device__ int low_og(int bits) { return (bits >> 6) & 31; }
+constexpr __host__ __device__ bool low_nb_norec(int bits, int cx, int cy, int cz) {
+    return (cx | cy | cz) != 0 && ((bits >> (XB_NB_SHIFT + nb_index(cx, cy, cz))) & 1) != 0;
+}
+namespace nb_check {
+constexpr bool subsets_ok() {
+    for (int m = 1; m < 8; m++) {
+        const int cx = m & 1, cy = (m >> 1) & 1, cz = m >> 2;
+        if (nb_index(cx, cy, cz) != m - 1) return false;
+        for (int code = 0; code < 64; code += 21)
+            for (int og = 0; og < 27; og += 13) {
+                const int one = key_low(code, og, 1 << (m - 1)), rest = key_low(code, og, 127 & ~(1 << (m - 1)));
+                if (low_code(one) != code || low_og(one) != og || low_code(rest) != code || low_og(rest) != og) return false;
+                if (one >> XB_KEY_BITS || rest >> XB_KEY_BITS) return false;
+                for (int k = 1; k < 8; k++) {
+                    if (low_nb_norec(one, k & 1, (k >> 1) & 1, k >> 2) != (k == m)) return false;
+                    if (low_nb_norec(rest, k & 1, (k >> 1) & 1, k >> 2) != (k != m)) return false;
+                }
+                if (low_nb_norec(one, 0, 0, 0) || low_nb_norec(key_low(code, og, 127), 0, 0, 0)) return false;
+            }
+    }
+    return true;
+}
+static_assert(subsets_ok(), "7 neighbour bits, one per subset of crossed axes, clear of the step code and the ongrid successor");
+static_assert(nb_side(0) == -1 && nb_side(1) == -1 && nb_side(3) == -1 && nb_side(4) == 1 && nb_side(6) == 1 && nb_side(7) == 1,
+              "the low side is within reach from positions 0-1 only, the high side from 6-7 only");
+static_assert(key_low(XB_STAY_CODE, 26, 127) == 0x3FEBF && key_low(63, 31, 127) < (1 << 18), "bits 18-20 stay 0");
+}
+__device__ __forceinline__ double pack_key(double rho, int code, int og, int nb = 0) {
+    return __longlong_as_double((__double_as_longlong(rho) & ~0x1FFFFFLL) | (long long)key_low(code, og, nb));
 }
 __device__ __forceinline__ double key_floor(double rho) {
     const long long b = __double_as_longlong(rho);
     return __longlong_as_double(b >= 0 ? (b & ~0x1FFFFFLL) : (b | 0x1FFFFFLL));
 }
 __device__ __forceinline__ int key_bits(double key) { return (int)(__double_as_longlong(key) & 0x1FFFFFLL); }
-__device__ __forceinline__ int key_code(double key) { return key_bits(key) & 63; }
-__device__ __forceinline__ int key_og(double key) { return (key_bits(key) >> 6) & 31; }
-__device__ __forceinline__ int key_box(double key) { return key_bits(key) >> 11; }
+__device__ __forceinline__ int key_code(double key) { return low_code(key_bits(key)); }
+__device__ __forceinline__ int key_og(double key) { return low_og(key_bits(key)); }
+static_assert((1 << XB_KEY_BITS) - 1 == 0x1FFFFF, "key_bits / key_floor / pack_key share one mask");
 
 __device__ __forceinline__ int wrap_u(int q, int n) {
     unsigned u = min((unsigned)q, (unsigned)(q + n));
diff --git a/pybader_amd/csrc/host_assign.h b/pybader_amd/csrc/host_assign.h
--- a/pybader_amd/csrc/host_assign.h
+++ b/pybader_amd/csrc/host_assign.h
@@ -3,11 +3,13 @@
 
 static int ensure_brick_bytes(xb_ctx *c, int nbr) {
     if (c->blab_alloc < nbr) {
-        hipFree(c->blab_buf); c->blab_buf = nullptr; c->blab_alloc = 0; c->brick_rec = nullptr; c->brick_max_valid = false;
-        if (c->grad_cover) { c->grad_cover = 0; c->grad_valid = false; }
-        HIPCHK(hipMalloc(&c->blab_buf, (size_t)nbr * sizeof(int) + (size_t)nbr + 16));
+        hipFree(c->blab_buf); c->blab_buf = nullptr; c->blab_alloc = 0; c->brick_rec = nullptr; c->nb_tab = nullptr; c->brick_max_valid = false;
+        if (c->grad_cover) { c->grad_cover = 0; c->grad_valid = false; c->grad_nb = false; }
+        const size_t rec_bytes = ((size_t)nbr + 16 + 7) & ~(size_t)7;
+        HIPCHK(hipMalloc(&c->blab_buf, (size_t)nbr * sizeof(int) + rec_bytes + (size_t)nbr * sizeof(unsigned long long)));
         c->blab_alloc = nbr;
         c->brick_rec = reinterpret_cast<unsigned char *>(c->blab_buf + nbr);
+        c->nb_tab = reinterpret_cast<unsigned long long *>(c->brick_rec + rec_bytes);
     }
     return XB_OK;
 }
@@ -517,7 +519,7 @@
     if (h[FS_GROW_RETRY]) {
         c->grow_kill_launches = 1 << 20;
         c->stat_grow_retries++;
-        c->grad_valid = false;
+        c->grad_valid = false; c->grad_nb = false;
         return assign_neargrid_fused(c, n_maxima);
     }
     if (h[FS_TIES] == 0) c->grad_rule = 2;
@@ -625,7 +627,7 @@
         launch_region_growth(c, nb0, nb1, nb2, bmask, bmaxv, bpot, seed, buf0, buf1, box_max, box_first, true);
         HIPCHK(hipGetLastError());
     }
-    c->grad_valid = false;
+    c->grad_valid = false; c->grad_nb = false;
     c->grad_cover = 0;
     c->brick_max_valid = true;
     c->blab = c->blab_buf;
diff --git a/pybader_amd/csrc/host_context.h b/pybader_amd/csrc/host_context.h
--- a/pybader_amd/csrc/host_context.h
+++ b/pybader_amd/csrc/host_context.h
@@ -44,8 +44,8 @@
     hipFree(c->st); hipFree(c->stage); hipFree(c->ec_pend); c->ec_pend = nullptr; hipFree(c->ec_share); c->ec_share = nullptr; hipFree(c->ec_pflag); c->ec_pflag = nullptr; hipFree(c->max_list); hipFree(c->max_aux); hipFree(c->ovf_list);
     hipFree(c->blab_buf); c->blab_buf = nullptr; c->blab_alloc = 0; c->labels_zero_pending = false;
     hipFree(c->ec_buf); c->ec_buf = nullptr; c->ec_buf_cap = 0; c->grad_cap = 0; c->list_cap = 0;
-    c->brick_rec = nullptr; c->grad_cover = 0;
-    c->rho = nullptr; c->grad = nullptr; c->grad_valid = false; c->brick_max_valid = false; c->labels = nullptr; c->known = nullptr; c->first = nullptr; c->list = nullptr;
+    c->brick_rec = nullptr; c->nb_tab = nullptr; c->grad_cover = 0;
+    c->rho = nullptr; c->grad = nullptr; c->grad_valid = false; c->grad_nb = false; c->brick_max_valid = false; c->labels = nullptr; c->known = nullptr; c->first = nullptr; c->list = nullptr;
     c->st = nullptr; c->stage = nullptr; c->max_list = nullptr; c->max_aux = nullptr; c->ovf_list = nullptr;
     c->n_alloc = 0; c->stage_bytes = 0;
 }
@@ -113,7 +113,7 @@
     g.ntot = (int)c->N;
     if (c->grad_cap < want || c->grad_cap > 2 * want) {
         HIPCHK(hipStreamSynchronize(c->stream));
-        hipFree(c->grad); c->grad = nullptr; c->grad_cap = 0; c->grad_valid = false; c->brick_max_valid = false;
+        hipFree(c->grad); c->grad = nullptr; c->grad_cap = 0; c->grad_valid = false; c->grad_nb = false; c->brick_max_valid = false;
         HIPCHK(hipMalloc(&c->grad, (size_t)want * sizeof(GradRec)));
         c->grad_cap = want;
     }
@@ -160,19 +160,19 @@
     }
     c->zero_outside[0] = -1;
     Grid &g = c->g;
-    if (g.nx != (int)shape[0] || g.ny != (int)shape[1] || g.nz != (int)shape[2]) { c->grad_valid = false; c->brick_max_valid = false; c->have_rho = c->have_labels = false; adjacency_free(c); merge_free(c); }
+    if (g.nx != (int)shape[0] || g.ny != (int)shape[1] || g.nz != (int)shape[2]) { c->grad_valid = false; c->grad_nb = false; c->brick_max_valid = false; c->have_rho = c->have_labels = false; adjacency_free(c); merge_free(c); }
     if (dist_mat && !T_grad) return fail(XB_E_ARG, "xb_set_grid: dist_mat without T_grad");
     g.nx = (int)shape[0]; g.ny = (int)shape[1]; g.nz = (int)shape[2];
     g.nyz = g.ny * g.nz;
     g.x0 = (int)x0; g.x1 = (int)x1;
     if (dist_mat) {
-        if (memcmp(g.dist, dist_mat, sizeof g.dist) != 0) { c->grad_valid = false; c->brick_max_valid = false; }
+        if (memcmp(g.dist, dist_mat, sizeof g.dist) != 0) { c->grad_valid = false; c->grad_nb = false; c->brick_max_valid = false; }
         memcpy(g.dist, dist_mat, sizeof g.dist);
         HIPCHK(hipMemcpyAsync(c->dist_dev, dist_mat, sizeof g.dist, hipMemcpyHostToDevice, c->stream));
         HIPCHK(hipMemcpyAsync(c->dist_dev + 27, T_grad, sizeof g.T, hipMemcpyHostToDevice, c->stream));
         HIPCHK(hipStreamSynchronize(c->stream));
     }
-    if (T_grad && memcmp(g.T, T_grad, sizeof g.T) != 0) { memcpy(g.T, T_grad, sizeof g.T); c->grad_valid = false; c->brick_max_valid = false; }
+    if (T_grad && memcmp(g.T, T_grad, sizeof g.T) != 0) { memcpy(g.T, T_grad, sizeof g.T); c->grad_valid = false; c->grad_nb = false; c->brick_max_valid = false; }
     c->N = N;
     c->thin = thin;
     c->halo = (x0 == 0 && x1 == shape[0]) ? g.nx : 0;
@@ -311,7 +311,7 @@
 int xb_upload_density(xb_ctx *c, const double *rho_host) {
     if (c) c->vac_by_tol = false;
     NEED_GRID_THIN("xb_upload_density");
-    c->grad_valid = false; c->brick_max_valid = false; c->have_rho = true;
+    c->grad_valid = false; c->grad_nb = false; c->brick_max_valid = false; c->have_rho = true;
     if (int rc = staged_h2d(c, c->rho, rho_host, c->N * sizeof(double))) return rc;
     HIPCHK(hipStreamSynchronize(c->stream));
     return XB_OK;
@@ -346,7 +346,7 @@
                       int64_t *n_host) {
     if (!text || nbytes <= 0) return fail(XB_E_ARG, "%s: empty text", who);
     if (nbytes / (TPB * TXT_BYTES) >= (1LL << 31) - 2) return fail(XB_E_LIMIT, "%s: text too large", who);
-    c->grad_valid = false; c->brick_max_valid = false; c->have_rho = true;
+    c->grad_valid = false; c->grad_nb = false; c->brick_max_valid = false; c->have_rho = true;
     static const double P10[23] = {1e0, 1e1, 1e2, 1e3, 1e4, 1e5, 1e6, 1e7, 1e8, 1e9, 1e10, 1e11,
                                    1e12, 1e13, 1e14, 1e15, 1e16, 1e17, 1e18, 1e19, 1e20, 1e21, 1e22};
     const int nblk = (int)((nbytes + TPB * TXT_BYTES - 1) / (TPB * TXT_BYTES));
@@ -448,7 +448,7 @@
     if (n_atoms < 0 || n_atoms > XB_SYNTH_ATOMS_MAX) return fail(XB_E_ARG, "xb_synth_density: bad atom count");
     if ((16 + 5 * (size_t)n_atoms) * sizeof(double) > c->stage_bytes)
         return fail(XB_E_LIMIT, "xb_synth_density: %lld atoms do not fit the scratch buffer", (long long)n_atoms);
-    c->grad_valid = false; c->brick_max_valid = false; c->have_rho = true;
+    c->grad_valid = false; c->grad_nb = false; c->brick_max_valid = false; c->have_rho = true;
     double *tmp = (double *)c->stage;
     HIPCHK(hipMemcpyAsync(tmp, lattice, 9 * sizeof(double), hipMemcpyHostToDevice, c->stream));
     HIPCHK(hipMemcpyAsync(tmp + 16, atoms5, n_atoms * 5 * sizeof(double), hipMemcpyHostToDevice, c->stream));
diff --git a/pybader_amd/csrc/host_interop.h b/pybader_amd/csrc/host_interop.h
--- a/pybader_amd/csrc/host_interop.h
+++ b/pybader_amd/csrc/host_interop.h
@@ -120,7 +120,7 @@
     if (io_overlaps(lo, hi, c->rho, (size_t)c->N * 8)) return fail(XB_E_ARG, "xb_import_density: the source overlaps the resident density");
     c->vac_by_tol = false;
     NEED_GRID_THIN("xb_import_density");
-    c->grad_valid = false; c->brick_max_valid = false; c->have_rho = true;
+    c->grad_valid = false; c->grad_nb = false; c->brick_max_valid = false; c->have_rho = true;
     const hipStream_t s = (hipStream_t)stream;
     if (int rc = io_after_caller(c, s)) return rc;
     if (int rc = dtype == XB_F32 ? io_import_density(c, (const float *)dev_ptr, stride, c->rho) : io_import_density(c, (const double *)dev_ptr, stride, c->rho)) return rc;
diff --git a/pybader_amd/csrc/host_refine.h b/pybader_amd/csrc/host_refine.h
--- a/pybader_amd/csrc/host_refine.h
+++ b/pybader_amd/csrc/host_refine.h
@@ -268,7 +268,7 @@
                 }
             }
             HIPCHK(hipMemsetAsync(c->counters + CT_DEFER, 0, sizeof(int), c->stream));
-            launch_refine_trace<2, false>(c, nblocks(n), TPB, c->list, n, nullptr, c->counters + CT_CHANGED, c->counters + CT_ESCAPED, c->ovf_list,
+            (brec && !slab && nb_bits_ok(c) ? launch_refine_trace<2, false, false, false, true> : launch_refine_trace<2, false>)(c, nblocks(n), TPB, c->list, n, nullptr, c->counters + CT_CHANGED, c->counters + CT_ESCAPED, c->ovf_list,
                                           c->counters + CT_N_OVF, c->ovf_cap, brec, defer, c->counters + CT_DEFER, regions_ok, slab_regions, WalkerIO{});
             if (brec || slab || table_windowed(c))
                 launch_refine_trace<2, true>(c, 512, TPB, defer, 0, c->counters + CT_DEFER, c->counters + CT_CHANGED, c->counters + CT_ESCAPED, c->ovf_list,
@@ -656,7 +656,7 @@
         int *defer = (int *)c->stage;
         WalkerIO wl{};
         constexpr int XB_RT_BLOCK = 128;
-        launch_refine_trace<2, false>(c, (unsigned)((c->N / 16 + XB_RT_BLOCK - 1) / XB_RT_BLOCK), XB_RT_BLOCK, c->list, 0, fs + FS_N_EDGES,
+        (brec && nb_bits_ok(c) ? launch_refine_trace<2, false, false, false, true> : launch_refine_trace<2, false>)(c, (unsigned)((c->N / 16 + XB_RT_BLOCK - 1) / XB_RT_BLOCK), XB_RT_BLOCK, c->list, 0, fs + FS_N_EDGES,
                                       fs + FS_CHANGED, fs + FS_ESCAPED, c->ovf_list, fs + FS_R_OVF, c->ovf_cap, brec, defer, fs + FS_R_DEFER,
                                       regions_ok, nullptr, wl);
         if (c->grad_cover == 1 && !regions_ok)
@@ -792,7 +792,7 @@
             if (int rc2 = assign_neargrid_tail(c, n_maxima)) return rc2;
             return xb_refine(c, mode, iters, log, log_capacity, n_iters);
         }
-        c->grad_valid = false;
+        c->grad_valid = false; c->grad_nb = false;
         c->first_clean = false;
         c->buni_valid = false; c->regions_labels = false;
         if (n_iters) *n_iters = 0;
diff --git a/pybader_amd/csrc/host_slab_table.h b/pybader_amd/csrc/host_slab_table.h
--- a/pybader_amd/csrc/host_slab_table.h
+++ b/pybader_amd/csrc/host_slab_table.h
@@ -3,7 +3,7 @@
 int xb_set_table_window(xb_ctx *c, int64_t margin) {
     NEED_GRID("xb_set_table_window");
     Grid &g = c->g;
-    c->grad_valid = false;
+    c->grad_valid = false; c->grad_nb = false;
     c->table_stage = 0;
     const int own = g.x1 - g.x0;
     if (margin < 0 || own == g.nx) { g.wx0 = 0; g.wlen = g.nx; c->table_margin = -1; g.wbase = 0; return XB_OK; }
diff --git a/pybader_amd/csrc/host_stages.h b/pybader_amd/csrc/host_stages.h
--- a/pybader_amd/csrc/host_stages.h
+++ b/pybader_amd/csrc/host_stages.h
@@ -43,10 +43,17 @@
     else launch(diag ? k_brick_masks<GridS, 1, true> : k_brick_masks<GridS, 1, false>, gs);
 }
 
+static bool nb_bits_ok(const xb_ctx *c) { return c->grad_valid && c->grad_nb && c->opt.nb_bits; }
 static void launch_brick_records(xb_ctx *c, const int *list, const int *n_dev, int nbr, int nb1, int nb2) {
     const Grid &g = c->g;
+    const bool part = g.nx % BRK || g.ny % BRK || g.nz % BRK;
+    const bool mark = !table_windowed(c) && g.x0 == 0 && g.x1 == g.nx && !part && (!list || c->blab) && c->nb_tab;
+    c->grad_nb = mark;
+    if (mark)
+        k_nb_table<<<(nbr + 255) / 256, 256, 0, c->stream>>>(nbr / (nb1 * nb2), nb1, nb2, list ? c->blab : nullptr, c->brick_rec, c->nb_tab);
     auto launch = [&](auto kernel, const auto &gt) {
-        kernel<<<4096, TPB, 0, c->stream>>>(gt, c->rho, c->grad, list, n_dev, nbr, nb1, nb2, c->brick_rec, small_grid(g));
+        kernel<<<4096, TPB, 0, c->stream>>>(gt, c->rho, c->grad, list, n_dev, nbr, nb1, nb2, c->brick_rec, small_grid(g),
+                                            mark ? c->nb_tab : nullptr);
     };
     GridS gs;
     if (sym_grid(g, gs)) launch(k_brick_records<GridS>, gs);
@@ -87,7 +94,9 @@
     const bool window = table_windowed(c);
     int *ovf = window ? (int *)c->stage : c->ovf_list;
     const int ovf_cap = window ? (int)std::min<size_t>(c->stage_bytes / sizeof(int), 0x7fffffffu) : c->ovf_cap;
+    const bool nb = lean && !window && !part && nb_bits_ok(c);
     auto kernel = !lean ? k_ng_trace_g<2, 0>
+                : nb ? (lean == 4 ? k_ng_trace_g<2, 4, false, false, true> : k_ng_trace_g<2, 3, false, false, true>)
                 : window ? (lean == 4 ? k_ng_trace_g<2, 4, true> : k_ng_trace_g<2, 3, true>)
                 : part ? (lean == 4 ? k_ng_trace_g<2, 4, false, true> : k_ng_trace_g<2, 3, false, true>)
                 : (lean == 4 ? k_ng_trace_g<2, 4> : k_ng_trace_g<2, 3>);
@@ -135,11 +144,11 @@
     if (n_maxima) *n_maxima = nmax;
 }
 
-extern "C++" template <int K, bool RHO, bool RESUME = false, bool EXPORT = false>
+extern "C++" template <int K, bool RHO, bool RESUME = false, bool EXPORT = false, bool NB = false>
 static void launch_refine_trace(xb_ctx *c, unsigned grid, int block, const int *list, int n_host, const int *n_dev, int *changed, int *escaped,
                                 int *ovf_list, int *ovf_count, int ovf_cap, const unsigned char *brec, int *defer_list, int *defer_count,
                                 int regions_ok, const int *region_blab, const WalkerIO &wio) {
-    k_refine_trace<K, RHO, RESUME, EXPORT><<<grid, block, 0, c->stream>>>(light(c->g), c->grad, c->labels, c->known, list, n_host, n_dev, changed,
+    k_refine_trace<K, RHO, RESUME, EXPORT, NB><<<grid, block, 0, c->stream>>>(light(c->g), c->grad, c->labels, c->known, list, n_host, n_dev, changed,
                                                                            escaped, ovf_list, ovf_count, ovf_cap, trace_maxsteps(c->g), c->rho,
                                                                            c->dist_dev, brec, defer_list, defer_count, regions_ok, region_blab, wio);
 }
diff --git a/pybader_amd/csrc/k_edges.h b/pybader_amd/csrc/k_edges.h
--- a/pybader_amd/csrc/k_edges.h
+++ b/pybader_amd/csrc/k_edges.h
@@ -555,7 +555,7 @@
 };
 #define XB_WALKER_STUCK (-2147483647 - 1)
 
-template <int K, bool RHO, bool RESUME = false, bool EXPORT = false>
+template <int K, bool RHO, bool RESUME = false, bool EXPORT = false, bool NB = false>
 __global__ __launch_bounds__(TPB) void k_refine_trace(GridL g, const GradRec *__restrict__ G, int *labels,
                                                       int8_t *known, const int *__restrict__ list, int n_host,
                                                       const int *n_dev, int *changed, int *escaped, int *ovf_list,
@@ -565,6 +565,7 @@
                                                       int *defer_count, int regions_ok, const int *__restrict__ region_blab,
                                                       WalkerIO wio) {
     static_assert(!RESUME || (RHO && K == 2), "walkers are carried on by the from-rho kernel");
+    static_assert(!NB || (K == 2 && !RHO && !RESUME && !EXPORT), "neighbour bits: the lean retrace of one GPU");
     const int n = n_dev ? *n_dev : n_host;
     int n_ch = 0, n_es = 0;
   const XcdRange xr = xcd_range((n + (int)blockDim.x - 1) / (int)blockDim.x);
@@ -660,9 +661,12 @@
             if (moving) {
                 const bool in_win = plane_in_window(g, qx);
                 const bool ok_plane = plane_valid(g, qx);
-                GradRec nr = fetch_rec(G, in_win ? rec_slot(g, lq) : 0);
+                const bool nb_missing = NB && low_nb_norec(key_bits(rec.key), (px >> 3) != (qx >> 3), (py >> 3) != (qy >> 3), (pz >> 3) != (qz >> 3));
+                GradRec nr;
+                if (!NB) nr = fetch_rec(G, in_win ? rec_slot(g, lq) : 0);
+                else nr = fetch_rec(G, lq);
                 const int8_t kq = known[ok_plane ? lq : lp];
-                const bool missing = !(in_win && rec_exists(brick_rec, g, qx, qy, qz));
+                const bool missing = NB ? nb_missing : !(in_win && rec_exists(brick_rec, g, qx, qy, qz));
                 const bool in_region = region_blab && ok_plane && region_blab[((qx >> 3) * ((g.ny + 7) >> 3) + (qy >> 3)) * ((g.nz + 7) >> 3) + (qz >> 3)] > 0;
                 if (in_region || (!RHO && regions_ok && in_win && missing && ok_plane)) {
                     result = lq;
diff --git a/pybader_amd/csrc/k_masks.h b/pybader_amd/csrc/k_masks.h
--- a/pybader_amd/csrc/k_masks.h
+++ b/pybader_amd/csrc/k_masks.h
@@ -333,11 +333,37 @@
     }
 }
 
+__global__ void k_nb_table(int nb0, int nb1, int nb2, const int *__restrict__ blab, const unsigned char *__restrict__ brick_rec,
+                           unsigned long long *__restrict__ tab) {
+    const int b = blockIdx.x * blockDim.x + threadIdx.x;
+    if (b >= nb0 * nb1 * nb2) return;
+    const int b0 = b / (nb1 * nb2), b1 = (b / nb2) % nb1, b2 = b % nb2;
+    unsigned m27 = 0;
+#pragma unroll
+    for (int t = 0; t < 27; t++) {
+        const int nbk = (wrapi(b0 + t / 9 - 1, nb0) * nb1 + wrapi(b1 + (t / 3) % 3 - 1, nb1)) * nb2 + wrapi(b2 + t % 3 - 1, nb2);
+        const bool has = blab ? (blab[nbk] <= 0 && blab[nbk] != XB_NOREC) : (brick_rec[nbk] & 1) != 0;
+        m27 |= has ? 0u : 1u << t;
+    }
+    unsigned long long w = 0;
+#pragma unroll
+    for (int o = 0; o < 8; o++) {
+        const int s0 = nb_side((o >> 2) * 4) + 1, s1 = nb_side(((o >> 1) & 1) * 4) + 1, s2 = nb_side((o & 1) * 4) + 1;
+#pragma unroll
+        for (int m = 1; m < 8; m++) {
+            const int cx = m & 1, cy = (m >> 1) & 1, cz = m >> 2;
+            const unsigned no = (m27 >> ((cx ? s0 : 1) * 9 + (cy ? s1 : 1) * 3 + (cz ? s2 : 1))) & 1u;
+            w |= (unsigned long long)no << (8 * o + nb_index(cx, cy, cz));
+        }
+    }
+    tab[b] = w;
+}
+
 #define BR_ROW 24
 template <typename GT>
 __global__ __launch_bounds__(TPB, 4) void k_brick_records(GT g, const double *__restrict__ rho, GradRec *__restrict__ G,
                                                        const int *__restrict__ walk, const int *n_list, int nbr, int nb1, int nb2,
-                                                       unsigned char *brick_rec, int small) {
+                                                       unsigned char *brick_rec, int small, const unsigned long long *__restrict__ nb_tab) {
     __shared__ double tile[10][10][BR_ROW];
     const int n = walk ? *n_list : nbr;
     int goff[4], loff[4];
@@ -352,6 +378,7 @@
     for (int item = xr.begin; item < xr.end; item += xr.step) {
         const int b = walk ? walk[item] : item;
         if (!walk && !(brick_rec[b] & 1)) continue;
+        const unsigned long long nbw = nb_tab ? nb_tab[b] : 0ull;
         const int b0 = b / (nb1 * nb2), b1 = (b / nb2) % nb1, b2 = b % nb2;
         const int x0 = b0 * 8, y0 = b1 * 8, z0 = b2 * 8;
         const bool inner = !(small & 1) && x0 >= 1 && x0 + 8 < g.nx && y0 >= 1 && y0 + 8 < g.ny && z0 >= 1 && z0 + 8 < g.nz;
@@ -416,7 +443,7 @@
                 o.r2 = d2 - (double)i2;
                 code = (i0 + 1) | ((i1 + 1) << 2) | ((i2 + 1) << 4);
             }
-            o.key = pack_key(c, code, og);
+            o.key = pack_key(c, code, og, (int)(nbw >> (8 * (((tx >> 2) << 2) | ((ty >> 2) << 1) | (tz >> 2)))) & 127);
             if (inner || (x0 + tx < g.nx && y0 + ty < g.ny && z0 + tz < g.nz)) G[rec_slot(g, vbase + (tx * g.ny + ty) * g.nz + tz)] = o;
         }
         if (threadIdx.x == 0) brick_rec[b] |= 1;
diff --git a/pybader_amd/csrc/k_trace.h b/pybader_amd/csrc/k_trace.h
--- a/pybader_amd/csrc/k_trace.h
+++ b/pybader_amd/csrc/k_trace.h
@@ -107,7 +107,6 @@
     x = (x ^ (x >> 16)) & 0x000003ffu;
     return (int)x;
 }
-#define XB_NOREC (-2147483647 - 1)
 __device__ __forceinline__ bool brick_is_vacuum(const int *__restrict__ bpot, int b, double vac_tol) {
     if (!bpot) return false;
     const int p = bpot[b];
@@ -170,7 +169,6 @@
         if (lab0 != -1) {
             px = sx; py = sy; pz = sz;
             lp = v;
-            if (b <= 0) b = key_box(rec.key);
             if (b > 0) result = box_max[b - 1];
             else { w.init(v, rec.key); moving = true; }
         }
@@ -202,7 +200,7 @@
                 GradRec nr = fetch_rec(G, in_win ? rec_slot(g, lq) : 0);
                 const int bl = blab ? blab[((qx >> 3) * nb1 + (qy >> 3)) * nb2 + (qz >> 3)] : 0;
                 if (WIN && !in_win && bl <= 0) nr = make_rec_rho(g, rho, gc, qx, qy, qz);
-                const int b = bl > 0 ? bl : key_box(nr.key);
+                const int b = bl > 0 ? bl : 0;
                 if (bl == XB_NOREC) {
                     result = -2;
                     moving = false;
@@ -243,11 +241,12 @@
 }
 constexpr int XB_TRACE_WAVES = 4;
 __shared__ GradRec xb_s_rec[512];
-template <bool OFF32, bool CACHE, bool WINDOW = false>
+template <bool OFF32, bool CACHE, bool WINDOW = false, bool NB = false>
 __device__ __forceinline__ int ng_walk_lean(const GridL &g, const GradRec *__restrict__ G, const int *__restrict__ box_max,
                                              const int *__restrict__ blab, int nb1, int nb2, int sx, int sy, int sz,
                                              int *labels, int *first, int *max_list, int *max_count, int max_cap,
                                              int *ovf_list, int *ovf_count, int ovf_cap, int maxsteps, bool has_vacuum) {
+    static_assert(!NB || (CACHE && !WINDOW), "neighbour bits: the whole-grid table of the group trace");
     const int v = lin24(g, sx, sy, sz);
     const int lab0 = has_vacuum ? labels[v] : 0;
     const int ox8 = sx & ~7, oy8 = sy & ~7, oz8 = sz & ~7;
@@ -256,6 +255,7 @@
     int px = sx, py = sy, pz = sz, steps = 0;
     double dr0 = 0., dr1 = 0., dr2 = 0.;
     int i0 = v, i1 = -1;
+    bool norec = false;
     double k0 = rec.key, k1 = -1.7976931348623157e308, m_old = -1.7976931348623157e308;
 #ifdef XB_DEBUG_COUNT
     int dbg_lane_steps = 0;
@@ -265,6 +265,7 @@
         const double t0 = dr0 + rec.r0, t1 = dr1 + rec.r1, t2 = dr2 + rec.r2;
         const int id0 = rha_cs(t0), id1 = rha_cs(t1), id2 = rha_cs(t2);
         const int m0 = (bits & 3) + id0 - 1, m1 = ((bits >> 2) & 3) + id1 - 1, m2 = ((bits >> 4) & 3) + id2 - 1;
+        int cross = NB ? (((px ^ (px + m0)) >> 3) != 0) | ((((py ^ (py + m1)) >> 3) != 0) << 1) | ((((pz ^ (pz + m2)) >> 3) != 0) << 2) : 0;
         px += m0; py += m1; pz += m2;
         dr0 = t0 - (double)id0; dr1 = t1 - (double)id1; dr2 = t2 - (double)id2;
         if (__builtin_amdgcn_ballot_w64((unsigned)px >= (unsigned)g.nx || (unsigned)py >= (unsigned)g.ny || (unsigned)pz >= (unsigned)g.nz) != 0) {
@@ -280,17 +281,22 @@
                 og_offsets(og, ox, oy, oz);
                 at_max = og == XB_OG_SELF;
                 dr0 = dr1 = dr2 = 0.;
-                px = wrap3(wrap3(px - m0, g.nx) + ox, g.nx);
-                py = wrap3(wrap3(py - m1, g.ny) + oy, g.ny);
-                pz = wrap3(wrap3(pz - m2, g.nz) + oz, g.nz);
+                const int ux = wrap3(px - m0, g.nx), uy = wrap3(py - m1, g.ny), uz = wrap3(pz - m2, g.nz);
+                if (NB) cross = (((ux ^ (ux + ox)) >> 3) != 0) | ((((uy ^ (uy + oy)) >> 3) != 0) << 1) | ((((uz ^ (uz + oz)) >> 3) != 0) << 2);
+                px = wrap3(ux + ox, g.nx);
+                py = wrap3(uy + oy, g.ny);
+                pz = wrap3(uz + oz, g.nz);
                 lq = lin24(g, px, py, pz);
             }
         }
         int bl = 0;
         const bool own = CACHE && (unsigned)((px ^ ox8) | (py ^ oy8) | (pz ^ oz8)) < 8u;
         const bool in_win = !WINDOW || own || plane_in_window(g, px);
+        if (NB) norec = cross != 0 && ((bits >> (XB_NB_SHIFT - 1) >> cross) & 1) != 0;
         if (own) rec = xb_s_rec[((px & 7) << 6) | ((py & 7) << 3) | (pz & 7)];
-        else {
+        else if (NB) {
+            if (!norec) rec = fetch_rec_o<OFF32>(G, lq);
+        } else {
             rec = fetch_rec_o<OFF32>(G, WINDOW ? (in_win ? rec_slot(g, lq) : 0) : lq);
             const unsigned bidx = (unsigned)mad24(mad24(px >> 3, nb1, py >> 3), nb2, pz >> 3);
             bl = *reinterpret_cast<const int *>(reinterpret_cast<const char *>(blab) + (bidx << 2));
@@ -299,6 +305,7 @@
 #ifdef XB_DEBUG_COUNT
         dbg_lane_steps++;
 #endif
+        if (NB && norec) break;
         const bool arrived = bl > 0 && !at_max;
         const bool undecided = (!og_move && rec.key <= m_old) || steps > maxsteps || (WINDOW && !in_win) || bl == XB_NOREC;
         if (arrived) result = box_max[bl - 1];
@@ -308,6 +315,11 @@
         m_old = max_raw(m_old, k1);
         i1 = i0; k1 = k0;
         i0 = lq; k0 = rec.key;
+    }
+    if (NB && norec) {
+        const unsigned bidx = (unsigned)mad24(mad24(px >> 3, nb1, py >> 3), nb2, pz >> 3);
+        const int bl = *reinterpret_cast<const int *>(reinterpret_cast<const char *>(blab) + (bidx << 2));
+        result = bl > 0 ? box_max[bl - 1] : -2;
     }
 #ifdef XB_DEBUG_COUNT
     if (xb_dbg_steps) xb_dbg_steps[v] = (signed char)min(dbg_lane_steps, 127);
@@ -392,7 +404,7 @@
     return x & 7;
 }
 
-template <int K, int LEAN, bool WINDOW = false, bool PART = false>
+template <int K, int LEAN, bool WINDOW = false, bool PART = false, bool NB = false>
 __global__ __launch_bounds__(XB_WAVE * XB_TRACE_WAVES, 8) void k_ng_trace_g(GridL g, const GradRec *__restrict__ G, const int *__restrict__ box_max,
                                                        const int *__restrict__ blab, int nb1, int nb2,
                                                        const int *__restrict__ walk, int *fs, int *labels, int *first,
@@ -401,6 +413,7 @@
     __shared__ int s_base, s_next;
     __shared__ int s_w[8], s_mixed;
     constexpr bool CACHE = LEAN >= 3;
+    static_assert(!NB || (CACHE && !WINDOW && !PART), "neighbour bits: whole bricks, the whole grid (a cut brick narrower than 5 voxels reaches both sides of an axis)");
     int prev_brick = -1;
 #ifdef XB_DEBUG_COUNT
     const long long pr_t0 = clock64();
@@ -479,7 +492,7 @@
 #ifdef XB_DEBUG_COUNT
                     const long long pr_c = clock64();
 #endif
-                    const int res = ng_walk_lean<LEAN == 4, CACHE, WINDOW>(g, G, box_max, blab, nb1, nb2, sx, sy, sz, labels, first, max_list, &fs[FS_N_MAX],
+                    const int res = ng_walk_lean<LEAN == 4, CACHE, WINDOW, NB>(g, G, box_max, blab, nb1, nb2, sx, sy, sz, labels, first, max_list, &fs[FS_N_MAX],
                                                                 max_cap, ovf_list, &fs[FS_N_OVF], ovf_cap, maxsteps, has_vacuum != 0);
 #ifdef XB_DEBUG_COUNT
                     pr_walk += clock64() - pr_c;
diff --git a/pybader_amd/csrc/slab_step.h b/pybader_amd/csrc/slab_step.h
--- a/pybader_amd/csrc/slab_step.h
+++ b/pybader_amd/csrc/slab_step.h
@@ -310,12 +310,12 @@
     if (h[FS_GROW_RETRY]) {
         c->grow_kill_launches = 1 << 20;
         c->stat_grow_retries++;
-        c->grad_valid = false;
+        c->grad_valid = false; c->grad_nb = false;
         if (status) *status = 1;
         return XB_OK;
     }
     if (!h[FS_SORT_OK]) {
-        c->grad_valid = false;
+        c->grad_valid = false; c->grad_nb = false;
         if (status) *status = 2;
         return XB_OK;
     }
```

Result: faster. 43210 Mvoxels/s (median of 6 runs) (+2.3%).
